# QiminWu/mceik

Hardware: AMD Instinct MI355X
Metric: MCMC proposals/sec (FSM eikonal + likelihood), 128³ grid, 1/2/4/8 MI355X (higher is better)
Workload: dtype f32

## Files before the change

### mceik_amd/csrc/capi.hip

```cpp
#include <hip/hip_runtime.h>
#include <float.h>
#include <math.h>
#include <stdint.h>
#include <stdio.h>
#include <stdlib.h>
#include <string.h>
#include <unistd.h>

#include <algorithm>
#include <vector>

#include "../../include/mceik.h"
#include "fsm_common.h"
#include "mcmc_common.h"
#include "fsm_single.h"
#include "rccl_rt.h"

hipError_t fsm_launch(const FsmLaunch &L, int is_double, int nwaves, hipStream_t st);
hipError_t fsm_zero_words(unsigned *p, int n, hipStream_t st);
int fsm_occupancy(const FsmLaunch &L, int is_double);
size_t fsm_launch_lds_bytes(const FsmLaunch &L, int is_double);
int fsm_launch_kind(const FsmLaunch &L, int is_double);
const char *fsm_launch_name(const FsmLaunch &L, int is_double);
hipError_t fsm_to_brick_f64(const double *src, void *dst, int dst_double, const FsmLaunch &L, int nfield, hipStream_t st);
hipError_t fsm_from_brick_f64(const void *src, int src_double, double *dst, const FsmLaunch &L, int nfield, hipStream_t st);
hipError_t fsm_from_brick_f32(const float *src, float *dst, const FsmLaunch &L, int nfield, hipStream_t st);
hipError_t fsm_to_brick_f32(const float *src, float *dst, const FsmLaunch &L, int nfield, hipStream_t st);
hipError_t mcmc_propose(const McmcDev &D, uint64_t step, hipStream_t st);
hipError_t mcmc_init_loglik(const McmcDev &D, hipStream_t st);
hipError_t mcmc_accept(const McmcDev &D, int keep_slot, hipStream_t st);
hipError_t mcmc_lpt_order(const unsigned long long *clk, int nsolve, int *order, hipStream_t st);
hipError_t l2_gridsearch_f32(int ldgrd, int ngrd, int nev, int iwantOT, float t0use, const int *ev_ptr,
                             const int *obs_row, const float *tc, const float *wt, const float *xnorm,
                             const float *test, float *t0, float *objfn, int negate, hipStream_t st);
size_t relocate_lds_bytes(int nrows, int nobs, int nev);
hipError_t relocate_lds(int ldgrd, int ngrd, int nrows, int nev, int nobs, int iwantOT, float t0use,
                        const int *ev_ptr, const int *obs_row, const float *tc, const float *wt, const float *xnorm,
                        const float *test, float *t0, float *objfn, int negate, hipStream_t st);
hipError_t gridsearch_f90(int is_double, int ldgrd, int ngrd, int nuse, int iwantOT, const int *row,
                          const void *tob, const void *w0, const void *wl, const void *test, void *logpdf,
                          hipStream_t st);
hipError_t l2_gridsearch(int ldgrd, int ngrd, int nuse, int iwantOT, double t0use, const int *use,
                         const double *tc, const double *wt, double xnorm, const double *test,
                         double *t0, double *objfn, hipStream_t st);

#define HIPCHK(x)                                                                      \
    do {                                                                               \
        hipError_t e_ = (x);                                                           \
        if (e_ != hipSuccess) {                                                        \
            fprintf(stderr, "mceik_hip: %s failed: %s (%s:%d)\n", #x,                  \
                    hipGetErrorString(e_), __FILE__, __LINE__);                        \
            return -1;                                                                 \
        }                                                                              \
    } while (0)

static double conv_threshold(double tol, int is_double)
{
    double tolr = is_double ? tol : (double)(float)tol;
    if (!(tolr > 0.0)) return HUGE_VAL;
    int p = is_double ? 53 : 24;
    int k = (int)ceil(log2(tolr)) + p;
    while (ldexp(1.0, k - p) < tolr) k++;
    while (ldexp(1.0, k - 1 - p) >= tolr) k--;
    double T = ldexp(1.0, k);
    double big = is_double ? DBL_MAX : (double)FLT_MAX;
    return T > big ? HUGE_VAL : T;
}

static void fill_launch(FsmLaunch &L, const mceik_fsm_batch *b)
{
    memset(&L, 0, sizeof(L));
    L.nx = b->nx; L.ny = b->ny; L.nz = b->nz;
    fsm_geometry(&L, b->precision == 64 ? 8 : 4);
    L.maxit = b->maxit; L.max_sweeps = b->max_sweeps;
    L.tol = b->tol; L.h = b->h; L.x0 = b->x0; L.y0 = b->y0; L.z0 = b->z0;
    int is_double = b->precision == 64;
    double T = conv_threshold(b->tol, is_double);
    L.conv_thresh = is_double ? (T == HUGE_VAL ? DBL_MAX : T) : (T == HUGE_VAL ? (double)FLT_MAX : T);
    L.nsolve = b->nmodel * b->nstat; L.nstat = b->nstat; L.nsrc = b->nsrc;
    L.src = b->src;
    L.slow_mode = b->slow_mode;
    L.nrx = b->nrx > 0 ? b->nrx : 1; L.nry = b->nry > 0 ? b->nry : 1; L.nrz = b->nrz > 0 ? b->nrz : 1;
    L.ncx = mceik_div_up(L.nx, L.nrx); L.ncy = mceik_div_up(L.ny, L.nry); L.ncz = mceik_div_up(L.nz, L.nrz);
    L.magic_rx = ((1u << 20) + L.nrx - 1) / L.nrx;
    L.magic_ry = ((1u << 20) + L.nry - 1) / L.nry;
    L.magic_rz = ((1u << 20) + L.nrz - 1) / L.nrz;
    L.ev_node = b->ev_node; L.nev = b->nev; L.ttab = b->ttab; L.ev_frac = b->ev_frac;
    L.model_phase = b->slow_mode == 1 ? b->model_phase : nullptr;
    L.skip = b->skip;
    L.solve_count = b->solve_count;
    L.nphase = b->nphase > 0 ? b->nphase : 1;
    {
        auto span = [](int a, int e, int nr) { return e / nr - a / nr + 1; };
        int mx = 0, my = 0, mz = 0;
        for (int t = 0; t < L.ntx; t++) {
            int v = span(t * 8, t * 8 + 7 < L.nx - 1 ? t * 8 + 7 : L.nx - 1, L.nrx); mx = v > mx ? v : mx;
        }
        for (int t = 0; t < L.nty; t++) {
            int v = span(t * 8, t * 8 + 7 < L.ny - 1 ? t * 8 + 7 : L.ny - 1, L.nry); my = v > my ? v : my;
        }
        for (int t = 0; t < L.nzk; t++) {
            int a = t * L.kb * 8, e = a + L.kb * 8 - 1 < L.nz - 1 ? a + L.kb * 8 - 1 : L.nz - 1;
            int v = span(a, e, L.nrz); mz = v > mz ? v : mz;
        }
        L.ccb = mx * my * mz;
        L.cell_cache = b->slow_mode == 1 && L.ccb <= MCEIK_CC_MAX && L.nx < 4096 && L.ny < 4096 && L.nz < 4096;
        if (!L.cell_cache) L.ccb = 0;
    }
    L.fast_sqrt = b->fast_sqrt;
    L.niter = b->niter; L.ierr = b->ierr;
    L.iter_total = b->iter_total;
    L.visit_stats = b->visit_stats;
    L.solve_order = b->solve_order;
    L.solve_clock = b->solve_clock;
    L.max_waves = b->max_waves;
    L.traffic = b->traffic;
    L.step_z = b->step_z;
}

static int g_device_cus = 0;

static int device_cus()
{
    if (g_device_cus == 0) {
        int dev = 0;
        hipDeviceProp_t p;
        if (hipGetDevice(&dev) == hipSuccess && hipGetDeviceProperties(&p, dev) == hipSuccess)
            g_device_cus = p.multiProcessorCount;
        else
            g_device_cus = 256;
    }
    return g_device_cus;
}

static size_t ws_budget_bytes()
{
    static size_t budget = 0;
    if (budget == 0) {
        const char *e = getenv("MCEIK_FSM_WS_GB");
        double gb = e ? atof(e) : 0.0;
        if (gb > 0.0) {
            budget = (size_t)(gb * 1073741824.0);
        } else {
            size_t fr = 0, tot = 0;
            const size_t margin = (size_t)8 << 30;
            if (hipMemGetInfo(&fr, &tot) == hipSuccess && tot) {
                budget = tot / 5 * 4;
                const size_t avail = fr > 2 * margin ? fr - margin : fr / 2;
                if (avail < budget) budget = avail;
            } else {
                budget = (size_t)96 << 30;
            }
        }
    }
    return budget;
}

static int batch_waves(const FsmLaunch &L, int is_double)
{
    int per_cu = fsm_occupancy(L, is_double);
    if (per_cu < 1) per_cu = 1;
    static const int env_cap = [] { const char *e = getenv("MCEIK_WAVES_PER_CU"); return e ? atoi(e) : 0; }();
    if (env_cap > 0 && env_cap < per_cu) per_cu = env_cap;
    long w = (long)per_cu * device_cus();
    if (L.max_waves > 0 && w > L.max_waves) w = L.max_waves;
    if (w > L.nsolve) w = L.nsolve;
    static const bool report = getenv("MCEIK_LAUNCH_REPORT") != nullptr;
    if (report)
        fprintf(stderr, "mceik fsm launch: %d-z steps, %d waves/CU (occupancy), %ld resident waves, %zu B LDS per wave\n",
                fsm_launch_kind(L, is_double), per_cu, w, fsm_launch_lds_bytes(L, is_double));
    return (int)(w < 1 ? 1 : w);
}

static int fsm_batch_waves_uncapped(const mceik_fsm_batch *b)
{
    FsmLaunch L;
    fill_launch(L, b);
    return batch_waves(L, b->precision == 64);
}

struct WsLayout {
    size_t counter, slow, u, u0, zf, total;
    int nwaves;
};

static WsLayout ws_layout(const mceik_fsm_batch *b)
{
    FsmLaunch L;
    fill_launch(L, b);
    int is_double = b->precision == 64;
    size_t es = is_double ? 8 : 4;
    WsLayout w;
    w.nwaves = batch_waves(L, is_double);
    const size_t zfw = fsm_launch_kind(L, is_double) == 16 ? zf_bytes(L, es) : 0;
    {
        const size_t per_wave = 2 * L.field_elems * es + zfw;
        const long cap = (long)(ws_budget_bytes() / (per_wave ? per_wave : 1));
        if (cap >= 1 && w.nwaves > cap) w.nwaves = (int)cap;
    }
    w.counter = 0;
    w.slow = 1024;
    size_t slow_bytes = b->slow_mode == 0 ? (size_t)b->nmodel * L.field_elems * es : 0;
    w.u = w.slow + ((slow_bytes + 255) & ~(size_t)255);
    size_t nu = b->u_out ? (size_t)L.nsolve : (size_t)w.nwaves;
    w.u0 = w.u + nu * L.field_elems * es;
    w.zf = w.u0 + (size_t)w.nwaves * L.field_elems * es;
    w.total = w.zf + (size_t)w.nwaves * zfw;
    return w;
}

extern "C" size_t mceik_fsm_workspace_bytes(const mceik_fsm_batch *b)
{
    return ws_layout(b).total;
}

extern "C" int mceik_fsm_step_z(const mceik_fsm_batch *b)
{
    if (!b) return 0;
    FsmLaunch L;
    fill_launch(L, b);
    return fsm_launch_kind(L, b->precision == 64);
}

extern "C" const char *mceik_fsm_kernel_name(const mceik_fsm_batch *b)
{
    if (!b) return "";
    FsmLaunch L;
    fill_launch(L, b);
    return fsm_launch_name(L, b->precision == 64);
}

extern "C" size_t mceik_fsm_lds_bytes(const mceik_fsm_batch *b)
{
    if (!b) return 0;
    FsmLaunch L;
    fill_launch(L, b);
    return fsm_launch_lds_bytes(L, b->precision == 64);
}

extern "C" double mceik_fsm_bytes_per_node_sweep(const mceik_fsm_batch *b)
{
    double es = b->precision == 64 ? 8.0 : 4.0;
    double s = b->slow_mode == 0 ? es : 4.0 / ((double)b->nrx * b->nry * b->nrz);
    return 2.0 * es + s / (b->nstat > 0 ? b->nstat : 1);
}

#define MCEIK_MC_CHUNK 64
struct McmcExt {
    const void *dev;
    unsigned *sync;
    unsigned spin_limit;
    int step0, nsteps, nburn, keepk, maxs, nkept0;
};

static int fsm_batch_solve_impl(const mceik_fsm_batch *b, void *workspace, size_t workspace_bytes, void *stream,
                                const McmcExt *ext);

extern "C" int mceik_fsm_batch_solve(const mceik_fsm_batch *b, void *workspace, size_t workspace_bytes,
                                     void *stream)
{
    return fsm_batch_solve_impl(b, workspace, workspace_bytes, stream, nullptr);
}

static int fsm_batch_solve_impl(const mceik_fsm_batch *b, void *workspace, size_t workspace_bytes, void *stream,
                                const McmcExt *ext)
{
    if (!b || b->nx < 2 || b->ny < 2 || b->nz < 2 || b->nx > 4096 || b->ny > 4096 || b->nz > 4096 ||
        b->nsrc < 1 ||
        b->nmodel < 1 || b->nstat < 1 || !(b->precision == 32 || b->precision == 64)) {
        fprintf(stderr, "mceik_fsm_batch_solve: invalid batch description\n");
        return 1;
    }
    if (b->slow_mode == 1 && b->precision != 32 && b->precision != 64) return 1;
    WsLayout w = ws_layout(b);
    {
        FsmLaunch G;
        fill_launch(G, b);
        if (G.field_elems * (b->precision == 64 ? 8 : 4) >= (size_t)1 << 31) {
            fprintf(stderr, "mceik_fsm_batch_solve: one travel-time field must stay below 2 GiB\n");
            return 1;
        }
        if (fsm_launch_lds_bytes(G, b->precision == 64) > MCEIK_MAX_LDS) {
            fprintf(stderr, "mceik_fsm_batch_solve: %d x %d x %d z-blocks exceed the LDS block tables\n", G.ntx, G.nty,
                    G.nzk);
            return 1;
        }
        const bool held = fsm_launch_kind(G, b->precision == 64) == 16 || fsm_compact_layout(G, 8);
        const int infl = fsm_launch_kind(G, b->precision == 64) == 16 ? fsm16_geo(G).infl : G.infl;
        if (held && hold_clock_bound(G.nblocks, infl) >= 65536) {
            fprintf(stderr, "mceik_fsm_batch_solve: %d z-blocks overflow the held stream's 16-bit clocks\n", G.nblocks);
            return 1;
        }
    }
    if (!workspace || workspace_bytes < w.total) {
        fprintf(stderr, "mceik_fsm_batch_solve: workspace too small (%zu < %zu)\n", workspace_bytes, w.total);
        return 1;
    }
    if (b->skip && b->u_out) {
        fprintf(stderr, "mceik_fsm_batch_solve: skip and u_out cannot be combined (a skipped solve has no field)\n");
        return 1;
    }
    hipStream_t st = (hipStream_t)stream;
    int is_double = b->precision == 64;
    FsmLaunch L;
    fill_launch(L, b);
    char *ws = (char *)workspace;
    L.counter = (unsigned *)(ws + w.counter);
    HIPCHK(fsm_zero_words(L.counter, 256, st));
    if (b->slow_mode == 0) {
        void *sb = ws + w.slow;
        if (is_double)
            HIPCHK(fsm_to_brick_f64((const double *)b->slow, sb, 1, L, b->nmodel, st));
        else
            HIPCHK(fsm_to_brick_f32((const float *)b->slow, (float *)sb, L, b->nmodel, st));
        L.slow = sb;
    } else {
        L.slow = b->slow;
    }
    L.u = ws + w.u;
    L.u0 = ws + w.u0;
    L.zf = ws + w.zf;
    L.slot_per_solve = b->u_out ? 1 : 0;
    if (ext) {
        if (is_double || fsm_launch_kind(L, 0) != 16 || b->solve_order || b->u_out) return 1;
        L.mc_dev = ext->dev;
        L.mc_sync = ext->sync;
        L.mc_spin_limit = ext->spin_limit;
        L.mc_step0 = ext->step0; L.mc_nsteps = ext->nsteps;
        L.mc_nburn = ext->nburn; L.mc_keepk = ext->keepk; L.mc_maxs = ext->maxs; L.mc_nkept0 = ext->nkept0;
        HIPCHK(fsm_zero_words(ext->sync, MC_SYNC_WORDS(L.nsolve / L.nstat) - 1, st));
    }
    HIPCHK(fsm_launch(L, is_double, w.nwaves, st));
    if (b->u_out) {
        if (is_double) HIPCHK(fsm_from_brick_f64(L.u, 1, (double *)b->u_out, L, L.nsolve, st));
        else HIPCHK(fsm_from_brick_f32((const float *)L.u, (float *)b->u_out, L, L.nsolve, st));
    }
    return 0;
}

static bool is_device_ptr(const void *p)
{
    hipPointerAttribute_t a;
    if (!p || hipPointerGetAttributes(&a, p) != hipSuccess) {
        (void)hipGetLastError();
        return false;
    }
    return a.type == hipMemoryTypeDevice;
}

extern "C" int eikonal3d_batch_solve(int nmodels, int nstations, int nx, int ny, int nz, double h, double x0,
                                     double y0, double z0, int maxit, double tol, const double *src,
                                     const float *slow, float *u, int *niter, int *ierr)
{
    if (nmodels < 1 || nstations < 1 || !src || !slow || !u) return 1;
    const size_t n = (size_t)nx * ny * nz, nsolve = (size_t)nmodels * nstations;
    mceik_fsm_batch b;
    memset(&b, 0, sizeof(b));
    b.nx = nx; b.ny = ny; b.nz = nz; b.h = h; b.x0 = x0; b.y0 = y0; b.z0 = z0;
    b.maxit = maxit; b.tol = tol; b.precision = 32;
    b.nmodel = nmodels; b.nstat = nstations; b.nsrc = 1; b.slow_mode = 0; b.max_sweeps = -1;
    std::vector<void *> tmp;
    auto stage = [&](const void *p, size_t bytes, bool in) -> void * {
        if (is_device_ptr(p)) return const_cast<void *>(p);
        void *d = nullptr;
        if (hipMalloc(&d, bytes) != hipSuccess) return nullptr;
        tmp.push_back(d);
        if (in && hipMemcpy(d, p, bytes, hipMemcpyHostToDevice) != hipSuccess) return nullptr;
        return d;
    };
    int rc = 0;
    void *d_src = stage(src, (size_t)nstations * 4 * sizeof(double), true);
    void *d_slow = stage(slow, (size_t)nmodels * n * sizeof(float), true);
    void *d_u = stage(u, nsolve * n * sizeof(float), false);
    void *d_it = niter ? stage(niter, nsolve * sizeof(int), false) : nullptr;
    void *d_ie = ierr ? stage(ierr, nsolve * sizeof(int), false) : nullptr;
    void *ws = nullptr;
    if (!d_src || !d_slow || !d_u || (niter && !d_it) || (ierr && !d_ie)) rc = -1;
    if (!rc) {
        b.src = (const double *)d_src; b.slow = d_slow; b.u_out = d_u;
        b.niter = (int *)d_it; b.ierr = (int *)d_ie;
        const size_t wsb = mceik_fsm_workspace_bytes(&b);
        if (hipMalloc(&ws, wsb) != hipSuccess) rc = -1;
        else rc = mceik_fsm_batch_solve(&b, ws, wsb, nullptr);
        if (!rc && hipDeviceSynchronize() != hipSuccess) rc = -1;
    }
    if (!rc && d_u != u) rc = hipMemcpy(u, d_u, nsolve * n * sizeof(float), hipMemcpyDeviceToHost) != hipSuccess;
    if (!rc && niter && d_it != niter) rc = hipMemcpy(niter, d_it, nsolve * sizeof(int), hipMemcpyDeviceToHost) != hipSuccess;
    if (!rc && ierr && d_ie != ierr) rc = hipMemcpy(ierr, d_ie, nsolve * sizeof(int), hipMemcpyDeviceToHost) != hipSuccess;
    if (ws) hipFree(ws);
    for (void *p : tmp) hipFree(p);
    return rc;
}

extern "C" int mceik_memcpy(void *dst, const void *src, size_t bytes, int kind)
{
    hipMemcpyKind k = kind == 0 ? hipMemcpyHostToDevice : kind == 1 ? hipMemcpyDeviceToHost : hipMemcpyDeviceToDevice;
    HIPCHK(hipMemcpy(dst, src, bytes, k));
    return 0;
}

struct SingleState {
    int init;
    int nx, ny, nz, maxit_cap, nsrc_cap;
    int is_double;
    SingleLaunch L;
    void *mem;
    double *dense, *src;
    int *ierr_bc;
    int nwaves;
    int bcfail;
    hipStream_t st;
    int iverb, maxit;
    double x0, y0, z0, h, tol;
    BlockDecomp D;
    double *snap;
    unsigned *d_count;
};
static SingleState g_single[3];

static void single_free(SingleState &S)
{
    if (S.snap) hipFree(S.snap);
    if (S.d_count) hipFree(S.d_count);
    if (S.mem) hipFree(S.mem);
    if (S.st) hipStreamDestroy(S.st);
    const SingleState keep = S;
    memset(&S, 0, sizeof(S));
    S.init = keep.init;
    S.iverb = keep.iverb; S.maxit = keep.maxit;
    S.x0 = keep.x0; S.y0 = keep.y0; S.z0 = keep.z0; S.h = keep.h; S.tol = keep.tol;
    S.D = keep.D;
}

static int blocks_buffers(SingleState &S)
{
    const size_t np = (size_t)S.L.nxp * S.L.nyp * S.L.nzp;
    if (!S.snap && hipMalloc(&S.snap, np * 8) != hipSuccess) { S.snap = nullptr; return 1; }
    if (!S.d_count && hipMalloc(&S.d_count, 16) != hipSuccess) { S.d_count = nullptr; return 1; }
    return 0;
}

static int single_alloc(SingleState &S, int is_double, int nx, int ny, int nz, int maxit, int nsrc)
{
    if (S.mem && S.is_double == is_double && S.nx == nx && S.ny == ny && S.nz == nz && maxit <= S.maxit_cap &&
        nsrc <= S.nsrc_cap)
        return 0;
    const int keep = S.init;
    single_free(S);
    S.init = keep;
    if (nx < 1 || ny < 1 || nz < 1 || (long)nx * ny * nz >= (1L << 31)) return 1;
    SingleLaunch &L = S.L;
    L.nx = nx; L.ny = ny; L.nz = nz;
    L.gx = nx; L.gy = ny; L.gz = nz;
    L.nbx = mceik_div_up(nx, 8); L.nby = mceik_div_up(ny, 8); L.nbz = mceik_div_up(nz, 8);
    if (L.nbx > 1024 || L.nby > 1024 || L.nbz > 1024) return 1;
    L.nxp = 8 * L.nbx; L.nyp = 8 * L.nby; L.nzp = 8 * L.nbz;
    L.nb = L.nbx * L.nby * L.nbz;
    if ((size_t)L.nxp * L.nyp * L.nzp * (is_double ? 8 : 4) >= ((size_t)1 << 31)) return 1;
    const int mcap = maxit > 0 ? maxit : 1, scap = nsrc > 0 ? nsrc : 1;
    const size_t es = is_double ? 8 : 4, np = (size_t)L.nxp * L.nyp * L.nzp, n = (size_t)nx * ny * nz;
    auto al = [](size_t v) { return (v + 255) & ~(size_t)255; };
    size_t off[12], o = 0;
    off[0] = o; o += al(np * es);
    off[1] = o; o += al(np * es);
    off[2] = o; o += al(np * es);
    off[3] = o; o += al(np);
    off[4] = o; o += al((size_t)L.nb * 4);
    off[5] = o; o += al((size_t)L.nb * 4);
    off[6] = o; o += al((size_t)(32 + mcap) * 4);
    off[7] = o; o += al((size_t)mcap * 8);
    off[8] = o; o += al((size_t)mcap * 4);
    off[9] = o; o += al(n * 8);
    off[10] = o; o += al((size_t)scap * 32);
    off[11] = o; o += al(16);
    if (hipMalloc(&S.mem, o) != hipSuccess) { S.mem = nullptr; return 1; }
    char *m = (char *)S.mem;
    L.u = m + off[0]; L.u0 = m + off[1]; L.slow = m + off[2]; L.bc = (unsigned char *)(m + off[3]);
    L.border = (const int *)(m + off[4]); L.done = (unsigned *)(m + off[5]); L.ctl = (unsigned *)(m + off[6]);
    L.arrive = (unsigned long long *)(m + off[7]); L.ierr_it = (int *)(m + off[8]);
    S.dense = (double *)(m + off[9]); S.src = (double *)(m + off[10]); S.ierr_bc = (int *)(m + off[11]);
    L.bcerr = S.ierr_bc;
    std::vector<int> ord;
    ord.reserve(L.nb);
    for (int lev = 0; lev <= L.nbx + L.nby + L.nbz - 3; lev++)
        for (int bz = 0; bz < L.nbz; bz++)
            for (int by = 0; by < L.nby; by++) {
                const int bx = lev - bz - by;
                if (bx >= 0 && bx < L.nbx) ord.push_back(bx | (by << 10) | (bz << 20));
            }
    if ((int)ord.size() != L.nb ||
        hipMemcpy((void *)L.border, ord.data(), ord.size() * 4, hipMemcpyHostToDevice) != hipSuccess ||
        hipStreamCreateWithFlags(&S.st, hipStreamNonBlocking) != hipSuccess) {
        single_free(S);
        return 1;
    }
    static const int wpc = [] { const char *e = getenv("MCEIK_SINGLE_WAVES_PER_CU"); return e ? atoi(e) : 2; }();
    int occ = fsm_single_occupancy(is_double);
    S.nwaves = device_cus() * std::max(1, std::min(wpc, occ));
    S.is_double = is_double; S.nx = nx; S.ny = ny; S.nz = nz; S.maxit_cap = mcap; S.nsrc_cap = scap;
    return 0;
}

static int single_solve(SingleState &S, int maxit, int nsrc, double tol, double h, double x0, double y0, double z0,
                        const double *ts, const double *xs, const double *ys, const double *zs, const double *slow,
                        double *u, int *niter_out)
{
    SingleLaunch &L = S.L;
    const size_t n = (size_t)L.nx * L.ny * L.nz;
    L.maxit = maxit; L.tol = tol; L.h = h; L.x0 = x0; L.y0 = y0; L.z0 = z0;
    std::vector<double> src((size_t)nsrc * 4);
    for (int k = 0; k < nsrc; k++) {
        src[k * 4 + 0] = ts[k]; src[k * 4 + 1] = xs[k]; src[k * 4 + 2] = ys[k]; src[k * 4 + 3] = zs[k];
    }
    const int mcap = maxit > 0 ? maxit : 1;
    std::vector<unsigned> ctl(32 + mcap);
    std::vector<int> ierr_it(mcap);
    int ierr_bc = 0;
    hipStream_t st = S.st;
    if (hipMemcpyAsync(S.dense, slow, n * 8, hipMemcpyHostToDevice, st) != hipSuccess ||
        hipMemcpyAsync(S.src, src.data(), src.size() * 8, hipMemcpyHostToDevice, st) != hipSuccess ||
        fsm_single_pad(S.dense, (void *)L.slow, S.is_double, L.nx, L.ny, L.nz, L.nxp, L.nyp, st) != hipSuccess ||
        hipMemsetAsync(L.done, 0, (size_t)L.nb * 4, st) != hipSuccess ||
        hipMemsetAsync(L.ctl, 0, (size_t)(32 + mcap) * 4, st) != hipSuccess ||
        hipMemsetAsync(L.arrive, 0, (size_t)mcap * 8, st) != hipSuccess ||
        hipMemsetAsync(L.ierr_it, 0, (size_t)mcap * 4, st) != hipSuccess ||
        fsm_single_solve(L, S.is_double, S.src, nsrc, S.ierr_bc, S.nwaves, st) != hipSuccess ||
        fsm_single_unpad(L.u, S.dense, S.is_double, L.nx, L.ny, L.nz, L.nxp, L.nyp, st) != hipSuccess ||
        hipMemcpyAsync(u, S.dense, n * 8, hipMemcpyDeviceToHost, st) != hipSuccess ||
        hipMemcpyAsync(ctl.data(), L.ctl, ctl.size() * 4, hipMemcpyDeviceToHost, st) != hipSuccess ||
        hipMemcpyAsync(ierr_it.data(), L.ierr_it, ierr_it.size() * 4, hipMemcpyDeviceToHost, st) != hipSuccess ||
        hipMemcpyAsync(&ierr_bc, S.ierr_bc, 4, hipMemcpyDeviceToHost, st) != hipSuccess ||
        hipStreamSynchronize(st) != hipSuccess)
        return -1;
    if (ctl[1] != 0) {
        std::vector<unsigned> done(L.nb);
        std::vector<unsigned long long> arr(mcap);
        hipMemcpy(done.data(), L.done, done.size() * 4, hipMemcpyDeviceToHost);
        hipMemcpy(arr.data(), L.arrive, arr.size() * 8, hipMemcpyDeviceToHost);
        unsigned dmin = ~0u, dmax = 0;
        for (unsigned d : done) { dmin = std::min(dmin, d); dmax = std::max(dmax, d); }
        fprintf(stderr, "mceik_hip: single-solve schedule timed out (code %u; waits timed out: deps %u, "
                        "iteration %u; tasks taken %u, nb %d, done %u..%u, arrivals it0 %llu/%llu it1 %llu, "
                        "decisions %u %u %u)\n", ctl[1], ctl[3], ctl[4], ctl[0], L.nb, dmin, dmax,
                arr[0] & 0xffffffffull, arr[0] >> 32, mcap > 1 ? arr[1] & 0xffffffffull : 0ull, ctl[32],
                mcap > 1 ? ctl[33] : 0u, mcap > 2 ? ctl[34] : 0u);
        return -1;
    }
    S.bcfail = ierr_bc != 0;
    if (ierr_bc) {
        if (niter_out) *niter_out = 0;
        return 1;
    }
    int niter = maxit > 0 ? maxit : 0;
    for (int it = 0; it < maxit; it++)
        if (ctl[32 + it] == 2) { niter = it + 1; break; }
    if (niter_out) *niter_out = niter;
    return niter > 0 ? ierr_it[niter - 1] : 0;
}

static void serial_driver(int is_double, const int *job, const int *iverb, const int *maxit,
                          const int *nsrc, const int *nx, const int *ny, const int *nz,
                          const double *tol, const double *h, const double *x0, const double *y0,
                          const double *z0, const double *ts, const double *xs, const double *ys,
                          const double *zs, const double *slow, double *u, int *ierr)
{
    SingleState &S = g_single[is_double];
    *ierr = 0;
    if (*job == 1) {
        if (S.init) { printf(" eikonal3d_serial_driver: Already initialized!\n"); *ierr = 1; return; }
        if (*iverb > 0) printf(" eikonal3d_serial_driver: Generating levels...\n");
        if (single_alloc(S, is_double, *nx, *ny, *nz, *maxit, *nsrc)) {
            printf(" eikonal3d_serial_driver: Error generating level structure\n");
            *ierr = 1;
            return;
        }
        S.init = 1;
        return;
    }
    if (*job != 2) {
        if (!S.init) printf(" eikonal3d_serial_driver: Never initialized!\n");
        single_free(S);
        S.init = 0;
        return;
    }
    if (!S.init) { printf(" eikonal3d_serial_driver: Solver not initalized!\n"); *ierr = 1; return; }
    if (*nsrc < 1) {
        printf(" eikonal3d_serial_driver: nsrc must be >= 1\n");
        *ierr = 1;
        return;
    }
    if (single_alloc(S, is_double, *nx, *ny, *nz, *maxit, *nsrc)) {
        printf(" eikonal3d_serial_driver: device allocation failed\n");
        *ierr = 1;
        return;
    }
    if (*iverb > 0) printf(" eikonal3d_serial_driver: Setting boundary conditions...\n");
    const int rc = single_solve(S, *maxit, *nsrc, *tol, *h, *x0, *y0, *z0, ts, xs, ys, zs, slow, u, nullptr);
    if (rc < 0) {
        printf(" eikonal3d_serial_driver: device failure\n");
        *ierr = 1;
        return;
    }
    *ierr = rc;
    if (S.bcfail) printf(" eikonal3d_serial_driver: Error setting boundary conditions\n");
    else if (rc != 0) printf(" eikonal3d_serial_driver: Error solving eikonal equation\n");
}

extern "C" void eikonal3d_serial_driver(const int *job, const int *iverb, const int *maxit, const int *nsrc,
                                        const int *nx, const int *ny, const int *nz, const double *tol,
                                        const double *h, const double *x0, const double *y0, const double *z0,
                                        const double *ts, const double *xs, const double *ys, const double *zs,
                                        const double *slow, double *u, int *ierr)
{
    serial_driver(1, job, iverb, maxit, nsrc, nx, ny, nz, tol, h, x0, y0, z0, ts, xs, ys, zs, slow, u, ierr);
}

extern "C" void eikonal3d_serial_driver_sp(const int *job, const int *iverb, const int *maxit, const int *nsrc,
                                           const int *nx, const int *ny, const int *nz, const double *tol,
                                           const double *h, const double *x0, const double *y0, const double *z0,
                                           const double *ts, const double *xs, const double *ys, const double *zs,
                                           const double *slow, double *u, int *ierr)
{
    serial_driver(0, job, iverb, maxit, nsrc, nx, ny, nz, tol, h, x0, y0, z0, ts, xs, ys, zs, slow, u, ierr);
// ... 1581 lines not shown
```

### mceik_amd/csrc/fsm16_kernel.hip

```cpp
#include <hip/hip_runtime.h>
#include <float.h>
#include <stdint.h>

#include "fsm_common.h"
#include "fsm_device.h"
#include "fsm_hold.h"
#include "fsm_update.h"
#include "mcmc_device.h"

namespace {

__device__ __forceinline__ uint32_t zoff16(int zb)
{
    const uint32_t u = (uint32_t)zb;
    return ((u >> 1) << 13) | ((u & 1u) << 6);
}

#ifdef MCEIK_PHASECLK
#undef TRAF
#undef TRAFU
#define TRAF(S, k, pred, bytes) do { } while (0)
#define TRAFU(S, k, bytes) do { } while (0)
#define PCLK(k)                                                                                         \
    do {                                                                                                \
        const unsigned long long t_ = __builtin_readcyclecounter();                                     \
        if (threadIdx.x == 0) S.scratch[8 + (k)] += (int)(t_ - pclk_t);                                 \
        pclk_t = t_;                                                                                    \
    } while (0)
#else
#define PCLK(k) do { } while (0)
#endif

struct Smem16 {
    int *box;
    float *cc;
    unsigned short *order;
    unsigned short *lastproc;
    unsigned short *lastchg;
    int *ring_e, *ring_b;
    unsigned *ring_base;
    unsigned *fmask;
    int *scratch;
    float *xr;
    unsigned *meta;
    unsigned char *fz;
    unsigned *vbits, *cbits;
};
template <bool FIXED>
__device__ __forceinline__ Smem16 smem16_bind(const FsmLaunch &L, unsigned char *base)
{
    size_t off[MCEIK_SMEM16_ARRAYS];
    if (FIXED) {
        off[8] = F16_CINFO; off[7] = F16_XR; off[1] = F16_CC; off[5] = F16_RING; off[6] = F16_SCRATCH;
        off[3] = F16_LASTPROC; off[4] = F16_LASTCHG; off[2] = F16_ORDER;
        off[9] = F16_ORDER + mceik_align16((size_t)L.ntiles * 2);
        off[10] = off[9] + mceik_align16((size_t)L.ntiles);
        off[0] = off[10] + f16_bitmap_bytes(L);
    } else {
        fsm16_smem_layout(L, off);
    }
    const int nr = fsm16_geo(L).nr;
    Smem16 S;
    S.box = reinterpret_cast<int *>(base + off[0]);
    S.cc = reinterpret_cast<float *>(base + off[1]);
    S.order = reinterpret_cast<unsigned short *>(base + off[2]);
    S.lastproc = reinterpret_cast<unsigned short *>(base + off[3]);
    S.lastchg = reinterpret_cast<unsigned short *>(base + off[4]);
    S.ring_e = reinterpret_cast<int *>(base + off[5]);
    S.ring_b = S.ring_e + (FIXED ? F16_NR : nr);
    S.ring_base = reinterpret_cast<unsigned *>(S.ring_b + (FIXED ? F16_NR : nr));
    S.fmask = S.ring_base + (FIXED ? F16_NR : nr);
    S.fz = base + off[9];
    S.vbits = reinterpret_cast<unsigned *>(base + off[10]);
    S.cbits = S.vbits + (L.nblocks + 31) / 32;
    S.scratch = reinterpret_cast<int *>(base + off[6]);
    S.xr = reinterpret_cast<float *>(base + off[7]);
    S.meta = reinterpret_cast<unsigned *>(base + off[8]);
    return S;
}

#define XROW16(arr, q, row) (((arr) * 4 + (q)) * MCEIK_X16Q + (row) * 4)
typedef float f4v16 __attribute__((ext_vector_type(4)));
__device__ __forceinline__ void lds_w4(float *p, float a, float b, float c, float d)
{
    *reinterpret_cast<f4v16 *>(p) = f4v16{a, b, c, d};
}
__device__ __forceinline__ void lds_r4(const float *p, float &a, float &b, float &c, float &d)
{
    const f4v16 v = *reinterpret_cast<const f4v16 *>(p);
    a = v.x; b = v.y; c = v.z; d = v.w;
}
__device__ __forceinline__ void store_row16(float *x, int arr, int lane, const float (&v)[16])
{
#pragma unroll
    for (int q = 0; q < 4; q++) lds_w4(x + XROW16(arr, q, lane), v[4 * q], v[4 * q + 1], v[4 * q + 2], v[4 * q + 3]);
}
__device__ __forceinline__ void load_row16(const float *x, int arr, int row, float (&v)[16])
{
#pragma unroll
    for (int q = 0; q < 4; q++) lds_r4(x + XROW16(arr, q, row), v[4 * q], v[4 * q + 1], v[4 * q + 2], v[4 * q + 3]);
}
__device__ __forceinline__ void load_half16(const float *x, int arr, int row, int h, float (&v)[8])
{
    lds_r4(x + XROW16(arr, 2 * h, row), v[0], v[1], v[2], v[3]);
    lds_r4(x + XROW16(arr, 2 * h + 1, row), v[4], v[5], v[6], v[7]);
}
__device__ __forceinline__ void halo_stage16(float *x, int lane, const float (&v)[8])
{
    const int j = lane >> 1, h = lane & 1;
    const int arr = (j >> 3) & 1, row = 64 + ((j >> 4) << 3) + (j & 7);
    lds_w4(x + XROW16(arr, 2 * h, row), v[0], v[1], v[2], v[3]);
    lds_w4(x + XROW16(arr, 2 * h + 1, row), v[4], v[5], v[6], v[7]);
}

#define NPASS16 4
#define W1_ZD (1u << 24)

__device__ __forceinline__ void seg_issue(Rsrc r, uint32_t seg, float (&a)[16])
{
    const bool odd = threadIdx.x & 1;
    const uint32_t segp = dpp_swap_pair(seg);
    float t[4];
    bload4(r, odd ? segp + 16u : seg, t);
    a[0] = t[0]; a[1] = t[1]; a[2] = t[2]; a[3] = t[3];
    bload4(r, odd ? segp + 48u : seg + 32u, t);
    a[4] = t[0]; a[5] = t[1]; a[6] = t[2]; a[7] = t[3];
    bload4(r, odd ? seg + 16u : segp, t);
    a[8] = t[0]; a[9] = t[1]; a[10] = t[2]; a[11] = t[3];
    bload4(r, odd ? seg + 48u : segp + 32u, t);
    a[12] = t[0]; a[13] = t[1]; a[14] = t[2]; a[15] = t[3];
}
#define XQE MCEIK_X16Q
__device__ __forceinline__ int pair_row(int arr, int lane)
{
    return (lane & 1) ? XROW16(arr, 1, lane - 1) : XROW16(arr, 0, lane);
}
__device__ __forceinline__ void raw_write(float *x, int pb, const float (&a)[16])
{
    lds_w4(x + pb, a[0], a[1], a[2], a[3]);
    lds_w4(x + pb + 2 * XQE, a[4], a[5], a[6], a[7]);
    lds_w4(x + pb + 4, a[8], a[9], a[10], a[11]);
    lds_w4(x + pb + 2 * XQE + 4, a[12], a[13], a[14], a[15]);
}
__device__ __forceinline__ void raw_read(const float *x, int pb, float (&a)[16])
{
    lds_r4(x + pb, a[0], a[1], a[2], a[3]);
    lds_r4(x + pb + 2 * XQE, a[4], a[5], a[6], a[7]);
    lds_r4(x + pb + 4, a[8], a[9], a[10], a[11]);
    lds_r4(x + pb + 2 * XQE + 4, a[12], a[13], a[14], a[15]);
}
template <int P>
struct Par16 {
    static constexpr int value = P;
};

struct LineLd {
    float a[8];
    int rowl, rowo;
};
__device__ __forceinline__ void line_issue(Rsrc r, uint32_t seg, bool isl, LineLd &q, float (&h)[8])
{
    const int lane = threadIdx.x, par = lane & 1;
    const bool islp = dpp_swap_pair((unsigned)isl) != 0u;
    const uint32_t segp = dpp_swap_pair(seg);
    const uint32_t sl = isl ? seg : (islp ? segp : OOB);
    const uint32_t o = (uint32_t)par * 16u;
    float t[4];
    bload4(r, sl + o, t);
    q.a[0] = t[0]; q.a[1] = t[1]; q.a[2] = t[2]; q.a[3] = t[3];
    bload4(r, sl + o + 32u, t);
    q.a[4] = t[0]; q.a[5] = t[1]; q.a[6] = t[2]; q.a[7] = t[3];
    const uint32_t sh = sl ^ 64u;
    bload4(r, sh + o, t);
    h[0] = t[0]; h[1] = t[1]; h[2] = t[2]; h[3] = t[3];
    bload4(r, sh + o + 32u, t);
    h[4] = t[0]; h[5] = t[1]; h[6] = t[2]; h[7] = t[3];
    q.rowl = isl ? lane : (lane ^ 1);
    q.rowo = lane ^ (q.rowl == lane ? 1 : 0);
}
__device__ __forceinline__ void line_write(float *x, const LineLd &q, const float (&hp)[8])
{
    const int par = threadIdx.x & 1;
    lds_w4(x + XROW16(1, par, q.rowl), q.a[0], q.a[1], q.a[2], q.a[3]);
    lds_w4(x + XROW16(1, par + 2, q.rowl), q.a[4], q.a[5], q.a[6], q.a[7]);
    lds_w4(x + XROW16(1, par, q.rowo), hp[0], hp[1], hp[2], hp[3]);
    lds_w4(x + XROW16(1, par + 2, q.rowo), hp[4], hp[5], hp[6], hp[7]);
}

__device__ __forceinline__ void raw_store(Rsrc r, uint32_t seg, bool chg, const float (&t)[16])
{
    const bool odd = threadIdx.x & 1;
    const uint32_t own = chg ? seg : OOB;
    const uint32_t oth = dpp_swap_pair(own);
    const uint32_t o = odd ? 16u : 0u;
    const uint32_t b01 = (odd ? oth : own) + o, b23 = (odd ? own : oth) + o;
    bstore4(r, b01, t[0], t[1], t[2], t[3]);
    bstore4(r, b01 + 32u, t[4], t[5], t[6], t[7]);
    bstore4(r, b23, t[8], t[9], t[10], t[11]);
    bstore4(r, b23 + 32u, t[12], t[13], t[14], t[15]);
}
__device__ __forceinline__ void store16_plain(Rsrc r, uint32_t off, const float (&v)[16])
{
#pragma unroll
    for (int q = 0; q < 4; q++) bstore4(r, off + 16u * q, v[4 * q], v[4 * q + 1], v[4 * q + 2], v[4 * q + 3]);
}

__device__ __forceinline__ void bload4h(Rsrc r, uint32_t off, float (&v)[4])
{
    f4v a = __builtin_bit_cast(f4v, __builtin_amdgcn_raw_buffer_load_b128(r, off, 0, 0));
    v[0] = a.x; v[1] = a.y; v[2] = a.z; v[3] = a.w;
}
struct BInfo16 {
    uint32_t seg;
    uint32_t zh;
    uint32_t lseg;
    uint32_t w1, w2, w3;
    __device__ __forceinline__ int fl() const { return (int)(w1 & 0xfffu); }
    __device__ __forceinline__ int zb() const { return (int)((w1 >> 12) & 0xffu); }
    __device__ __forceinline__ int ri() const { return (int)((w1 >> 20) & 0xfu); }
    __device__ __forceinline__ int ccb() const { return (int)(w2 << 16) >> 16; }
    __device__ __forceinline__ int clk() const { return (int)(w2 >> 16); }
    __device__ __forceinline__ int bid() const { return (int)(w3 & 0xffffu); }
    __device__ __forceinline__ int bcm() const { return (int)(w3 >> 16); }
};
template <bool RZ>
__device__ __forceinline__ BInfo16 brick_info16(const FsmLaunch &L, const Fsm16Geo &g, int kb, const Smem16 &S,
                                                const Pos &p, int nstream, int lx, int ly, const BcBoxes &bc,
                                                unsigned meta, uint32_t col)
{
    BInfo16 b;
    const int tz = ci_tz(meta);
    const int zb = tz * kb + (RZ ? kb - 1 - p.zbs : p.zbs);
    const bool valid = pos_valid(p, nstream) && (meta & C_BLK) && zb < g.nzb;
    b.seg = valid ? col + zoff16(zb) : OOB;
    b.lseg = pos_valid(p, nstream) && (meta & C_BLK) && (zb & ~1) < g.nzb ? col + zoff16(zb) : OOB;
    const int zu = RZ ? zb * 16 + 16 : zb * 16 - 1;
    b.zh = (valid && (meta & C_ZH) && p.zbs == 0) ? col + zoff16(zu >> 4) + (uint32_t)(zu & 15) * 4u : OOB;
    int fl = valid ? (int)((meta & 0x7f) | F_VALID) : 0;
    if (zb == (RZ ? g.nzb - 1 : 0)) fl |= F_FIRST;
    if (zb == (RZ ? 0 : g.nzb - 1)) fl |= F_LAST;
    const bool zd = valid && p.zbs == kb - 1 && !(fl & F_LAST);
    if (b.zh != OOB) b.zh = zf_boundary<float, RZ>(L, S.ring_b[p.ri], false, lx, ly);
    if (zd) b.zh = zf_boundary<float, RZ>(L, S.ring_b[p.ri], true, lx, ly);
    if ((meta & C_ZH) && p.zbs == 0) fl |= F_ZH;
    bool slow = (fl & C_PART) || ((fl & C_00) && zb == 0) || (valid && zb * 16 + 16 > L.nz);
    unsigned bcm = 0;
    if (__any(fl & C_BC)) {
        const int e = S.ring_e[p.ri];
        const int x = (e & 0xfff) * 8 + lx, y = ((e >> 12) & 0xfff) * 8 + ly;
        unsigned m = 0;
        if (fl & C_BC) {
            for (int k = 0; k < bc.n; k++) {
                const int *q = bc.box + 6 * k;
                if (x >= q[0] && x <= q[1] && y >= q[2] && y <= q[3]) {
                    int lo = q[4] - zb * 16, hi = q[5] - zb * 16;
                    lo = lo < 0 ? 0 : lo; hi = hi > 15 ? 15 : hi;
                    if (lo <= hi) m |= ((2u << hi) - (1u << lo));
                }
            }
        }
        bcm = m;
        slow |= m != 0;
    }
    if (slow) fl |= F_SLOW;
    const int ccb = ci_ccb(meta) + zb * 4;
    b.w1 = (uint32_t)fl | ((uint32_t)(valid ? zb : 0) << 12) | ((uint32_t)p.ri << 20) | (zd ? W1_ZD : 0u);
    b.w2 = ((uint32_t)ccb & 0xffffu) | ((uint32_t)p.sp << 16);
    b.w3 = ((uint32_t)S.ring_b[p.ri] & 0xffffu) | (bcm << 16);
    return b;
}
template <bool RZ>
__device__ __forceinline__ uint32_t halo_offset16(const Fsm16Geo &g, int kb, const Pos &pe, int nstream, int half,
                                                  unsigned meta, uint32_t col, unsigned hbit, uint32_t hdelta)
{
    const int zb = ci_tz(meta) * kb + (RZ ? kb - 1 - pe.zbs : pe.zbs);
    const bool valid = pos_valid(pe, nstream) && (meta & C_BLK) && zb < g.nzb;
    const uint32_t base = col + ((meta & hbit) ? 0u : hdelta);
    return valid ? base + zoff16(zb) + (uint32_t)half * 32u : OOB;
}

#define LW_G(p) (9 + 5 * (p))
#define LW_CCB 19
template <bool RZ>
__device__ __forceinline__ unsigned lean_word(const FsmLaunch &L, const Fsm16Geo &g, const ColTile &ct, int tz, int ri,
                                              int u0flag, int zh)
{
    int cz0, nczb;
    block_zcells(L, L.kb, tz, cz0, nczb);
    const int m = ct.fl | C_BLK | (u0flag ? C_U0 : 0) | (zh ? C_ZH : 0);
    const int zb0 = 2 * tz + (RZ ? 1 : 0);
    unsigned w = (unsigned)m & 0x1ffu;
#pragma unroll
    for (int p = 0; p < 2; p++) {
        const int zb = RZ ? zb0 - p : zb0 + p;
        unsigned gp = zb < g.nzb ? 16u : 0u;
        if (zb == (RZ ? g.nzb - 1 : 0)) gp |= 1u;
        if (zb == (RZ ? 0 : g.nzb - 1)) gp |= 2u;
        if ((m & C_PART) || ((m & C_00) && zb == 0) || zb * 16 + 16 > L.nz) gp |= 4u;
        if (p == 0 && (m & C_ZH)) gp |= 8u;
        w |= gp << LW_G(p);
    }
    const int ccb0 = ri * L.ccb + ct.cl * nczb - cz0 + zb0 * 4;
    return w | ((unsigned)ccb0 << LW_CCB);
}
template <bool RZ>
__device__ __forceinline__ BInfo16 brick_info_lean(const FsmLaunch &L, const Smem16 &S, const Pos &p, int nstream,
                                                   int lx, int ly, const BcBoxes &bc, unsigned w, uint32_t base)
{
    BInfo16 b;
    const int ph = p.zbs;
    const unsigned gp = (w >> (ph ? LW_G(1) : LW_G(0))) & 31u;
    const bool pv = pos_valid(p, nstream);
    const bool valid = pv && (gp & 16u);
    const uint32_t off = base + ((uint32_t)(ph ^ (RZ ? 1 : 0)) << 6);
    b.seg = valid ? off : OOB;
    b.lseg = pv && (w & ((16u << LW_G(0)) | (16u << LW_G(1)))) ? off : OOB;
    b.zh = valid && (gp & 8u) ? off + (RZ ? 8192u - 64u : 124u - 8192u) : OOB;
    const bool zd = valid && ph == 1 && !(gp & 2u);
    if (b.zh != OOB) b.zh = zf_boundary<float, RZ>(L, S.ring_b[p.ri], false, lx, ly);
    if (zd) b.zh = zf_boundary<float, RZ>(L, S.ring_b[p.ri], true, lx, ly);
    int fl = valid ? (int)((w & 0x7fu) | F_VALID | ((gp & 15u) << 8)) : 0;
    unsigned bcm = 0;
    if (__any(fl & C_BC)) {
        const int e = S.ring_e[p.ri];
        const int zb = 2 * ((e >> 24) & 0xff) + (RZ ? 1 - ph : ph);
        const int x = (e & 0xfff) * 8 + lx, y = ((e >> 12) & 0xfff) * 8 + ly;
        if (fl & C_BC) {
            for (int k = 0; k < bc.n; k++) {
                const int *q = bc.box + 6 * k;
                if (x >= q[0] && x <= q[1] && y >= q[2] && y <= q[3]) {
                    int lo = q[4] - zb * 16, hi = q[5] - zb * 16;
                    lo = lo < 0 ? 0 : lo; hi = hi > 15 ? 15 : hi;
                    if (lo <= hi) bcm |= ((2u << hi) - (1u << lo));
                }
            }
        }
        if (bcm) fl |= F_SLOW;
    }
    const int ccb = (int)(w >> LW_CCB) + (RZ ? -4 * ph : 4 * ph);
    b.w1 = (uint32_t)fl | ((uint32_t)ph << 12) | ((uint32_t)p.ri << 20) | (zd ? W1_ZD : 0u);
    b.w2 = ((uint32_t)ccb & 0xffffu) | ((uint32_t)p.sp << 16);
    b.w3 = ((uint32_t)S.ring_b[p.ri] & 0xffffu) | (bcm << 16);
    return b;
}
template <bool RZ>
__device__ __forceinline__ uint32_t halo_offset_lean(const Pos &pe, int nstream, int half, unsigned me, uint32_t base,
                                                     unsigned hbit, uint32_t hdelta)
{
    const int ph = pe.zbs;
    const bool valid = pos_valid(pe, nstream) && ((me >> (ph ? LW_G(1) : LW_G(0))) & 16u);
    const uint32_t o = base + ((me & hbit) ? 0u : hdelta) + ((uint32_t)(ph ^ (RZ ? 1 : 0)) << 6) + (uint32_t)half * 32u;
    return valid ? o : OOB;
}
template <bool RZ>
__device__ __forceinline__ uint32_t halo_line_lean(const Pos &pe, int nstream, unsigned me, uint32_t base,
                                                   unsigned hbit, uint32_t hdelta)
{
    const bool valid = pos_valid(pe, nstream) && (me & ((16u << LW_G(0)) | (16u << LW_G(1))));
    return valid ? base + ((me & hbit) ? 0u : hdelta) : OOB;
}
__device__ __forceinline__ unsigned dpp_swap_quad_half(unsigned v)
{
    return (unsigned)__builtin_amdgcn_mov_dpp((int)v, 0x4E, 0xf, 0xf, false);
}
template <bool RZ, bool LEAN>
__device__ __forceinline__ BInfo16 brick_info_any(const FsmLaunch &L, const Fsm16Geo &g, int kb, const Smem16 &S,
                                                  const Pos &p, int nstream, int lx, int ly, const BcBoxes &bc,
                                                  unsigned meta, uint32_t col)
{
    if (LEAN) return brick_info_lean<RZ>(L, S, p, nstream, lx, ly, bc, meta, col);
    return brick_info16<RZ>(L, g, kb, S, p, nstream, lx, ly, bc, meta, col);
}
template <bool RZ, bool LEAN>
__device__ __forceinline__ uint32_t halo_offset_any(const Fsm16Geo &g, int kb, const Pos &pe, int nstream, int half,
                                                    unsigned meta, uint32_t col, unsigned hbit, uint32_t hdelta)
{
    if (LEAN) return halo_offset_lean<RZ>(pe, nstream, half, meta, col, hbit, hdelta);
    return halo_offset16<RZ>(g, kb, pe, nstream, half, meta, col, hbit, hdelta);
}

__device__ __forceinline__ void build_order16(const FsmLaunch &L, unsigned short *order)
{
    for (int id = threadIdx.x; id < L.ntiles; id += 64) {
        const int txs = id % L.ntx, tys = id / L.ntx, dg = txs + tys;
        int rank = 0;
        for (int e = 0; e < dg; e++)
            rank += min(e, L.nty - 1) - max(0, e - L.ntx + 1) + 1;
        rank += tys - max(0, dg - L.ntx + 1);
        order[rank] = (unsigned short)(txs | (tys << 8));
    }
}


__device__ __forceinline__ HoldLds<unsigned short> hold_lds16(const Smem16 &S)
{
    HoldLds<unsigned short> H;
    H.order = S.order; H.fz = S.fz; H.lastproc = S.lastproc; H.need = S.lastchg; H.fmask = S.fmask;
    H.ring_e = S.ring_e; H.vbits = S.vbits; H.cbits = S.cbits;
    return H;
}


template <bool RZ, bool LEAN>
__device__ __forceinline__ void admit16(const FsmLaunch &L, const Fsm16Geo &g, const Smem16 &S, const BcBoxes &bc,
                                        int entry, int zh, int u0flag, int ri, int C, int lx, int ly, int lxs,
                                        int lys, int rx, int ry, ColTile &ct)
{
    unsigned meta = 0;
    int bid = 0, nbv = 0;
    uint32_t base = 0;
    if (entry >= 0) {
        const int tz = (entry >> 24) & 0xff, tx = entry & 0xfff, ty = (entry >> 12) & 0xfff;
        bid = tz * L.ntiles + tx + ty * L.ntx;
        nbv = min(L.kb, L.nzb - tz * L.kb);
        if ((entry & 0xffffff) != ct.tile) column_tile<float>(L, bc, entry, lx, ly, lxs, lys, rx, ry, ct);
        meta = LEAN ? lean_word<RZ>(L, g, ct, tz, ri, u0flag, zh) : column_word(L, L.kb, ct, tz, ri, u0flag, zh);
        base = (uint32_t)(ty * L.ntx + tx) * tile_bytes<float>(L) + (LEAN ? (uint32_t)tz << 13 : 0u);
    }
    const int nact = L.visit_stats && entry >= 0 ? __builtin_popcountll(__ballot(ct.fl & C_ACT)) : 0;
    asm volatile("" ::: "memory");
    S.meta[ri * 64 + threadIdx.x] = meta;
    if (threadIdx.x == 0) {
        if (entry >= 0) {
            S.lastproc[bid] = (unsigned short)C;
            S.vbits[bid >> 5] |= 1u << (bid & 31);
            if (L.visit_stats) {
                S.scratch[0] += nbv;
                S.scratch[1] += nbv * nact;
            }
        }
        S.ring_e[ri] = entry;
        S.ring_b[ri] = bid;
        S.ring_base[ri] = base;
    }
    asm volatile("" ::: "memory");
}


template <bool RZ, bool GENERIC, bool LEAN, bool NC = true>
__device__ __forceinline__ void brick16(const FsmLaunch &L, const Smem16 &S, const BInfo16 &b0, float (&v)[16],
                                        float zprev0, float znext, int lx, int ly, int rx, int ry, bool &changed,
                                        bool &nc, int &ierr_last, bool &c0, bool &c15)
{
    const int lane = threadIdx.x;
    const float T = (float)L.conv_thresh;
    const int fl = b0.fl();
    bool xp = true, xn = true, yp = true, yn = true, act = true;
    int zbg = 0;
    if (GENERIC) {
        const int e = S.ring_e[b0.ri()];
        zbg = LEAN ? 2 * ((e >> 24) & 0xff) + (RZ ? 1 - b0.zb() : b0.zb()) : b0.zb();
        const int x = (e & 0xfff) * 8 + lx, y = ((e >> 12) & 0xfff) * 8 + ly;
        const bool xlo = x > 0, xhi = x < L.nx - 1, ylo = y > 0, yhi = y < L.ny - 1;
        xp = rx ? xhi : xlo; xn = rx ? xlo : xhi; yp = ry ? yhi : ylo; yn = ry ? ylo : yhi;
        act = (fl & C_ACT) != 0;
    }
    const bool first = (fl & F_FIRST) != 0, last = (fl & F_LAST) != 0;
    const int lxs = lane & 7, lys = lane >> 3;
    const int rxm = lxs > 0 ? lane - 1 : 64 + lys, rym = lys > 0 ? lane - 8 : 72 + lxs;
    const int rxp = lxs < 7 ? lane + 1 : 64 + lys, ryp = lys < 7 ? lane + 8 : 72 + lxs;
    float fc = 0.f, ffc = 0.f, ff2c = 0.f, ff3c = 0.f;
#pragma unroll
    for (int hh = 0; hh < NPASS16; hh++) {
        constexpr int PZ = 16 / NPASS16;
        const int h = RZ ? NPASS16 - 1 - hh : hh;
        float xm[PZ], xq[PZ], ym[PZ], yq[PZ];
        lds_r4(S.xr + XROW16(0, h, rxm), xm[0], xm[1], xm[2], xm[3]);
        lds_r4(S.xr + XROW16(0, h, rym), ym[0], ym[1], ym[2], ym[3]);
        lds_r4(S.xr + XROW16(1, h, rxp), xq[0], xq[1], xq[2], xq[3]);
        lds_r4(S.xr + XROW16(1, h, ryp), yq[0], yq[1], yq[2], yq[3]);
#pragma unroll
        for (int jj = 0; jj < PZ; jj++) {
            const int j = hh * PZ + jj;
            const int pj = RZ ? 15 - j : j;
            const int ph = pj % PZ;
            const int pprev = RZ ? pj + 1 : pj - 1, pnext = RZ ? pj - 1 : pj + 1;
            const float self = v[pj];
            if (!GENERIC) {
                if ((j & 3) == 0) {
                    fc = S.cc[b0.ccb() + (pj >> 2)];
                    ffc = fc * fc;
                    ff2c = ffc + ffc;
                    ff3c = 3.0f * ffc;
                }
            }
            float xup = xm[ph], xdn = xq[ph], yup = ym[ph], ydn = yq[ph];
            float zup, zdn;
            if (GENERIC) {
                xup = xp ? xup : self; xdn = xn ? xdn : self; yup = yp ? yup : self; ydn = yn ? ydn : self;
                const int zabs = zbg * 16 + pj;
                const bool zp_ex = RZ ? (zabs < L.nz - 1) : (zabs > 0);
                const bool zn_ex = RZ ? (zabs > 0) : (zabs < L.nz - 1);
                zup = zp_ex ? (j > 0 ? v[pprev] : zprev0) : self;
                zdn = zn_ex ? (j < 15 ? v[pnext] : znext) : self;
            } else {
                zup = j > 0 ? v[pprev] : (first ? self : zprev0);
                zdn = j < 15 ? v[pnext] : (last ? self : znext);
            }
            const float ux = fmin_(xup, xdn), uy = fmin_(yup, ydn), uz = fmin_(zup, zdn);
            float nv;
            if (GENERIC) {
                const int zabs = zbg * 16 + pj;
                const int zc_ = zabs < L.nz ? zabs : L.nz - 1;
                const float f = S.cc[b0.ccb() - zbg * 4 + (zc_ >> 2)];
                int e;
                const float ub = godunov_bl<true>(ux, uy, uz, f, e);
                const bool upd = act && zabs < L.nz && !((b0.bcm() >> pj) & 1);
                nv = upd ? fmin_(self, ub) : self;
                if ((fl & C_00) && zabs == 0) ierr_last = upd ? e : 0;
            } else {
                nv = fmin_(self, godunov_v<true>(ux, uy, uz, fc, ffc, ff2c, ff3c));
            }
            const bool dec = nv < self;
            if (NC) nc |= dec && self >= T;
            changed |= dec;
            if (pj == 0) c0 = dec;
            if (pj == 15) c15 = dec;
            v[pj] = nv;
        }
    }
}

template <bool RZ, int KB16, int CCR>
__device__ __forceinline__ int sweep16(const FsmLaunch &L, const Fsm16Geo &g, Rsrc ur, Rsrc u0r, Rsrc sr, Rsrc zfr,
                                       const BcBoxes &bc, const Smem16 &S, int rx, int ry, int clock0, bool &notconv,
                                       int &ierr_last, unsigned &nchg, unsigned &nsteps)
{
    const Rsrc zr_ = zfr;
#ifdef MCEIK_PHASECLK
    unsigned long long pclk_t = __builtin_readcyclecounter();
#endif
    const int lane = threadIdx.x, lxs = lane & 7, lys = lane >> 3, d = lxs + lys;
    const int lx = rx ? 7 - lxs : lxs, ly = ry ? 7 - lys : lys;
    const float UN = FLT_MAX;
    const int kb = KB16 > 0 ? KB16 : g.kb;
    const int nr = KB16 > 0 ? F16_NR : g.nr;
    const uint32_t lanecol = (uint32_t)colpos(lx, ly) * 128u;

    const int hj = lane >> 1, hh = lane & 1, he = halo_edge_lane(hj), hd = (he & 7) + (he >> 3);
    const unsigned hbit = hj < 16 ? C_XOWN : C_YOWN;
    const uint32_t hdelta = halo_delta(L, tile_bytes<float>(L), hj, he, rx, ry);
    const int hlx = rx ? 7 - (he & 7) : (he & 7), hly = ry ? 7 - (he >> 3) : (he >> 3);
    const uint32_t hcol = (uint32_t)colpos(hlx, hly) * 128u;

    const HoldLds<unsigned short> H = hold_lds16(S);
    const unsigned xyface = HOLD_OWN | (lx == 0 ? 2u : 0u) | (lx == 7 ? 4u : 0u) | (ly == 0 ? 8u : 0u) |
                            (ly == 7 ? 16u : 0u);
    hold_norm(L, H);
    if (lane == 0) { S.scratch[4] = 0; S.scratch[5] = -1; }
    clock0 = 64;
    auto decide_any = [&](int pos, int ri, int &zh, int &u0) __attribute__((always_inline)) -> int {
        const HoldSt hs = hold_state(S.scratch + 4);
        const int q = pos - g.infl;
        if (q >= 0) hold_settle(L, H, q % nr, clock0 + q);
        return hold_decide<RZ>(L, H, S.scratch + 4, hs, clock0 + pos, rx, ry, ri == 0 ? nr - 1 : ri - 1, g.infl,
                               g.vis, zh, u0);
    };
    constexpr bool FL = KB16 == 2;
    constexpr bool LEAN = KB16 == 2;
    float v[16], qa[16], hs[2][8];
    LineLd lq;
    float hps[2][8];
    float (&hq)[8] = hs[0];
    constexpr bool HFL = FL && LEAN;
    const int hr = lane & 3, hpi = (lane >> 4) & 1, hcme = (lane >> 1) & 1;
    const int hj0 = (lane >> 1) & ~1;
    const int hst = XROW16((hj0 >> 3) & 1, hr, 64 + ((hj0 >> 4) << 3) + (hj0 & 7));
    float hA[2][4], hB[2][4], hBs[4];
    float (&hn)[8] = hs[1];
    float (&hp)[8] = hps[0];
    float zc, zn, zq;
    float ccv[CCR];
    int ccsize = 0;
    ColTile ct;
    ct.tile = -1;
    constexpr int AH = MCEIK_AHEAD16;
    int ndecided = 0, nstream = 0x7fffffff, dri = 0;
    for (int pos = 0; pos <= (AH - 1) / kb; pos++) {
        int zh, u0;
        const int e = decide_any(pos, dri, zh, u0);
        if (e == -2) {
            if (pos == 0) return 0;
            nstream = pos;
            break;
        }
        admit16<RZ, LEAN>(L, g, S, bc, e, zh, u0, dri, clock0 + pos, lx, ly, lxs, lys, rx, ry, ct);
        if (e >= 0) {
            cc_issue<CCR>(L, L.kb, sr, e, ccv, ccsize);
            TRAFU(S, 5, ccsize * 4);
            cc_write<float, CCR>(L, S.cc, dri, ccv, ccsize, (float)L.h);
        }
        ndecided = pos + 1;
        if (++dri == nr) dri = 0;
    }
    asm volatile("" ::: "memory");
    Pos p3, pe;
    pos_init(p3, -d, kb, nr);
    BInfo16 b0 = brick_info_any<RZ, LEAN>(L, g, kb, S, p3, nstream, lx, ly, bc, S.meta[p3.ri * 64 + lane],
                                  S.ring_base[p3.ri] + lanecol);
    const int pbr = pair_row(0, lane), pbn = pair_row(1, lane);
    {
        float t[16];
        seg_issue(ur, b0.seg, t);
        raw_write(S.xr, pbn, t);
        load_row16(S.xr, 1, lane, v);
    }
    pos_init(pe, -hd, kb, nr);
    {
        const uint32_t ho = halo_offset_any<RZ, LEAN>(g, kb, pe, nstream, hh, S.meta[pe.ri * 64 + he],
                                              S.ring_base[pe.ri] + hcol, hbit, hdelta);
        bload4h(ur, ho, *reinterpret_cast<float (*)[4]>(&hq[0]));
        bload4h(ur, ho + 16u, *reinterpret_cast<float (*)[4]>(&hq[4]));
        TRAF(S, 1, ho != OOB, 32);
    }
    zc = bload1(zr_, b0.zh, 0.0f);
    TRAF(S, 0, b0.seg != OOB, 64);
    TRAF(S, 2, b0.zh != OOB, 4);
    pos_adv(p3, kb, nr);
    BInfo16 b1 = brick_info_any<RZ, LEAN>(L, g, kb, S, p3, nstream, lx, ly, bc, S.meta[p3.ri * 64 + lane],
                                  S.ring_base[p3.ri] + lanecol);
    {
        float t[16];
        seg_issue(ur, b1.seg, t);
        raw_write(S.xr, pbn, t);
    }
    if (FL) {
        Pos pn = p3;
        pos_adv(pn, kb, nr);
        const bool nl = pn.vb >= 0 && pn.zbs == 1;
        const uint32_t sn = nl ? brick_info_any<RZ, LEAN>(L, g, kb, S, pn, nstream, lx, ly, bc, S.meta[pn.ri * 64 + lane],
                                                  S.ring_base[pn.ri] + lanecol).seg
                               : OOB;
        const bool nlp = dpp_swap_pair((unsigned)nl) != 0u;
        const uint32_t snp = dpp_swap_pair(sn);
        const uint32_t s0 = (nl ? sn : (nlp ? snp : OOB)) + (uint32_t)(lane & 1) * 16u;
        float t[4];
        bload4(ur, s0, t);
        hp[0] = t[0]; hp[1] = t[1]; hp[2] = t[2]; hp[3] = t[3];
        bload4(ur, s0 + 32u, t);
        hp[4] = t[0]; hp[5] = t[1]; hp[6] = t[2]; hp[7] = t[3];
#pragma unroll
        for (int i = 0; i < 8; i++) asm volatile("" : "+v"(hp[i]));
    }
    pos_adv(pe, kb, nr);
    if (HFL) {
        const uint32_t lo = halo_line_lean<RZ>(pe, nstream, S.meta[pe.ri * 64 + he], S.ring_base[pe.ri] + hcol, hbit,
                                               hdelta);
        const uint32_t lp = dpp_swap_quad_half(lo);
        const uint32_t l1 = hcme == (hpi ^ 1) ? lo : lp, l0 = hcme == hpi ? lo : lp;
        const uint32_t qo = 16u * (uint32_t)hr, oa = (RZ ? 64u : 0u) + qo, ob = (RZ ? 0u : 64u) + qo;
        bload4h(ur, l1 + oa, hA[1]);
        bload4h(ur, l0 + ob, hB[0]);
        bload4h(ur, l1 + ob, hB[1]);
        TRAF(S, 1, l1 != OOB, 32);
    } else {
        const uint32_t ho = halo_offset_any<RZ, LEAN>(g, kb, pe, nstream, hh, S.meta[pe.ri * 64 + he],
                                              S.ring_base[pe.ri] + hcol, hbit, hdelta);
        bload4h(ur, ho, *reinterpret_cast<float (*)[4]>(&hn[0]));
        bload4h(ur, ho + 16u, *reinterpret_cast<float (*)[4]>(&hn[4]));
        TRAF(S, 1, ho != OOB, 32);
    }
    zn = bload1(zr_, b1.zh, 0.0f);
    TRAF(S, 0, b1.seg != OOB, 64);
    TRAF(S, 2, b1.zh != OOB, 4);
    {
        float un[16];
#pragma unroll
        for (int i = 0; i < 16; i++) un[i] = UN;
        store_row16(S.xr, 0, lane, un);
    }
    halo_stage16(S.xr, lane, hq);
    float zprev = UN;
    if (HFL) {
#pragma unroll
        for (int i = 0; i < 4; i++) asm volatile("" : "+v"(hA[1][i]), "+v"(hB[0][i]), "+v"(hB[1][i]));
    } else {
#pragma unroll
        for (int i = 0; i < 8; i++) hs[0][i] = hs[1][i];
#pragma unroll
        for (int i = 0; i < 8; i++) asm volatile("" : "+v"(hs[0][i]));
    }
#pragma unroll
    for (int i = 0; i < 16; i++) asm volatile("" : "+v"(v[i]));
    asm volatile("" : "+v"(zc), "+v"(zn));
    asm volatile("" ::: "memory");

    int ph = AH % kb;
    int cc_pend = -1;
    int B = 0;
    bool ccfill = false;
    int ccri = 0;
    auto decide_step = [&]() __attribute__((always_inline)) {
        ccfill = false;
        ccri = 0;
        if (ph == 0 && nstream == 0x7fffffff) {
            const int pos = ndecided;
            int zh, u0;
            const int e = decide_any(pos, dri, zh, u0);
            PCLK(4);
            if (e == -2) {
                nstream = pos;
            } else {
                admit16<RZ, LEAN>(L, g, S, bc, e, zh, u0, dri, clock0 + pos, lx, ly, lxs, lys, rx, ry, ct);
                if (e >= 0) {
                    cc_issue<CCR>(L, L.kb, sr, e, ccv, ccsize);
                    TRAFU(S, 5, ccsize * 4);
                    ccfill = true;
                    ccri = dri;
                }
                ndecided = pos + 1;
                if (++dri == nr) dri = 0;
            }
        }
    };
    auto more = [&]() __attribute__((always_inline)) -> bool {
        return !(nstream != 0x7fffffff && B >= nstream * kb + 14);
    };
    auto step = [&](auto par) __attribute__((always_inline)) -> bool {
        constexpr int P = FL ? decltype(par)::value : 0;
        float (&hcur)[8] = hs[P];
        float (&hnew)[8] = hs[1 - P];
        float (&hpcur)[8] = hps[P];
        float (&hpnew)[8] = hps[1 - P];
        pos_adv(p3, kb, nr);
        pos_adv(pe, kb, nr);
        const unsigned m3 = S.meta[p3.ri * 64 + lane], me = S.meta[pe.ri * 64 + he];
        const uint32_t c3 = S.ring_base[p3.ri] + lanecol, ce = S.ring_base[pe.ri] + hcol;
        __builtin_amdgcn_sched_barrier(0);
        const BInfo16 b3 = brick_info_any<RZ, LEAN>(L, g, kb, S, p3, nstream, lx, ly, bc, m3, c3);
        if (FL)
            line_issue(ur, b3.lseg, p3.vb >= 0 && p3.zbs == 0, lq, hpnew);
        else
            seg_issue(ur, b3.seg, qa);
        zq = __any(b3.zh != OOB) ? bload1(zr_, b3.zh, 0.0f) : 0.0f;
        if (HFL) {
            const uint32_t lo = halo_line_lean<RZ>(pe, nstream, me, ce, hbit, hdelta);
            const uint32_t lp = dpp_swap_quad_half(lo);
            const uint32_t sl = hcme == (hpi ^ P) ? lo : lp;
            const uint32_t qo = 16u * (uint32_t)hr;
#pragma unroll
            for (int i = 0; i < 4; i++) hBs[i] = hB[P][i];
            bload4h(ur, sl + (RZ ? 64u : 0u) + qo, hA[P]);
            bload4h(ur, sl + (RZ ? 0u : 64u) + qo, hB[P]);
            TRAF(S, 1, sl != OOB, 32);
            TRAF(S, 0, b3.seg != OOB, 64);
            TRAF(S, 2, b3.zh != OOB, 4);
        } else {
            const uint32_t ho = halo_offset_any<RZ, LEAN>(g, kb, pe, nstream, hh, me, ce, hbit, hdelta);
            bload4h(ur, ho, *reinterpret_cast<float (*)[4]>(&hnew[0]));
            bload4h(ur, ho + 16u, *reinterpret_cast<float (*)[4]>(&hnew[4]));
            TRAF(S, 1, ho != OOB, 32);
            TRAF(S, 0, b3.seg != OOB, 64);
            TRAF(S, 2, b3.zh != OOB, 4);
        }
        PCLK(0);
        __builtin_amdgcn_s_setprio(0);
        const bool wnc = !__any(notconv);
        if (wnc && __any(b0.fl() & C_U0)) {
            unsigned m = __builtin_bit_cast(unsigned, v[0]);
#pragma unroll
            for (int i = 1; i < 16; i++) m = min(m, __builtin_bit_cast(unsigned, v[i]));
            const bool st0 = __builtin_bit_cast(float, m) < (float)L.conv_thresh && (b0.fl() & C_U0);
            if (__any(st0)) store16_plain(u0r, st0 ? b0.seg : OOB, v);
            TRAF(S, 4, st0, 64);
        }
        float znext = S.xr[XROW16(1, RZ ? 3 : 0, lane) + (RZ ? 3 : 0)];
        const unsigned fmk = S.fmask[b0.ri()];
        if ((b0.w1 & W1_ZD) && !(fmk & HOLD_CONT)) znext = zc;
        const float zp0 = (b0.fl() & F_ZH) ? zc : zprev;
        PCLK(1);
        bool changed = false, nc = false, c0 = false, c15 = false;
        if (__any(b0.fl() & F_SLOW))
            brick16<RZ, true, LEAN>(L, S, b0, v, zp0, znext, lx, ly, rx, ry, changed, nc, ierr_last, c0, c15);
        else if (wnc)
            brick16<RZ, false, LEAN>(L, S, b0, v, zp0, znext, lx, ly, rx, ry, changed, nc, ierr_last, c0, c15);
        else
            brick16<RZ, false, LEAN, false>(L, S, b0, v, zp0, znext, lx, ly, rx, ry, changed, nc, ierr_last, c0, c15);
        const bool val = (b0.fl() & F_VALID) != 0;
        changed = changed && val;
        notconv |= nc && val;
        nchg += changed ? 2u : 0u;
        PCLK(2);
        __builtin_amdgcn_s_setprio(2);

        if (cc_pend >= 0) cc_write<float, CCR>(L, S.cc, cc_pend, ccv, ccsize, (float)L.h);
        cc_pend = ccfill ? ccri : -1;
        float nn[16];
        if (FL) {
#pragma unroll
            for (int i = 0; i < 8; i++) asm volatile("" : "+v"(lq.a[i]), "+v"(hpnew[i]));
        } else {
#pragma unroll
            for (int i = 0; i < 16; i++) nn[i] = qa[i];
        }
        if (HFL) {
            const int lc = hpi ^ P;
            lds_w4(S.xr + hst + 4 * (1 - lc), hA[1 - P][0], hA[1 - P][1], hA[1 - P][2], hA[1 - P][3]);
            lds_w4(S.xr + hst + 4 * lc, hBs[0], hBs[1], hBs[2], hBs[3]);
        } else {
            halo_stage16(S.xr, lane, hcur);
        }
        zc = zn; zn = zq;
        if (!FL) {
#pragma unroll
            for (int i = 0; i < 16; i++) asm volatile("" : "+v"(nn[i]));
        }
        if (!FL) {
#pragma unroll
            for (int i = 0; i < 8; i++) hcur[i] = hnew[i];
        }
        if (HFL) {
#pragma unroll
            for (int i = 0; i < 4; i++) asm volatile("" : "+v"(hA[P][i]), "+v"(hB[P][i]));
        } else {
            asm volatile("" : "+v"(hnew[0]), "+v"(hnew[1]), "+v"(hnew[2]), "+v"(hnew[3]), "+v"(hnew[4]),
                         "+v"(hnew[5]), "+v"(hnew[6]), "+v"(hnew[7]));
        }
        asm volatile("" : "+v"(zn));
        asm volatile("" ::: "memory");
        store_row16(S.xr, 0, lane, v);
        zprev = v[RZ ? 0 : 15];
        if (__any(changed)) {
            float t[16];
            raw_read(S.xr, pbr, t);
            raw_store(ur, b0.seg, changed, t);
        }
        TRAF(S, 3, changed, 64);
        {
            const int zr = LEAN ? (b0.zb() ^ (RZ ? 1 : 0)) : b0.zb() % kb;
            const bool zlo = changed && zr == 0 && c0, zhi = changed && zr == kb - 1 && c15;
            if (changed) atomicOr(&S.fmask[b0.ri()], xyface | (zlo ? HOLD_ZLO : 0u) | (zhi ? HOLD_ZHI : 0u));
            if (__any(zlo || zhi)) {
                bstore1(zfr, zlo ? zf_off<float>(b0.bid(), 0, lx, ly) : OOB, v[0]);
                bstore1(zfr, zhi ? zf_off<float>(b0.bid(), 1, lx, ly) : OOB, v[15]);
            }
        }
        load_row16(S.xr, 1, lane, v);
        if (FL) {
            line_write(S.xr, lq, hpcur);
        } else {
            raw_write(S.xr, pbn, nn);
        }
        asm volatile("" ::: "memory");
        b0 = b1;
        b1 = b3;
        if (++ph == kb) ph = 0;
        B++;
        PCLK(3);
        decide_step();
        PCLK(5);
        return more();
    };
    decide_step();
    PCLK(6);
    if (more()) {
        if (FL) {
            do {
                if (!step(Par16<0>())) break;
            } while (step(Par16<1>()));
        } else {
            do {
            } while (step(Par16<0>()));
        }
    }
    __builtin_amdgcn_s_setprio(0);
    nsteps += (unsigned)B;
    for (int q = max(0, nstream - g.infl + 1); q < nstream; q++) hold_settle(L, H, q % nr, clock0 + q);
    PCLK(6);
    return nstream;
}

__device__ __forceinline__ void verify16(const FsmLaunch &L, Rsrc ur, Rsrc u0r, const Smem16 &S, bool &notconv)
{
    const int lane = threadIdx.x, lx = lane & 7, ly = lane >> 3;
    const float T = (float)L.conv_thresh, tolr = (float)L.tol;
    for (int base = 0; base < L.nblocks; base += 64) {
        const int k = base + lane;
        const bool flag = k < L.nblocks && ((S.cbits[k >> 5] >> (k & 31)) & 1u) != 0;
        unsigned long long m = __ballot(flag);
        while (m) {
            const int bid = base + __builtin_ctzll(m);
            m &= m - 1;
            const int tz = bid / L.ntiles, id = bid - tz * L.ntiles;
            const int tx = id % L.ntx, ty = id / L.ntx;
            const int x = tx * 8 + lx, y = ty * 8 + ly;
            const int zend = min(tz * L.kb + L.kb, L.nzb);
            for (int zb = tz * L.kb; zb < zend; zb++) {
                const uint32_t seg = (uint32_t)id * tile_bytes<float>(L) + zoff_bytes<float>(zb) +
                                     (uint32_t)colpos(lx, ly) * 128u;
                float u[8], v0[8];
                bload8(ur, seg, u);
                bload8(u0r, seg, v0);
                TRAF(S, 6, x < L.nx && y < L.ny, 64);
#pragma unroll
                for (int i = 0; i < 8; i++) {
                    float dl = v0[i] - u[i];
                    dl = dl < 0.0f ? -dl : dl;
                    if (x < L.nx && y < L.ny && zb * 8 + i < L.nz && u[i] < T && !(dl < tolr)) notconv = true;
                }
            }
        }
    }
}

struct McQueue {
    unsigned xcc;
    int cur;
};
__device__ __forceinline__ unsigned mc_group_tickets(const FsmLaunch &L, int g, int &clo)
{
    const int nch = L.nsolve / L.nstat;
    clo = (int)((long long)nch * g / 8);
    const int chi = (int)((long long)nch * (g + 1) / 8);
    return (unsigned)(chi - clo) * (unsigned)L.nstat;
}
__device__ __forceinline__ void mc_l1_invalidate()
{
    asm volatile("buffer_inv sc1\n\ts_waitcnt vmcnt(0)" ::: "memory");
}
__device__ __forceinline__ void mc_stores_done()
{
    asm volatile("s_waitcnt vmcnt(0)" ::: "memory");
}
__device__ __forceinline__ bool mc_next(const FsmLaunch &L, McQueue &q, int &solve, int &k)
{
    const int lane = threadIdx.x;
    unsigned *owner = L.mc_sync, *tick = L.mc_sync + 8;
    int *ready = reinterpret_cast<int *>(L.mc_sync + 8 + 8 * 32);
    for (;;) {
        if (q.cur >= 0) {
            int clo;
            const unsigned gs = mc_group_tickets(L, q.cur, clo), tot = gs * (unsigned)L.mc_nsteps;
            unsigned t = 0;
            if (lane == 0) t = atomicAdd(tick + 32 * q.cur, 1u);
            t = __builtin_amdgcn_readfirstlane(__shfl(t, 0, 64));
            if (t < tot) {
                k = (int)(t / gs);
                solve = clo * L.nstat + (int)(t - (unsigned)k * gs);
                const int c = solve / L.nstat;
                unsigned broken = 0;
                if (lane == 0) {
                    for (unsigned it = 0; atomicAdd(ready + c, 0) < k; it++) {
                        if (it >= L.mc_spin_limit) {
                            atomicExch(L.mc_sync + MC_SYNC_WORDS(L.nsolve / L.nstat) - 1, 1u);
                            broken = 1;
                            break;
                        }
                        __builtin_amdgcn_s_sleep(32);
                    }
                }
                broken = __builtin_amdgcn_readfirstlane(__shfl(broken, 0, 64));
                if (broken) return false;
                __builtin_amdgcn_wave_barrier();
                mc_l1_invalidate();
                return true;
            }
            q.cur = -1;
        }
        int found = -1;
        for (int j = 0; j < 8 && found < 0; j++) {
            const int g = (int)((q.xcc - 1u + (unsigned)j) & 7u);
            unsigned own = 0, left = 0;
            if (lane == 0) {
                own = atomicCAS(owner + g, 0u, q.xcc);
                if (own == 0u) own = q.xcc;
                int clo;
                const unsigned tot = mc_group_tickets(L, g, clo) * (unsigned)L.mc_nsteps;
                left = own == q.xcc && atomicAdd(tick + 32 * g, 0u) < tot ? 1u : 0u;
            }
            left = __builtin_amdgcn_readfirstlane(__shfl(left, 0, 64));
            if (left) found = g;
        }
        if (found < 0) return false;
        q.cur = found;
    }
}
__device__ __forceinline__ int mc_keep_slot(const FsmLaunch &L, long long gs)
{
    if (!L.mc_maxs || gs < L.mc_nburn || (gs - L.mc_nburn) % L.mc_keepk) return -1;
    auto nk = [&](long long x) -> long long {
        return x <= L.mc_nburn ? 0 : (x - L.mc_nburn + L.mc_keepk - 1) / L.mc_keepk;
    };
    return (int)((L.mc_nkept0 + nk(gs) - nk(L.mc_step0)) % L.mc_maxs);
}
__device__ __forceinline__ void mc_finish(const FsmLaunch &L, int solve, int k)
{
    const int lane = threadIdx.x;
    const int nch = L.nsolve / L.nstat, c = solve / L.nstat;
    int *ready = reinterpret_cast<int *>(L.mc_sync + 8 + 8 * 32);
    unsigned *done = L.mc_sync + 8 + 8 * 32 + nch;
    mc_stores_done();
    unsigned old = 0;
    if (lane == 0) old = atomicAdd(done + c, 1u);
    old = __builtin_amdgcn_readfirstlane(__shfl(old, 0, 64));
    if (old + 1u != (unsigned)(k + 1) * (unsigned)L.nstat) return;
    mc_l1_invalidate();
    const McmcDev &D = *reinterpret_cast<const McmcDev *>(L.mc_dev);
    const long long gstep = (long long)L.mc_step0 + k;
    const int keep_slot = mc_keep_slot(L, gstep);
    const int inp = mcmcd::ldv(&D.prop_inprior[c]), ph = mcmcd::ldv(&D.prop_phase[c]);
    double ln = 0.0;
    if (inp) {
        for (int e0 = 0; e0 < D.nev; e0 += 64) {
            const int e = e0 + lane, n = min(64, D.nev - e0);
            const double obj = e < D.nev ? mcmcd::event_obj(D, c, ph, e) : 0.0;
            for (int i = 0; i < n; i++) ln = ln - __shfl(obj, i, 64);
        }
    }
    int acc = 0;
    if (lane == 0) acc = mcmcd::chain_accept(D, c, ln, keep_slot);
    acc = __builtin_amdgcn_readfirstlane(__shfl(acc, 0, 64));
    if (acc && D.nphase > 1) mcmcd::chain_copy_tables(D, c, ph, lane, 64);
    if (keep_slot >= 0) {
        const int cell = mcmcd::ldv(&D.prop_cell[c]), pv = mcmcd::ldv(&D.prop_v[c]);
        int *dst = D.keep_v + ((size_t)keep_slot * D.keep_stride + c) * D.ncm;
        const int *src = D.v + (size_t)c * D.ncm;
        for (int j = lane; j < D.ncm; j += 64) dst[j] = (acc && j == cell) ? pv : mcmcd::ldv(src + j);
    }
    if (k + 1 < L.mc_nsteps && lane == 0) mcmcd::chain_propose(D, c, (uint64_t)(gstep + 1));
    mc_stores_done();
    if (lane == 0) atomicExch(ready + c, k + 1);
}

template <int KB16, int CCR, bool MC>
__device__ __forceinline__ void fsm16_body(const FsmLaunch &L)
{
    extern __shared__ __attribute__((aligned(16))) unsigned char smem[];
    const Smem16 S = smem16_bind<KB16 == 2>(L, smem);
    const Fsm16Geo g = fsm16_geo(L);
    const int lane = threadIdx.x;
    const uint32_t fbytes = (uint32_t)(L.field_elems * 4);
    build_order16(L, S.order);
    int pass = 0;
    McQueue mq;
    mq.cur = -1;
    mq.xcc = 1u;
    if (MC) {
        unsigned x;
        asm volatile("s_getreg_b32 %0, hwreg(HW_REG_XCC_ID)" : "=s"(x));
        mq.xcc = (x & 0xfu) + 1u;
    }
    for (;;) {
        int snext, mk = 0;
        if (MC) {
            if (!mc_next(L, mq, snext, mk)) break;
        } else {
            snext = next_solve(L, pass);
            if (snext < 0) break;
        }
        const unsigned solve = (unsigned)snext;
        if (L.solve_clock && lane == 0) L.solve_clock[2 * (size_t)solve] = __builtin_amdgcn_s_memrealtime();
        const int model = (int)solve / L.nstat, station = (int)solve - model * L.nstat;
        const size_t slot = L.slot_per_solve ? solve : blockIdx.x;
        float *u = reinterpret_cast<float *>(L.u) + slot * L.field_elems;
        float *u0 = reinterpret_cast<float *>(L.u0) + (size_t)blockIdx.x * L.field_elems;
        const size_t ncell = (size_t)L.ncx * L.ncy * L.ncz;
        const int phase = L.model_phase ? (MC ? mcmcd::ldv(L.model_phase + model) : L.model_phase[model])
                                        : fsm_plain_phase(L, model);
        if (L.skip && L.skip[phase * L.nstat + station]) {
            skip_solve<float>(L, solve);
            if (MC) mc_finish(L, (int)solve, mk);
            __builtin_amdgcn_s_waitcnt(0);
            __builtin_amdgcn_fence(__ATOMIC_SEQ_CST, "workgroup");
            continue;
        }
        const size_t sentry = !L.model_phase ? (size_t)model : (size_t)model * L.nphase + phase;
        const void *slow_model = reinterpret_cast<const float *>(L.slow) + sentry * ncell;
        const Rsrc ur = make_rsrc(u, fbytes), u0r = make_rsrc(u0, fbytes),
                   sr = make_rsrc(slow_model, (uint32_t)(ncell * 4));
        const size_t zfb = zf_bytes(L, 4);
        const Rsrc zfr = make_rsrc(reinterpret_cast<char *>(L.zf) + (size_t)blockIdx.x * zfb, (uint32_t)zfb);
        if (lane == 0) { S.scratch[0] = 0; S.scratch[1] = 0; S.scratch[2] = 0; S.scratch[3] = 0; }
#ifdef MCEIK_TRAFFIC
        if (lane == 0)
            for (int k = 0; k < MCEIK_TRAFFIC_N; k++) S.scratch[8 + k] = 0;
#endif
        unsigned nchg = 0, nsteps = 0;
        BcBoxes bc;
        bc.box = S.box;
        const bool ok = init_field<float, 1>(L, u, ur, slow_model, L.src + (size_t)station * L.nsrc * 4, bc);
        hold_solve_start(L, hold_lds16(S), bc, g.nr);
        zf_init<float>(L, zfr, u, bc);
        asm volatile("" ::: "memory");
        int iters = 0, ierr_last = 0;
        if (ok) {
            int sweeps_left = L.max_sweeps < 0 ? 0x7fffffff : L.max_sweeps;
            for (int it = 0; it < L.maxit && sweeps_left > 0; it++) {
                bool notconv = false;
                hold_iter_start(L, hold_lds16(S));
                int clock = 64;
                for (int sw = 0; sw < 8 && sweeps_left > 0; sw++, sweeps_left--) {
                    const int rx = sw & 1, ry = (sw >> 1) & 1;
                    if (sw & 4)
                        clock += g.infl + sweep16<true, KB16, CCR>(L, g, ur, u0r, sr, zfr, bc, S, rx, ry, clock, notconv,
                                                              ierr_last, nchg, nsteps);
                    else
                        clock += g.infl + sweep16<false, KB16, CCR>(L, g, ur, u0r, sr, zfr, bc, S, rx, ry, clock, notconv,
                                                               ierr_last, nchg, nsteps);
                    __builtin_amdgcn_s_waitcnt(0);
                    __builtin_amdgcn_fence(__ATOMIC_SEQ_CST, "workgroup");
                    TRAF_FLUSH(L, S);
                }
                iters = it + 1;
                if (sweeps_left > 0 || L.max_sweeps < 0) {
                    if (!__any(notconv)) verify16(L, ur, u0r, S, notconv);
                    if (!__any(notconv)) break;
                }
            }
        }
        int ierr = ierr_last;
        for (int o = 32; o > 0; o >>= 1) ierr = max(ierr, __shfl_xor(ierr, o, 64));
        if (!ok) ierr = 1;
        if (L.visit_stats) {
            for (int o = 32; o > 0; o >>= 1) nchg += __shfl_xor(nchg, o, 64);
            asm volatile("" ::: "memory");
            if (lane == 0) {
                atomicAdd(L.visit_stats, (unsigned long long)(unsigned)S.scratch[0]);
                atomicAdd(L.visit_stats + 1, (unsigned long long)(unsigned)S.scratch[1]);
                atomicAdd(L.visit_stats + 2, (unsigned long long)nchg);
                atomicAdd(L.visit_stats + 3, (unsigned long long)nsteps);
            }
        }
        if (lane == 0) {
            if (L.solve_clock) L.solve_clock[2 * (size_t)solve + 1] = __builtin_amdgcn_s_memrealtime();
            if (L.iter_total) atomicAdd(L.iter_total, (unsigned long long)iters);
            if (L.solve_count) atomicAdd(L.solve_count, 1ull);
            if (L.niter) L.niter[solve] = iters;
            if (L.ierr) L.ierr[solve] = ierr;
        }
        TRAFU(S, 7, (unsigned)(L.field_elems * 4) + (L.ttab ? (unsigned)L.nev * (4u + 64u) : 0u));
        TRAF_FLUSH(L, S);
        if (L.ttab) {
            for (int e = lane; e < L.nev; e += 64) L.ttab[(size_t)solve * L.nev + e] = event_time<float>(L, u, e);
        }
        if (MC) mc_finish(L, (int)solve, mk);
        __builtin_amdgcn_s_waitcnt(0);
        __builtin_amdgcn_fence(__ATOMIC_SEQ_CST, "workgroup");
    }
}

#define FSM16_WPE __attribute__((amdgpu_waves_per_eu(2, 2)))
template <int KB16, int CCR, bool MC>
__global__ __launch_bounds__(64) FSM16_WPE void fsm16_solve_kernel(FsmLaunch L)
{
    fsm16_body<KB16, CCR, MC>(L);
}

}

hipError_t fsm16_launch(const FsmLaunch &L, int nwaves, hipStream_t st)
{
    if (!fsm16_eligible(L, 4)) return hipErrorInvalidValue;
    const size_t lds = fsm16_lds_bytes(L);
    const bool mc = L.mc_dev != nullptr;
    if (fsm16_fixed_layout(L)) {
        if (mc) hipLaunchKernelGGL((fsm16_solve_kernel<2, 1, true>), dim3(nwaves), dim3(64), lds, st, L);
        else hipLaunchKernelGGL((fsm16_solve_kernel<2, 1, false>), dim3(nwaves), dim3(64), lds, st, L);
    } else if (L.ccb <= 64) {
        if (mc) hipLaunchKernelGGL((fsm16_solve_kernel<0, 1, true>), dim3(nwaves), dim3(64), lds, st, L);
        else hipLaunchKernelGGL((fsm16_solve_kernel<0, 1, false>), dim3(nwaves), dim3(64), lds, st, L);
    } else {
        if (mc) hipLaunchKernelGGL((fsm16_solve_kernel<0, 4, true>), dim3(nwaves), dim3(64), lds, st, L);
        else hipLaunchKernelGGL((fsm16_solve_kernel<0, 4, false>), dim3(nwaves), dim3(64), lds, st, L);
    }
    return hipGetLastError();
}

int fsm16_occupancy(const FsmLaunch &L)
{
    int nb = 0;
    const size_t lds = fsm16_lds_bytes(L);
    hipError_t e;
    if (fsm16_fixed_layout(L))
        e = hipOccupancyMaxActiveBlocksPerMultiprocessor(&nb, fsm16_solve_kernel<2, 1, false>, 64, lds);
    else if (L.ccb <= 64)
        e = hipOccupancyMaxActiveBlocksPerMultiprocessor(&nb, fsm16_solve_kernel<0, 1, false>, 64, lds);
    else
        e = hipOccupancyMaxActiveBlocksPerMultiprocessor(&nb, fsm16_solve_kernel<0, 4, false>, 64, lds);
    return e == hipSuccess ? nb : 1;
}
```

### mceik_amd/csrc/fsm_common.h

```cpp
#pragma once
#include <stddef.h>
#include <stdint.h>
#include <hip/hip_runtime.h>

#define MCEIK_TILE 8
#define MCEIK_BRICK 512
#define MCEIK_KB 4
#define MCEIK_MAX_BLOCKS 1024
#define MCEIK_AHEAD 2

struct FsmLaunch {
    int nx, ny, nz;
    int ntx, nty, nzb, ntiles;
    int kb, nzk, nblocks, nr;
    int infl, vis;
    int ccb;
    int maxit, max_sweeps;
    double tol, h, x0, y0, z0;
    double conv_thresh;
    int nsolve, nstat, nsrc;
    const double *src;
    int slow_mode;
    const void *slow;
    int ncx, ncy, ncz, nrx, nry, nrz;
    unsigned magic_rx, magic_ry, magic_rz;
    int nzq;
    size_t field_elems;
    void *u;
    void *u0;
    void *zf;
    int slot_per_solve;
    const int *ev_node;
    int nev;
    float *ttab;
    int *niter;
    int *ierr;
    int cell_cache;
    int fast_sqrt;
    unsigned *counter;
    unsigned long long *iter_total;
    unsigned long long *visit_stats;
    const int *solve_order;
    unsigned long long *solve_clock;
    int max_waves;
    unsigned long long *traffic;
    int step_z;
    const float *ev_frac;
    const int *model_phase;
    int nphase;
    const unsigned char *skip;
    unsigned long long *solve_count;
    const void *mc_dev;
    unsigned *mc_sync;
    unsigned mc_spin_limit;
    int mc_step0, mc_nsteps;
    int mc_nburn, mc_keepk, mc_maxs, mc_nkept0;
};
#define MC_SYNC_WORDS(nchains) (8 + 8 * 32 + 2 * (nchains) + 1)

static inline __host__ __device__ int fsm_plain_phase(const FsmLaunch &L, int m)
{
    return L.nphase > 1 ? m % L.nphase : 0;
}

static inline __host__ __device__ size_t fsm_slow_entry(const FsmLaunch &L, int m)
{
    return L.model_phase ? (size_t)m * L.nphase + L.model_phase[m] : (size_t)m;
}

static inline __host__ __device__ int mceik_div_up(int a, int b) { return (a + b - 1) / b; }
static inline __host__ __device__ size_t zf_bytes(const FsmLaunch &L, size_t es) { return (size_t)L.nblocks * 128 * es; }

#if defined(MCEIK_TRAFFIC)
#define MCEIK_SCRATCH_BYTES 64
#else
#define MCEIK_SCRATCH_BYTES 32
#endif
#define MCEIK_TRAFFIC_N 8

#define MCEIK_CC_MAX 256
#define MCEIK_F64_HOLD (2 * 64 * 16)
#define MCEIK_SMEM_ARRAYS 14
#define MCEIK_XROWS 80
static inline __host__ __device__ size_t mceik_align16(size_t v) { return (v + 15) & ~(size_t)15; }
#define FSMF_NR (2 + (16 + MCEIK_KB - 1) / MCEIK_KB)
#define FSMF_CINFO 0
#define FSMF_XR (FSMF_CINFO + FSMF_NR * 64 * 8)
#define FSMF_XN (FSMF_XR + 2 * MCEIK_XROWS * 16)
#define FSMF_CC (FSMF_XN + 2 * MCEIK_XROWS * 16)
#define FSMF_RING (FSMF_CC + FSMF_NR * 64 * 4)
#define FSMF_SCRATCH (FSMF_RING + 64)
#define FSMF_LASTPROC (FSMF_SCRATCH + MCEIK_SCRATCH_BYTES)
#define FSMF_LASTCHG (FSMF_LASTPROC + MCEIK_MAX_BLOCKS * 4)
#define FSMF_ORDER (FSMF_LASTCHG + MCEIK_MAX_BLOCKS * 4)
static inline __host__ __device__ bool fsm_fixed_layout(const FsmLaunch &L, size_t es)
{
    return es == 4 && L.slow_mode != 0 && L.cell_cache && L.fast_sqrt && L.nrz == 4 && L.ccb <= 64 &&
           L.kb == MCEIK_KB && L.nr == FSMF_NR && L.nblocks <= MCEIK_MAX_BLOCKS;
}
static inline __host__ __device__ bool fsm_compact_layout(const FsmLaunch &L, size_t es)
{
    return es == 8 && L.slow_mode != 0 && L.cell_cache && L.nrz == 4 && L.ccb <= 64 && L.kb == MCEIK_KB &&
           L.nblocks <= MCEIK_MAX_BLOCKS;
}
static inline __host__ __device__ size_t fsm_smem_layout(const FsmLaunch &L, size_t es, size_t *off)
{
    if (fsm_fixed_layout(L, es)) {
        off[11] = FSMF_CINFO; off[9] = FSMF_XR; off[10] = FSMF_XN; off[1] = FSMF_CC;
        off[6] = FSMF_RING; off[7] = FSMF_SCRATCH; off[3] = FSMF_LASTPROC; off[4] = FSMF_LASTCHG;
        off[5] = FSMF_ORDER; off[2] = FSMF_ORDER; off[8] = FSMF_ORDER;
        off[0] = FSMF_ORDER + mceik_align16((size_t)L.ntiles * 4);
        off[12] = off[13] = off[0];
        return off[0] + mceik_align16((size_t)(L.nsrc > 0 ? L.nsrc : 1) * 6 * 4);
    }
    const bool cached = L.slow_mode != 0 && L.cell_cache;
    const size_t nt = (size_t)L.ntiles, nb = (size_t)L.nblocks, nr = (size_t)L.nr;
    size_t o = 0;
    off[0] = o; o += mceik_align16((size_t)(L.nsrc > 0 ? L.nsrc : 1) * 6 * 4);
    off[1] = o; o += cached ? mceik_align16(nr * L.ccb * 4) : 0;
    const bool cmp = fsm_compact_layout(L, es);
    off[2] = o; o += mceik_align16(nt * 4);
    off[3] = o; o += mceik_align16(nb * (cmp ? 2 : 4));
    off[4] = o; o += mceik_align16(nb * (cmp ? 2 : 4));
    off[5] = o;
    off[6] = o; o += mceik_align16(nr * (cmp ? 16 : 8));
    off[12] = o; o += cmp ? mceik_align16(nt) : 0;
    off[13] = o; o += cmp ? mceik_align16((nb + 31) / 32 * 4 * 2) : 0;
    off[7] = o; o += MCEIK_SCRATCH_BYTES;
    off[8] = o; o += cached ? 0 : 512 * es;
    off[9] = o; o += 2 * MCEIK_XROWS * 4 * es;
    off[10] = o; o += 2 * MCEIK_XROWS * 4 * es + (es == 8 ? MCEIK_F64_HOLD : 0);
    off[11] = o; o += nr * 64 * (cmp ? 4 : 8);
    return o;
}
static inline size_t fsm_lds_bytes(const FsmLaunch &L, size_t es)
{
    size_t off[MCEIK_SMEM_ARRAYS];
    return fsm_smem_layout(L, es, off);
}
#define MCEIK_MAX_LDS (64 * 1024)

#define MCEIK_AHEAD16 2
struct Fsm16Geo {
    int nzb, kb, nr, infl, vis;
};
static inline __host__ __device__ Fsm16Geo fsm16_geo(const FsmLaunch &L)
{
    Fsm16Geo g;
    g.nzb = mceik_div_up(L.nz, 16);
    g.kb = L.kb / 2;
    g.infl = 1 + mceik_div_up(14 + MCEIK_AHEAD16, g.kb);
    g.vis = mceik_div_up(12, g.kb);
    g.nr = 1 + mceik_div_up(15 + MCEIK_AHEAD16, g.kb);
    return g;
}
static inline __host__ __device__ bool fsm16_eligible(const FsmLaunch &L, size_t es)
{
    return es == 4 && L.slow_mode != 0 && L.cell_cache && L.fast_sqrt && L.nrz == 4 && L.ccb <= MCEIK_CC_MAX &&
           L.kb >= 4 && (L.kb & 1) == 0 && L.nblocks <= MCEIK_MAX_BLOCKS && L.ntx <= 256 && L.nty <= 256;
}
#define MCEIK_SMEM16_ARRAYS 11
#define MCEIK_X16PAD 4
#define MCEIK_X16Q (MCEIK_XROWS * 4 + MCEIK_X16PAD)
#define F16_NR (1 + (15 + MCEIK_AHEAD16 + 1) / 2)
#define F16_CINFO 0
#define F16_XR (F16_CINFO + F16_NR * 64 * 4)
#define F16_CC (F16_XR + 2 * 4 * MCEIK_X16Q * 4)
#define F16_RING (F16_CC + F16_NR * 32 * 4)
#define F16_SCRATCH (F16_RING + 176)
#define F16_LASTPROC (F16_SCRATCH + MCEIK_SCRATCH_BYTES)
#define F16_LASTCHG (F16_LASTPROC + MCEIK_MAX_BLOCKS * 2)
#define F16_ORDER (F16_LASTCHG + MCEIK_MAX_BLOCKS * 2)
static inline __host__ __device__ bool fsm16_fixed_layout(const FsmLaunch &L)
{
    return fsm16_eligible(L, 4) && L.kb == 4 && L.ccb <= 32 && fsm16_geo(L).nr == F16_NR;
}
static inline __host__ __device__ size_t f16_bitmap_bytes(const FsmLaunch &L)
{
    return mceik_align16((size_t)((L.nblocks + 31) / 32) * 4 * 2);
}
static inline __host__ __device__ size_t fsm16_smem_layout(const FsmLaunch &L, size_t *off)
{
    const size_t nbox = mceik_align16((size_t)(L.nsrc > 0 ? L.nsrc : 1) * 6 * 4);
    if (fsm16_fixed_layout(L)) {
        off[8] = F16_CINFO; off[7] = F16_XR; off[1] = F16_CC; off[5] = F16_RING; off[6] = F16_SCRATCH;
        off[3] = F16_LASTPROC; off[4] = F16_LASTCHG; off[2] = F16_ORDER;
        off[9] = F16_ORDER + mceik_align16((size_t)L.ntiles * 2);
        off[10] = off[9] + mceik_align16((size_t)L.ntiles);
        off[0] = off[10] + f16_bitmap_bytes(L);
        return off[0] + nbox;
    }
    const Fsm16Geo g = fsm16_geo(L);
    const size_t nr = (size_t)g.nr, nb = (size_t)L.nblocks;
    size_t o = 0;
    off[0] = o; o += nbox;
    off[1] = o; o += mceik_align16(nr * L.ccb * 4);
    off[2] = o; o += mceik_align16((size_t)L.ntiles * 2);
    off[3] = o; o += mceik_align16(nb * 2);
    off[4] = o; o += mceik_align16(nb * 2);
    off[9] = o; o += mceik_align16((size_t)L.ntiles);
    off[10] = o; o += f16_bitmap_bytes(L);
    off[5] = o; o += mceik_align16(nr * 16);
    off[6] = o; o += MCEIK_SCRATCH_BYTES;
    off[7] = o; o += 2 * 4 * MCEIK_X16Q * 4;
    off[8] = o; o += nr * 64 * 4;
    return o;
}
static inline size_t fsm16_lds_bytes(const FsmLaunch &L)
{
    size_t off[MCEIK_SMEM16_ARRAYS];
    return fsm16_smem_layout(L, off);
}

static inline __host__ __device__ constexpr int hold_clock_bound(int nblocks, int infl)
{
    return nblocks * (1 + infl) + 64;
}
static_assert(hold_clock_bound(MCEIK_MAX_BLOCKS, 1 + (14 + MCEIK_AHEAD16 + 1) / 2) < 65536,
              "16-bit held-stream clocks: MCEIK_MAX_BLOCKS / MCEIK_AHEAD16 too large");
static_assert(hold_clock_bound(MCEIK_MAX_BLOCKS, 1 + (14 + MCEIK_AHEAD + MCEIK_KB - 1) / MCEIK_KB) < 65536,
              "16-bit held-stream clocks: MCEIK_MAX_BLOCKS / MCEIK_AHEAD too large");

static inline void fsm_geometry(FsmLaunch *L, int es)
{
    L->ntx = mceik_div_up(L->nx, MCEIK_TILE);
    L->nty = mceik_div_up(L->ny, MCEIK_TILE);
    L->nzb = mceik_div_up(L->nz, MCEIK_TILE);
    L->ntiles = L->ntx * L->nty;
    int kb = L->nzb < MCEIK_KB ? L->nzb : MCEIK_KB;
    while (kb < L->nzb && ((long)L->ntiles * mceik_div_up(L->nzb, kb) > MCEIK_MAX_BLOCKS || mceik_div_up(L->nzb, kb) > 128))
        kb *= 2;
    if (kb > L->nzb) kb = L->nzb;
    L->kb = kb;
    L->nzk = mceik_div_up(L->nzb, kb);
    L->nblocks = L->ntiles * L->nzk;
    L->infl = 1 + mceik_div_up(14 + MCEIK_AHEAD, kb);
    L->vis = mceik_div_up(12, kb);
    L->nr = 2 + mceik_div_up(16, kb);
    const int bpl = 16 / es;
    L->nzq = mceik_div_up(L->nzb, bpl);
    L->field_elems = (size_t)L->ntiles * L->nzq * 64 * (128 / es);
}
```

### mceik_amd/csrc/fsm_device.h

```cpp
#pragma once
#include <hip/hip_runtime.h>
#include <float.h>
#include <stdint.h>

#include "fsm_common.h"
#include "fsm_update.h"

namespace {

#define OOB 0x80000000u
typedef __amdgpu_buffer_rsrc_t Rsrc;

__device__ __forceinline__ Rsrc make_rsrc(const void *p, uint32_t bytes)
{
    return __builtin_amdgcn_make_buffer_rsrc(const_cast<void *>(p), 0, bytes, 0x00020000);
}

typedef float f4v __attribute__((ext_vector_type(4)));
typedef double d2v __attribute__((ext_vector_type(2)));
typedef unsigned u4v __attribute__((ext_vector_type(4)));
typedef unsigned u2v __attribute__((ext_vector_type(2)));

__device__ __forceinline__ void bload8(Rsrc r, uint32_t off, float (&v)[8])
{
    f4v a = __builtin_bit_cast(f4v, __builtin_amdgcn_raw_buffer_load_b128(r, off, 0, 0));
    f4v b = __builtin_bit_cast(f4v, __builtin_amdgcn_raw_buffer_load_b128(r, off + 16, 0, 0));
    v[0] = a.x; v[1] = a.y; v[2] = a.z; v[3] = a.w; v[4] = b.x; v[5] = b.y; v[6] = b.z; v[7] = b.w;
}
__device__ __forceinline__ void bstore8(Rsrc r, uint32_t off, const float (&v)[8])
{
    f4v a = {v[0], v[1], v[2], v[3]}, b = {v[4], v[5], v[6], v[7]};
    __builtin_amdgcn_raw_buffer_store_b128(__builtin_bit_cast(u4v, a), r, off, 0, 0);
    __builtin_amdgcn_raw_buffer_store_b128(__builtin_bit_cast(u4v, b), r, off + 16, 0, 0);
}
__device__ __forceinline__ void bload8(Rsrc r, uint32_t off, double (&v)[8])
{
#pragma unroll
    for (int k = 0; k < 4; k++) {
        d2v a = __builtin_bit_cast(d2v, __builtin_amdgcn_raw_buffer_load_b128(r, off + 16 * k, 0, 0));
        v[2 * k] = a.x; v[2 * k + 1] = a.y;
    }
}
__device__ __forceinline__ void bstore8(Rsrc r, uint32_t off, const double (&v)[8])
{
#pragma unroll
    for (int k = 0; k < 4; k++) {
        d2v a = {v[2 * k], v[2 * k + 1]};
        __builtin_amdgcn_raw_buffer_store_b128(__builtin_bit_cast(u4v, a), r, off + 16 * k, 0, 0);
    }
}
__device__ __forceinline__ void bstore4(Rsrc r, uint32_t off, float a0, float a1, float a2, float a3)
{
    f4v a = {a0, a1, a2, a3};
    __builtin_amdgcn_raw_buffer_store_b128(__builtin_bit_cast(u4v, a), r, off, 0, 0);
}
__device__ __forceinline__ float bload1f(Rsrc r, uint32_t off)
{
    return __builtin_bit_cast(float, __builtin_amdgcn_raw_buffer_load_b32(r, off, 0, 0));
}

__host__ __device__ __forceinline__ int colpos(int lx, int ly)
{
    if (ly == 0) return lx;
    if (ly == 7) return 8 + lx;
    if (lx == 0) return 15 + ly;
    if (lx == 7) return 21 + ly;
    return 28 + (ly - 1) * 6 + (lx - 1);
}
__host__ __device__ __forceinline__ void colpos_inv(int p, int &lx, int &ly)
{
    if (p < 8) { lx = p; ly = 0; }
    else if (p < 16) { lx = p - 8; ly = 7; }
    else if (p < 22) { lx = 0; ly = p - 15; }
    else if (p < 28) { lx = 7; ly = p - 21; }
    else { lx = 1 + (p - 28) % 6; ly = 1 + (p - 28) / 6; }
}

template <typename R> struct Lay {
    static constexpr int ZQ = 128 / (int)sizeof(R);
    static constexpr int BPL = ZQ / 8;
};
template <typename R>
__device__ __forceinline__ uint32_t zoff_bytes(int zb)
{
    constexpr int LB = Lay<R>::BPL == 4 ? 2 : 1, LS = sizeof(R) == 4 ? 5 : 6;
    const uint32_t u = (uint32_t)zb;
    return ((u >> LB) << 13) | ((u & (uint32_t)(Lay<R>::BPL - 1)) << LS);
}
template <typename R>
__device__ __forceinline__ uint32_t tile_bytes(const FsmLaunch &L) { return (uint32_t)L.nzq * 8192u; }

template <typename R>
__device__ __forceinline__ size_t brick_index(const FsmLaunch &L, int x, int y, int z)
{
    constexpr int ZQ = Lay<R>::ZQ;
    const int tile = (y >> 3) * L.ntx + (x >> 3);
    return (((size_t)tile * L.nzq + z / ZQ) * 64 + colpos(x & 7, y & 7)) * ZQ + z % ZQ;
}

template <typename R>
__device__ __forceinline__ float event_time(const FsmLaunch &L, const R *u, int e)
{
    const int node = L.ev_node[e];
    const int nxy = L.nx * L.ny;
    const int z = node / nxy, rem = node - z * nxy, y = rem / L.nx, x = rem - y * L.nx;
    if (!L.ev_frac) return (float)u[brick_index<R>(L, x, y, z)];
    const float wx = L.ev_frac[3 * e], wy = L.ev_frac[3 * e + 1], wz = L.ev_frac[3 * e + 2];
    const int x1 = min(x + 1, L.nx - 1), y1 = min(y + 1, L.ny - 1), z1 = min(z + 1, L.nz - 1);
    float c[8];
#pragma unroll
    for (int k = 0; k < 8; k++)
        c[k] = (float)u[brick_index<R>(L, (k & 1) ? x1 : x, (k & 2) ? y1 : y, (k & 4) ? z1 : z)];
    float a[4];
#pragma unroll
    for (int k = 0; k < 4; k++) a[k] = __fadd_rn(c[2 * k], __fmul_rn(wx, __fsub_rn(c[2 * k + 1], c[2 * k])));
    const float b0 = __fadd_rn(a[0], __fmul_rn(wy, __fsub_rn(a[1], a[0])));
    const float b1 = __fadd_rn(a[2], __fmul_rn(wy, __fsub_rn(a[3], a[2])));
    return __fadd_rn(b0, __fmul_rn(wz, __fsub_rn(b1, b0)));
}

template <typename R>
__device__ __forceinline__ void skip_solve(const FsmLaunch &L, unsigned solve)
{
    const int lane = threadIdx.x;
    if (lane == 0) {
        if (L.solve_clock) {
            const unsigned long long t = __builtin_amdgcn_s_memrealtime();
            L.solve_clock[2 * (size_t)solve] = t;
            L.solve_clock[2 * (size_t)solve + 1] = t;
        }
        if (L.niter) L.niter[solve] = 0;
        if (L.ierr) L.ierr[solve] = 0;
    }
    if (L.ttab)
        for (int e = lane; e < L.nev; e += 64) L.ttab[(size_t)solve * L.nev + e] = FLT_MAX;
}

struct BcBoxes {
    int n;
    int *box;
};

#ifdef MCEIK_TRAFFIC
#define TRAF(S, k, pred, bytes)                                                                         \
    do {                                                                                                \
        const unsigned n_ = (unsigned)__builtin_popcountll(__ballot(pred));                             \
        if (threadIdx.x == 0) (S).scratch[8 + (k)] += (int)(n_ * (unsigned)(bytes));                     \
    } while (0)
#define TRAFU(S, k, bytes)                                                                              \
    do {                                                                                                \
        if (threadIdx.x == 0) (S).scratch[8 + (k)] += (int)(bytes);                                     \
    } while (0)
#endif
#ifdef MCEIK_TRAFFIC
#define TRAF_FLUSH(L, S)                                                                                \
    do {                                                                                                \
        asm volatile("" ::: "memory");                                                                  \
        if (threadIdx.x == 0 && (L).traffic)                                                            \
            for (int k_ = 0; k_ < MCEIK_TRAFFIC_N; k_++) {                                              \
                atomicAdd((L).traffic + k_, (unsigned long long)(unsigned)(S).scratch[8 + k_]);         \
                (S).scratch[8 + k_] = 0;                                                                \
            }                                                                                           \
        asm volatile("" ::: "memory");                                                                  \
    } while (0)
#else
#define TRAF(S, k, pred, bytes) do { } while (0)
#define TRAFU(S, k, bytes) do { } while (0)
#define TRAF_FLUSH(L, S) do { } while (0)
#endif

__device__ __forceinline__ void tile_cells(int t, int n, unsigned magic, int &c0, int &nc)
{
    const int a = t * 8, b = min(t * 8 + 7, n - 1);
    c0 = (int)(((unsigned)a * magic) >> 20);
    nc = (int)(((unsigned)b * magic) >> 20) - c0 + 1;
}
__device__ __forceinline__ void block_zcells(const FsmLaunch &L, int kb, int tz, int &cz0, int &ncz)
{
    const int a = tz * kb * 8, b = min(a + kb * 8, L.nz) - 1;
    cz0 = (int)(((unsigned)a * L.magic_rz) >> 20);
    ncz = (int)(((unsigned)b * L.magic_rz) >> 20) - cz0 + 1;
}

__device__ __forceinline__ void bload4(Rsrc r, uint32_t off, float (&v)[4])
{
    f4v a = __builtin_bit_cast(f4v, __builtin_amdgcn_raw_buffer_load_b128(r, off, 0, 0));
    v[0] = a.x; v[1] = a.y; v[2] = a.z; v[3] = a.w;
}
__device__ __forceinline__ void bload4(Rsrc r, uint32_t off, double (&v)[4])
{
    d2v a = __builtin_bit_cast(d2v, __builtin_amdgcn_raw_buffer_load_b128(r, off, 0, 0));
    d2v b = __builtin_bit_cast(d2v, __builtin_amdgcn_raw_buffer_load_b128(r, off + 16, 0, 0));
    v[0] = a.x; v[1] = a.y; v[2] = b.x; v[3] = b.y;
}
__device__ __forceinline__ void bstore1(Rsrc r, uint32_t off, float v)
{
    __builtin_amdgcn_raw_buffer_store_b32(__builtin_bit_cast(unsigned, v), r, off, 0, 0);
}
__device__ __forceinline__ void bstore1(Rsrc r, uint32_t off, double v)
{
    __builtin_amdgcn_raw_buffer_store_b64(__builtin_bit_cast(u2v, v), r, off, 0, 0);
}
__device__ __forceinline__ float bload1(Rsrc r, uint32_t off, float)
{
    return __builtin_bit_cast(float, __builtin_amdgcn_raw_buffer_load_b32(r, off, 0, 0));
}
__device__ __forceinline__ double bload1(Rsrc r, uint32_t off, double)
{
    return __builtin_bit_cast(double, __builtin_amdgcn_raw_buffer_load_b64(r, off, 0, 0));
}

template <typename R, int SLOWMODE>
__device__ __forceinline__ double slow_at(const FsmLaunch &L, const void *slow_model, int x, int y, int z)
{
    if (SLOWMODE == 0)
        return (double)reinterpret_cast<const R *>(slow_model)[brick_index<R>(L, x, y, z)];
    const float *si = reinterpret_cast<const float *>(slow_model);
    asm volatile("" : "+v"(si));
    return (double)si[((size_t)(z / L.nrz) * L.ncy + y / L.nry) * L.ncx + x / L.nrx];
}

__device__ __forceinline__ int wave_max(int v)
{
#pragma unroll
    for (int o = 32; o > 0; o >>= 1) v = max(v, __shfl_xor(v, o, 64));
    return v;
}

template <bool FAST>
__device__ __forceinline__ float godunov_v(float a, float b, float c, float f, float ff, float ff2, float ff3)
{
    const unsigned ia = __builtin_bit_cast(unsigned, a), ib = __builtin_bit_cast(unsigned, b),
                   ic = __builtin_bit_cast(unsigned, c);
    unsigned u1, u2, u3;
    asm("v_min3_u32 %0, %1, %2, %3" : "=v"(u1) : "v"(ia), "v"(ib), "v"(ic));
    asm("v_med3_u32 %0, %1, %2, %3" : "=v"(u2) : "v"(ia), "v"(ib), "v"(ic));
    asm("v_max3_u32 %0, %1, %2, %3" : "=v"(u3) : "v"(ia), "v"(ib), "v"(ic));
    const float a1 = __builtin_bit_cast(float, u1), a2 = __builtin_bit_cast(float, u2),
                a3 = __builtin_bit_cast(float, u3);
    const float d2 = a2 - a1, d3 = a3 - a1;
    const float e = d3 - d2;
    const float d22 = d2 * d2, d33 = d3 * d3;
    const float t = d33 + e * e;
    const bool two = t >= ff;
    const float r2 = ff2 - d22;
    const float sm = d2 + d3;
    const float disc = ff3 - (d22 + t);
    const float rad = two ? r2 : disc;
    const float s = FAST ? sqrt_normal(rad) : __builtin_sqrtf(rad);
    const float y23 = ((two ? d2 : sm) + s) * (two ? 0.5f : (1.0f / 3.0f));
    const float y = !(f > d2) ? f : y23;
    const unsigned ix = __builtin_bit_cast(unsigned, a1 + y);
    return __builtin_bit_cast(float, __builtin_elementwise_min(ix, 0x7f7fffffu));
}
template <bool FAST>
__device__ __forceinline__ double godunov_v(double a, double b, double c, double f, double, double, double)
{
    return godunov_fast64<FAST>(a, b, c, f);
}

template <typename R, int SLOWMODE>
__device__ __forceinline__ bool init_field(const FsmLaunch &L, R *u, Rsrc ur, const void *slow_model, const double *src,
                           BcBoxes &bc)
{
    const int lane = threadIdx.x;
    const R UN = Num<R>::unan();
    const uint32_t nvec = (uint32_t)(L.field_elems / 8);
    R fill[8];
#pragma unroll
    for (int i = 0; i < 8; i++) fill[i] = UN;
    for (uint32_t i = lane; i < nvec; i += 64) bstore8(ur, i * 8u * (uint32_t)sizeof(R), fill);
    __builtin_amdgcn_s_waitcnt(0);
    __builtin_amdgcn_fence(__ATOMIC_SEQ_CST, "workgroup");
    bc.n = L.nsrc;
    bool ok = true;
    for (int s = 0; s < L.nsrc; s++) {
        const double *sp = src + (size_t)s * 4;
        const double ts = sp[0];
        int loc[3][3];
        const int nn[3] = {L.nx, L.ny, L.nz};
        const double org[3] = {L.x0, L.y0, L.z0};
        for (int a = 0; a < 3; a++) {
            double xs = sp[1 + a], x0 = org[a], dx = L.h;
            int n = nn[a], is;
            if (xs <= x0) is = 1;
            else if (xs >= x0 + (double)(n - 1) * dx) is = n;
            else is = (int)((xs - x0) / dx + 0.5) + 1;
            int np = 0;
            loc[a][0] = loc[a][1] = loc[a][2] = -1;
            double xe = x0 + (double)(is - 1) * dx;
            if (xe > xs) { loc[a][0] = is - 1; loc[a][1] = is; np = 2; }
            else if (xe < xs) { loc[a][0] = is; loc[a][1] = is + 1; np = 2; }
            else {
                loc[a][np++] = is - 1;
                loc[a][np++] = is;
                if (is < n - 1) loc[a][np++] = is + 1;
            }
            for (int i = 0; i < np; i++) if (loc[a][i] < 1 || loc[a][i] > n) ok = false;
            int lo = 1 << 30, hi = -1;
            for (int i = 0; i < np; i++) { lo = min(lo, loc[a][i] - 1); hi = max(hi, loc[a][i] - 1); }
            if (lane == 0) { bc.box[6 * s + 2 * a] = lo; bc.box[6 * s + 2 * a + 1] = hi; }
        }
        if (!ok) { bc.n = s; break; }
        if (lane < 27) {
            int i = lane % 3, j = (lane / 3) % 3, k = lane / 9;
            int ix = loc[0][i], iy = loc[1][j], iz = loc[2][k];
            if (ix != -1 && iy != -1 && iz != -1) {
                double x = L.x0 + (double)(ix - 1) * L.h, y = L.y0 + (double)(iy - 1) * L.h,
                       z = L.z0 + (double)(iz - 1) * L.h;
                double ddx = sp[1] - x, ddy = sp[2] - y, ddz = sp[3] - z;
                double dd = __builtin_sqrt((ddx * ddx + ddy * ddy) + ddz * ddz);
                double sl = slow_at<R, SLOWMODE>(L, slow_model, ix - 1, iy - 1, iz - 1);
                R t = (R)(ts + dd * sl);
                size_t idx = brick_index<R>(L, ix - 1, iy - 1, iz - 1);
                R cur = u[idx];
                u[idx] = (__builtin_fabs(dd) < 1.e-10) ? t : (cur < t ? cur : t);
            }
        }
        __builtin_amdgcn_s_waitcnt(0);
        __builtin_amdgcn_fence(__ATOMIC_SEQ_CST, "workgroup");
    }
    __builtin_amdgcn_fence(__ATOMIC_SEQ_CST, "workgroup");
    return ok;
}

__device__ __forceinline__ int next_solve(const FsmLaunch &L, int &pass)
{
    const int g0 = blockIdx.x & 7;
    while (pass < 8) {
        const int g = (g0 + pass) & 7;
        const int lo = (int)((long long)L.nsolve * g / 8), hi = (int)((long long)L.nsolve * (g + 1) / 8);
        unsigned i = 0;
        if (threadIdx.x == 0) i = atomicAdd(L.counter + 32 * g, 1u);
        i = __builtin_amdgcn_readfirstlane(__shfl(i, 0, 64));
        if ((int)i < hi - lo) return L.solve_order ? L.solve_order[lo + (int)i] : lo + (int)i;
        pass++;
    }
    return -1;
}

__device__ __forceinline__ void build_order(const FsmLaunch &L, int *order)
{
    for (int id = threadIdx.x; id < L.ntiles; id += 64) {
        const int txs = id % L.ntx, tys = id / L.ntx, dg = txs + tys;
        int rank = 0;
        for (int e = 0; e < dg; e++)
            rank += min(e, L.nty - 1) - max(0, e - L.ntx + 1) + 1;
        rank += tys - max(0, dg - L.ntx + 1);
        order[rank] = txs | (tys << 16);
    }
}

struct Pos {
    int vb, sp, zbs, ri;
};
__device__ __forceinline__ void pos_init(Pos &p, int vb, int kb, int nr)
{
    p.vb = vb;
    const int v = vb < 0 ? 0 : vb;
    p.sp = v / kb; p.zbs = v - p.sp * kb;
    p.ri = p.sp % nr;
}
__device__ __forceinline__ void pos_adv(Pos &p, int kb, int nr)
{
    const int z1 = p.zbs + (p.vb >= 0 ? 1 : 0);
    const bool wrap = z1 == kb;
    const int r1 = p.ri + (wrap ? 1 : 0);
    p.zbs = wrap ? 0 : z1;
    p.sp += wrap ? 1 : 0;
    p.ri = r1 == nr ? 0 : r1;
    p.vb++;
}
__device__ __forceinline__ bool pos_valid(const Pos &p, int nstream)
{
    return p.vb >= 0 && p.sp < nstream;
}

enum {
    C_ACT = 1,
    C_U0 = 2,
    C_PART = 4,
    C_00 = 8,
    C_BC = 16,
    C_BLK = 32,
    C_ZH = 64,
    C_XOWN = 128,
    C_YOWN = 256,
    F_VALID = 128, F_FIRST = 256, F_LAST = 512, F_SLOW = 1024, F_ZH = 2048
};
__device__ __forceinline__ int ci_tz(unsigned w) { return (int)((w >> 9) & 0x7f); }
__device__ __forceinline__ int ci_ccb(unsigned w) { return (int)w >> 16; }

struct ColTile {
    int tile;
    uint32_t col;
    int fl, cl;
};
template <typename R>
__device__ __forceinline__ void column_tile(const FsmLaunch &L, const BcBoxes &bc, int entry, int lx, int ly,
                                            int lxs, int lys, int rx, int ry, ColTile &t)
{
    const int tx = entry & 0xfff, ty = (entry >> 12) & 0xfff;
    const int x = tx * 8 + lx, y = ty * 8 + ly;
    const uint32_t st = tile_bytes<R>(L);
    const uint32_t col = (uint32_t)(ty * L.ntx + tx) * st + (uint32_t)colpos(lx, ly) * 128u;
    int m = (x < L.nx && y < L.ny) ? C_ACT : 0;
    if (lxs == 0 || lxs == 7) {
        const int xn = x + (((lxs == 0) != (rx != 0)) ? -1 : 1);
        if (!(xn >= 0 && xn < L.nx)) m |= C_XOWN;
    }
    if (lys == 0 || lys == 7) {
        const int yn = y + (((lys == 0) != (ry != 0)) ? -1 : 1);
        if (!(yn >= 0 && yn < L.ny)) m |= C_YOWN;
    }
    if (tx * 8 + 8 > L.nx || ty * 8 + 8 > L.ny) m |= C_PART;
    if (x == 0 && y == 0) m |= C_00;
    for (int k = 0; k < bc.n; k++) {
        const int *q = bc.box + 6 * k;
        if (x >= q[0] && x <= q[1] && y >= q[2] && y <= q[3]) m |= C_BC;
    }
    int cx0, ncxt, cy0, ncyt;
    tile_cells(tx, L.nx, L.magic_rx, cx0, ncxt);
    tile_cells(ty, L.ny, L.magic_ry, cy0, ncyt);
    const int xc = x < L.nx ? x : L.nx - 1, yc = y < L.ny ? y : L.ny - 1;
    const int cxl = (int)(((unsigned)xc * L.magic_rx) >> 20) - cx0;
    const int cyl = (int)(((unsigned)yc * L.magic_ry) >> 20) - cy0;
    t.tile = entry & 0xffffff;
    t.col = col;
    t.fl = m;
    t.cl = cyl * ncxt + cxl;
}
__device__ __forceinline__ unsigned column_word(const FsmLaunch &L, int kb, const ColTile &t, int tz, int ri,
                                                int u0flag, int zh)
{
    int cz0, nczb;
    block_zcells(L, kb, tz, cz0, nczb);
    const int ccb = ri * L.ccb + t.cl * nczb - cz0;
    const int m = t.fl | C_BLK | (u0flag ? C_U0 : 0) | (zh ? C_ZH : 0);
    return (unsigned)(m | (tz << 9) | (ccb << 16));
}

__device__ __forceinline__ int halo_edge_lane(int j)
{
    return j < 8 ? j * 8 : j < 16 ? (j - 8) * 8 + 7 : j < 24 ? j - 16 : 56 + (j - 24);
}
__device__ __forceinline__ uint32_t halo_delta(const FsmLaunch &L, uint32_t tile_bytes, int j, int he, int rx, int ry)
{
    const int lxs = he & 7, lys = he >> 3;
    const int lx = rx ? 7 - lxs : lxs, ly = ry ? 7 - lys : lys;
    if (j < 16) {
        const int dx = ((j < 8) != (rx != 0)) ? -1 : 1;
        return (uint32_t)(dx * (int)tile_bytes) + (uint32_t)((colpos((lx + dx) & 7, ly) - colpos(lx, ly)) * 128);
    }
    const int dy = ((j < 24) != (ry != 0)) ? -1 : 1;
    return (uint32_t)(dy * L.ntx * (int)tile_bytes) + (uint32_t)((colpos(lx, (ly + dy) & 7) - colpos(lx, ly)) * 128);
}
__device__ __forceinline__ unsigned dpp_swap_pair(unsigned v)
{
    return (unsigned)__builtin_amdgcn_mov_dpp((int)v, 0xB1, 0xf, 0xf, false);
}
template <int CCR>
__device__ __forceinline__ void cc_issue(const FsmLaunch &L, int kb, Rsrc sr, int entry, float (&v)[CCR], int &size)
{
    const int lane = threadIdx.x;
    const int tx = entry & 0xfff, ty = (entry >> 12) & 0xfff, tz = (entry >> 24) & 0xff;
    int cx0, ncxt, cy0, ncyt, cz0, nczb;
    tile_cells(tx, L.nx, L.magic_rx, cx0, ncxt);
    tile_cells(ty, L.ny, L.magic_ry, cy0, ncyt);
    block_zcells(L, kb, tz, cz0, nczb);
    size = entry >= 0 ? ncxt * ncyt * nczb : 0;
    const float rz = __builtin_amdgcn_rcpf((float)nczb), rx = __builtin_amdgcn_rcpf((float)ncxt);
#pragma unroll
    for (int r = 0; r < CCR; r++) {
        const int idx = lane + 64 * r;
        const int t = (int)(((float)idx + 0.5f) * rz), cz = idx - t * nczb;
        const int cyl = (int)(((float)t + 0.5f) * rx), cxl = t - cyl * ncxt;
        const uint32_t off = (uint32_t)((((cz0 + cz) * L.ncy + cy0 + cyl) * L.ncx) + cx0 + cxl) * 4u;
        v[r] = bload1f(sr, idx < size ? off : OOB);
    }
}
template <typename R, int CCR>
__device__ __forceinline__ void cc_write(const FsmLaunch &L, float *cc, int ri, const float (&v)[CCR], int size,
                                         float h)
{
    const int lane = threadIdx.x;
#pragma unroll
    for (int r = 0; r < CCR; r++) {
        const int idx = lane + 64 * r;
        if (idx < size) cc[ri * L.ccb + idx] = sizeof(R) == 4 ? v[r] * h : v[r];
    }
}

struct Stream {
    int cursor, tile, k, k0, wait;
};

}
```

### mceik_amd/csrc/fsm_hold.h

```cpp
#pragma once
#include <hip/hip_runtime.h>

#include "fsm_common.h"
#include "fsm_device.h"

#define HOLD_OWN 1u
#define HOLD_ZLO 32u
#define HOLD_ZHI 64u
#define HOLD_CONT 256u

namespace {

template <typename OrderT>
struct HoldLds {
    const OrderT *order;
    unsigned char *fz;
    unsigned short *lastproc;
    unsigned short *need;
    unsigned *fmask;
    const int *ring_e;
    unsigned *vbits, *cbits;
};
enum { HOLD_DONE = 0, HOLD_BLOCKED, HOLD_HELD, HOLD_WAIT, HOLD_SKIP, HOLD_READY };

// ... 22 lines not shown
    u0 = !((vw >> (b & 31)) & 1u);
    runon = 0;
    if (k >= nzk) return HOLD_DONE;
    if ((xu >= 0 && fxu <= k) || (yu >= 0 && fyu <= k)) return HOLD_BLOCKED;
    const bool reason = nb >= lb;
    int dep = -0x40000000;
    if (xu >= 0) dep = max(dep, lxu);
    if (yu >= 0) dep = max(dep, lyu);
    const int zl = k > 0 ? lzl : -0x40000000;
    runon = zl == C - 1;
    if (!runon) dep = max(dep, zl);
    if (reason) return dep + vis <= C ? HOLD_READY : HOLD_WAIT;
    return (runon || dep > C - infl) ? HOLD_HELD : HOLD_SKIP;
}
struct HoldSt {
    int done, last, lc;
};
__device__ __forceinline__ HoldSt hold_state(const int *sst)
{
    asm volatile("" ::: "memory");
    return HoldSt{sst[0], sst[1], sst[2]};
}
template <bool RZ, typename OrderT>
__device__ __forceinline__ int hold_decide(const FsmLaunch &L, const HoldLds<OrderT> &H, int *sst, const HoldSt &sr,
                                           int C, int rx, int ry, int rprev, int infl, int vis, int &zh, int &u0)
{
    const int lane = threadIdx.x, nt = L.ntiles, nzk = L.nzk;
    const int dxu = rx ? 1 : -1, dyu = ry ? L.ntx : -L.ntx;
    zh = 0;
    u0 = 0;
    int pick = -1, pid = 0, pk = 0, pro = 0, pfl = 0, pu0 = 0;
    int done = __builtin_amdgcn_readfirstlane(sr.done);
    const int last = __builtin_amdgcn_readfirstlane(sr.last), lc = __builtin_amdgcn_readfirstlane(sr.lc);
    if (last >= 0) {
        const int id = lc & 0xffff, k = (lc >> 16) & 0xff, fl = (lc >> 24) & 3;
        int ro, v0;
        const int s = hold_status<RZ>(L, H, id, (fl & 1) ? id + dxu : -1, (fl & 2) ? id + dyu : -1, k, C, infl, vis,
                                      ro, v0);
        if (__builtin_amdgcn_readfirstlane(s) == HOLD_READY) {
            pick = last;
            pid = id;
            pk = k;
            pro = __builtin_amdgcn_readfirstlane(ro);
            pu0 = __builtin_amdgcn_readfirstlane(v0);
            pfl = fl;
        }
    }
    if (pick < 0) {
        int wbase = -1, ti = 0, id = 0, xu = -1, yu = -1, k = 255;
        auto window = [&](int base) __attribute__((always_inline)) {
            wbase = base;
            ti = base + lane;
            const bool in = ti < nt;
            int txs, tys;
            hold_txy(H, in ? ti : 0, txs, tys);
            const int tx = rx ? L.ntx - 1 - txs : txs, ty = ry ? L.nty - 1 - tys : tys;
            id = ty * L.ntx + tx;
            xu = txs > 0 ? id + dxu : -1;
            yu = tys > 0 ? id + dyu : -1;
            const int f = H.fz[id];
            k = in ? f : 255;
        };
        for (;;) {
            window(done);
            const unsigned long long m = ~__ballot(ti < nt && k >= nzk);
            const int n = m ? __builtin_ctzll(m) : 64;
            done += n;
            if (n < 64) break;
        }
        if (done >= nt) {
            asm volatile("" ::: "memory");
            if (lane == 0) { sst[0] = done; sst[1] = -1; }
            asm volatile("" ::: "memory");
            return -2;
        }
        for (int base = done; base < nt && pick < 0; base += 64) {
            if (base != wbase) window(base);
            for (;;) {
#ifdef MCEIK_PHASECLK
                if (lane == 0) sst[4 + 7] += 1;
#endif
                int ro, v0;
                const int s0 = hold_status<RZ>(L, H, id, xu, yu, k, C, infl, vis, ro, v0);
                const int s = ti < nt ? s0 : HOLD_DONE;
                const bool sk = s == HOLD_SKIP;
                if (sk) H.fz[id] = (unsigned char)(k + 1);
                const unsigned long long rm = __ballot(s == HOLD_READY);
                if (rm) {
                    const int f = __builtin_ctzll(rm);
                    pick = base + f;
                    pid = __builtin_amdgcn_readfirstlane(__shfl(id, f, 64));
                    pk = __builtin_amdgcn_readfirstlane(__shfl(k, f, 64));
                    pro = __builtin_amdgcn_readfirstlane(__shfl(ro, f, 64));
                    pu0 = __builtin_amdgcn_readfirstlane(__shfl(v0, f, 64));
                    pfl = __builtin_amdgcn_readfirstlane(__shfl((xu >= 0 ? 1 : 0) | (yu >= 0 ? 2 : 0), f, 64));
                    break;
                }
                if (!__ballot(sk)) break;
                k += sk ? 1 : 0;
                asm volatile("" ::: "memory");
            }
        }
    }
    asm volatile("" ::: "memory");
    if (pick < 0) {
        if (lane == 0) { sst[0] = done; sst[1] = -1; }
        asm volatile("" ::: "memory");
        return -1;
    }
    if (lane == 0) {
        H.fz[pid] = (unsigned char)(pk + 1);
        if (pro) atomicOr(&H.fmask[rprev], HOLD_CONT);
        sst[0] = done;
        sst[1] = pick;
        sst[2] = pid | ((pk + 1) << 16) | (pfl << 24);
    }
    asm volatile("" ::: "memory");
    zh = pk > 0 && !pro;
    u0 = pu0;
    const int ty = pid / L.ntx, tx = pid - ty * L.ntx;
    return tx | (ty << 12) | ((RZ ? L.nzk - 1 - pk : pk) << 24);
}
template <typename OrderT>
__device__ __forceinline__ int hold_tile_id(const FsmLaunch &L, const HoldLds<OrderT> &H, int ti, int rx, int ry)
{
    int txs, tys;
    hold_txy(H, ti, txs, tys);
    return (ry ? L.nty - 1 - tys : tys) * L.ntx + (rx ? L.ntx - 1 - txs : txs);
}
template <bool RZ, typename OrderT>
__device__ __forceinline__ int hold_status_scan(const FsmLaunch &L, const HoldLds<OrderT> &H, int ti, int C, int rx, int ry,
                                           int infl, int vis, int &id, int &k, int &runon)
{
    int txs, tys;
    hold_txy(H, ti, txs, tys);
    const int tx = rx ? L.ntx - 1 - txs : txs, ty = ry ? L.nty - 1 - tys : tys;
    const int nt = L.ntiles, nzk = L.nzk;
    id = ty * L.ntx + tx;
    k = H.fz[id];
    runon = 0;
    if (k >= nzk) return HOLD_DONE;
    const int xu = txs > 0 ? id + (rx ? 1 : -1) : -1;
    const int yu = tys > 0 ? id + (ry ? L.ntx : -L.ntx) : -1;
    if ((xu >= 0 && (int)H.fz[xu] <= k) || (yu >= 0 && (int)H.fz[yu] <= k)) return HOLD_BLOCKED;
    const int tz = RZ ? nzk - 1 - k : k;
    const int b = tz * nt + id;
    const bool reason = H.need[b] >= H.lastproc[b];
    int dep = -0x40000000;
    if (xu >= 0) dep = max(dep, (int)H.lastproc[tz * nt + xu]);
    if (yu >= 0) dep = max(dep, (int)H.lastproc[tz * nt + yu]);
    const int zl = k > 0 ? (int)H.lastproc[b + (RZ ? nt : -nt)] : -0x40000000;
    runon = zl == C - 1;
    if (!runon) dep = max(dep, zl);
    if (reason) return dep + vis <= C ? HOLD_READY : HOLD_WAIT;
    return (runon || dep > C - infl) ? HOLD_HELD : HOLD_SKIP;
}
template <bool RZ, typename OrderT>
__device__ __forceinline__ int hold_decide_scan(const FsmLaunch &L, const HoldLds<OrderT> &H, int *sst, int C, int rx,
                                           int ry, int rprev, int infl, int vis, int &zh)
{
    const int lane = threadIdx.x, nt = L.ntiles;
    zh = 0;
    int pick = -1, pid = 0, pk = 0, pro = 0;
    asm volatile("" ::: "memory");
    struct { int done, last; } st = {__builtin_amdgcn_readfirstlane(sst[0]), __builtin_amdgcn_readfirstlane(sst[1])};
    if (st.last >= 0) {
        int id, k, ro;
        const int s = hold_status_scan<RZ>(L, H, st.last, C, rx, ry, infl, vis, id, k, ro);
        if (__builtin_amdgcn_readfirstlane(s) == HOLD_READY) {
            pick = st.last;
            pid = __builtin_amdgcn_readfirstlane(id);
            pk = __builtin_amdgcn_readfirstlane(k);
            pro = __builtin_amdgcn_readfirstlane(ro);
        }
    }
    if (pick < 0) {
        for (;;) {
            const int ti = st.done + lane;
            const bool cpl = ti < nt && (int)H.fz[hold_tile_id(L, H, ti, rx, ry)] >= L.nzk;
            const unsigned long long m = ~__ballot(cpl);
            const int n = m ? __builtin_ctzll(m) : 64;
            st.done += n;
            if (n < 64) break;
        }
        if (st.done >= nt) {
            asm volatile("" ::: "memory");
            if (lane == 0) { sst[0] = st.done; sst[1] = -1; }
            asm volatile("" ::: "memory");
            return -2;
        }
        for (int base = st.done; base < nt && pick < 0; base += 64) {
            const int ti = base + lane;
            for (;;) {
                int s = HOLD_DONE, id = 0, k = 0, ro = 0;
                if (ti < nt) s = hold_status_scan<RZ>(L, H, ti, C, rx, ry, infl, vis, id, k, ro);
                const bool sk = s == HOLD_SKIP;
                if (sk) H.fz[id] = (unsigned char)(k + 1);
                const unsigned long long rm = __ballot(s == HOLD_READY);
                if (rm) {
                    const int f = __builtin_ctzll(rm);
                    pick = base + f;
                    pid = __builtin_amdgcn_readfirstlane(__shfl(id, f, 64));
                    pk = __builtin_amdgcn_readfirstlane(__shfl(k, f, 64));
                    pro = __builtin_amdgcn_readfirstlane(__shfl(ro, f, 64));
                    break;
                }
                if (!__ballot(sk)) break;
                asm volatile("" ::: "memory");
            }
        }
    }
    asm volatile("" ::: "memory");
    if (pick < 0) {
        if (lane == 0) { sst[0] = st.done; sst[1] = -1; }
        asm volatile("" ::: "memory");
        return -1;
    }
    if (lane == 0) {
        H.fz[pid] = (unsigned char)(pk + 1);
        if (pro) atomicOr(&H.fmask[rprev], HOLD_CONT);
        sst[0] = st.done;
        sst[1] = pick;
    }
    asm volatile("" ::: "memory");
    zh = pk > 0 && !pro;
    const int ty = pid / L.ntx, tx = pid - ty * L.ntx;
    return tx | (ty << 12) | ((RZ ? L.nzk - 1 - pk : pk) << 24);
}
template <typename OrderT>
__device__ __forceinline__ void hold_settle(const FsmLaunch &L, const HoldLds<OrderT> &H, int ri, int clk)
{
    const int lane = threadIdx.x;
    asm volatile("" ::: "memory");
    const int e = H.ring_e[ri];
    const unsigned m = H.fmask[ri];
    if (e >= 0 && lane < 7 && ((m >> lane) & 1u)) {
        const int tx = e & 0xfff, ty = (e >> 12) & 0xfff, tz = (e >> 24) & 0xff;
        const int nt = L.ntiles, b = tz * nt + ty * L.ntx + tx;
        const int t = lane == 0 ? b
                    : lane == 1 ? (tx > 0 ? b - 1 : -1)
                    : lane == 2 ? (tx < L.ntx - 1 ? b + 1 : -1)
                    : lane == 3 ? (ty > 0 ? b - L.ntx : -1)
                    : lane == 4 ? (ty < L.nty - 1 ? b + L.ntx : -1)
                    : lane == 5 ? (tz > 0 ? b - nt : -1)
                    : (tz < L.nzk - 1 ? b + nt : -1);
        if (t >= 0) H.need[t] = (unsigned short)clk;
        if (lane == 0) H.cbits[b >> 5] |= 1u << (b & 31);
    }
    asm volatile("" ::: "memory");
    if (lane == 0) H.fmask[ri] = 0;
    asm volatile("" ::: "memory");
}
template <typename OrderT>
__device__ __forceinline__ void hold_norm(const FsmLaunch &L, const HoldLds<OrderT> &H)
{
    asm volatile("" ::: "memory");
    for (int b = threadIdx.x; b < L.nblocks; b += 64) {
        const bool pend = H.need[b] >= H.lastproc[b];
        H.lastproc[b] = 1;
        H.need[b] = pend ? 1 : 0;
    }
    for (int t = threadIdx.x; t < L.ntiles; t += 64) H.fz[t] = 0;
    asm volatile("" ::: "memory");
}
template <typename OrderT>
__device__ __forceinline__ void hold_iter_start(const FsmLaunch &L, const HoldLds<OrderT> &H)
{
    for (int w = threadIdx.x; w < (L.nblocks + 31) / 32; w += 64) {
        H.vbits[w] = 0;
        H.cbits[w] = 0;
    }
    asm volatile("" ::: "memory");
}
template <typename OrderT>
__device__ __forceinline__ void hold_solve_start(const FsmLaunch &L, const HoldLds<OrderT> &H, const BcBoxes &bc, int nr)
{
    const int lane = threadIdx.x;
    for (int t = lane; t < L.nblocks; t += 64) {
        H.lastproc[t] = 2;
        H.need[t] = 1;
    }
    if (lane < nr) H.fmask[lane] = 0;
    asm volatile("" ::: "memory");
    if (lane == 0) {
        for (int k = 0; k < bc.n; k++) {
            const int *q = bc.box + 6 * k;
            for (int tz = q[4] / (8 * L.kb); tz <= q[5] / (8 * L.kb); tz++)
                for (int ty = q[2] >> 3; ty <= q[3] >> 3; ty++)
                    for (int tx = q[0] >> 3; tx <= q[1] >> 3; tx++) {
                        const int b = (tz * L.nty + ty) * L.ntx + tx;
                        H.need[b] = 3;
                        if (tx > 0) H.need[b - 1] = 3;
                        if (tx < L.ntx - 1) H.need[b + 1] = 3;
                        if (ty > 0) H.need[b - L.ntx] = 3;
                        if (ty < L.nty - 1) H.need[b + L.ntx] = 3;
                        if (tz > 0) H.need[b - L.ntiles] = 3;
                        if (tz < L.nzk - 1) H.need[b + L.ntiles] = 3;
                    }
        }
    }
    asm volatile("" ::: "memory");
}

template <typename R>
__device__ __forceinline__ uint32_t zf_off(int b, int side, int lx, int ly)
{
    return ((uint32_t)(b * 2 + side) * 64u + (uint32_t)(lx + 8 * ly)) * (uint32_t)sizeof(R);
}
template <typename R, bool RZ>
__device__ __forceinline__ uint32_t zf_boundary(const FsmLaunch &L, int b, bool zd, int lx, int ly)
{
    const bool up = zd != RZ;
    return zf_off<R>(b + (up ? L.ntiles : -L.ntiles), up ? 0 : 1, lx, ly);
}
template <typename R>
__device__ __forceinline__ void zf_init(const FsmLaunch &L, Rsrc zfr, const R *u, const BcBoxes &bc)
{
    const int lane = threadIdx.x;
    const R UN = Num<R>::unan();
    R fill[8];
#pragma unroll
    for (int i = 0; i < 8; i++) fill[i] = UN;
    const uint32_t nvec = (uint32_t)(zf_bytes(L, sizeof(R)) / (8 * sizeof(R)));
    for (uint32_t i = lane; i < nvec; i += 64) bstore8(zfr, i * 8u * (uint32_t)sizeof(R), fill);
    __builtin_amdgcn_s_waitcnt(0);
    const int zbk = 8 * L.kb;
    for (int s = 0; s < bc.n; s++) {
        const int *q = bc.box + 6 * s;
        const int x = q[0] + lane % 3, y = q[2] + (lane / 3) % 3, z = q[4] + lane / 9;
        if (lane < 27 && x <= q[1] && y <= q[3] && z <= q[5]) {
            const int zr = z % zbk;
            if (zr == 0 || zr == zbk - 1) {
                const int b = ((z / zbk) * L.nty + (y >> 3)) * L.ntx + (x >> 3);
                bstore1(zfr, zf_off<R>(b, zr == 0 ? 0 : 1, x & 7, y & 7), u[brick_index<R>(L, x, y, z)]);
            }
        }
    }
    __builtin_amdgcn_s_waitcnt(0);
    __builtin_amdgcn_fence(__ATOMIC_SEQ_CST, "workgroup");
}

}
```

### mceik_amd/csrc/fsm_kernel.hip

```cpp
#include <hip/hip_runtime.h>
#include <float.h>
#include <stdint.h>
#include <stdlib.h>

#include <type_traits>

#include "fsm_common.h"
#include "fsm_device.h"
#include "fsm_hold.h"
#include "fsm_update.h"


namespace {


template <typename R, bool CMP = false>
struct Smem {
    using clk_t = typename std::conditional<CMP, unsigned short, int>::type;
    int *box;
    float *cc;
    int *order;
    clk_t *lastproc, *lastchg;
    int *ring;
    int *scratch;
// ... 706 lines not shown
            } else if (ccfill) {
                cc_write<R, CCR>(L, S.cc, ccri, ccv, ccsize, (float)L.h);
            }
        } else {
#pragma unroll
            for (int i = 0; i < 8; i++) S.sf[i * 64 + lane] = fq[i] * hr;
        }
        store4(S.xr + hso, hq);
        R nn[8];
        if (PAIR) {
            pair_finish(qa, qb, reinterpret_cast<float (&)[8]>(nn));
        } else {
#pragma unroll
            for (int i = 0; i < 8; i++) {
                if (!FL64) nn[i] = q[i];
            }
        }
        auto u0_store = [&]() __attribute__((always_inline)) {
            if (__any(b0.fl & C_U0) && !__any(notconv)) {
                R m = fmin_(fmin_(fmin_(c[0], c[1]), fmin_(c[2], c[3])), fmin_(fmin_(c[4], c[5]), fmin_(c[6], c[7])));
                const bool st0 = m < (R)L.conv_thresh && (b0.fl & C_U0);
                if (__any(st0)) bstore8(u0r, st0 ? b0.seg : OOB, c);
                TRAF(S, 4, st0, 8 * sizeof(R));
            }
        };
        constexpr bool LAZYN = sizeof(R) == 8;
        if (LAZYN) u0_store();
        store_row(S.xr, 0, lane, r);
        if (LAZYN) load_row(S.xr, xrow<R>(1, lane), c);
        if (FL64)
            line_write64(reinterpret_cast<double *>(S.xr), rowl, rowo, la, lh);
        else
            store_row(S.xr, 1, lane, nn);
#pragma unroll
        for (int i = 0; i < 4; i++) hq[i] = hn[i];
        zc = zn; zn = zq;
#pragma unroll
        for (int i = 0; i < 8; i++) {
            if (!FL64) asm volatile("" : "+v"(nn[i]));
        }
        if (FL64) {
#pragma unroll
            for (int i = 0; i < 4; i++) asm volatile("" : "+v"(la[i]), "+v"(lh[i]));
        }
        asm volatile("" : "+v"(hq[0]), "+v"(hq[1]), "+v"(hq[2]), "+v"(hq[3]));
        asm volatile("" : "+v"(zn));
        asm volatile("" ::: "memory");

        if (__any(changed)) {
            if (PAIR)
                pair_store(ur, b0.seg, changed, reinterpret_cast<const float (&)[8]>(r));
            else
                bstore8(ur, changed ? b0.seg : OOB, r);
            TRAF(S, 3, changed, 8 * sizeof(R));
        }
        if (!LAZYN) u0_store();
        if constexpr (HOLD) {
            const int zr = (b0.zb8 >> 3) % kb;
            const bool zlo = changed && zr == 0 && c0, zhi = changed && zr == kb - 1 && c7;
            if (changed) atomicOr(&S.fmask[b0.ri], xyface | (zlo ? HOLD_ZLO : 0u) | (zhi ? HOLD_ZHI : 0u));
        } else if (changed) {
            S.lastchg[b0.bid] = (typename Smem<R, CMP>::clk_t)(clock0 + b0.clk);
        }
        asm volatile("" ::: "memory");
        if (!LAZYN) {
#pragma unroll
            for (int i = 0; i < 8; i++) {
                c[i] = n[i];
                n[i] = nn[i];
            }
        }
        b0 = b1;
        b1 = b3;
        if (++ph == kb) ph = 0;
        B++;
        decide_step();
        return more();
    };
    decide_step();
    if (more()) {
        do {
        } while (step(c, n, hq, hn));
    }
    __builtin_amdgcn_s_setprio(0);
    nsteps += (unsigned)B;
    if constexpr (HOLD) {
        const HoldLds<int> H = hold_lds(S);
        for (int q = max(0, nstream - L.infl + 1); q < nstream; q++) hold_settle(L, H, q % nr, clock0 + q);
    }
    return nstream;
}

template <typename R, bool CMP>
__device__ __forceinline__ void verify_small(const FsmLaunch &L, Rsrc ur, Rsrc u0r, const Smem<R, CMP> &S, int clock_it, bool &notconv)
{
    const int lane = threadIdx.x, lx = lane & 7, ly = lane >> 3;
    const R T = (R)L.conv_thresh, tolr = (R)L.tol;
    for (int base = 0; base < L.nblocks; base += 64) {
        const int k = base + lane;
        const bool flag = k < L.nblocks && (CMP ? ((S.cbits[k >> 5] >> (k & 31)) & 1u) != 0
                                                 : S.lastchg[k] >= clock_it);
        unsigned long long m = __ballot(flag);
        while (m) {
            const int bid = base + __builtin_ctzll(m);
            m &= m - 1;
            const int tz = bid / L.ntiles, id = bid - tz * L.ntiles;
            const int tx = id % L.ntx, ty = id / L.ntx;
            const int x = tx * 8 + lx, y = ty * 8 + ly;
            const int zend = min(tz * L.kb + L.kb, L.nzb);
            for (int zb = tz * L.kb; zb < zend; zb++) {
                const uint32_t seg = (uint32_t)id * tile_bytes<R>(L) + zoff_bytes<R>(zb) + (uint32_t)colpos(lx, ly) * 128u;
                R u[8], v0[8];
                bload8(ur, seg, u);
                bload8(u0r, seg, v0);
                TRAF(S, 6, x < L.nx && y < L.ny, 16 * sizeof(R));
#pragma unroll
                for (int i = 0; i < 8; i++) {
                    R dl = v0[i] - u[i];
                    dl = dl < (R)0 ? -dl : dl;
                    if (x < L.nx && y < L.ny && zb * 8 + i < L.nz && u[i] < T && !(dl < tolr)) notconv = true;
                }
            }
            if (__any(notconv)) return;
        }
    }
}

#define FSM_WPE __attribute__((amdgpu_waves_per_eu(sizeof(R) == 8 ? 2 : 1)))
template <typename R, int SLOWMODE, bool FAST, int ZSH, int CCR, int KB>
__global__ __launch_bounds__(64) FSM_WPE void fsm_solve_kernel(FsmLaunch L)
{
    extern __shared__ __attribute__((aligned(16))) unsigned char smem[];
    constexpr bool CMP = sizeof(R) == 8 && KB > 0;
    const Smem<R, CMP> S = smem_bind<R, KB == MCEIK_KB && sizeof(R) == 4 && SLOWMODE == 2, CMP>(L, smem);
    const int lane = threadIdx.x;
    const uint32_t fbytes = (uint32_t)(L.field_elems * sizeof(R));
    build_order(L, S.order);
    int pass = 0;
    for (;;) {
        const int snext = next_solve(L, pass);
        if (snext < 0) break;
        const unsigned solve = (unsigned)snext;
        if (L.solve_clock && lane == 0) L.solve_clock[2 * (size_t)solve] = __builtin_amdgcn_s_memrealtime();
        const int model = (int)solve / L.nstat, station = (int)solve - model * L.nstat;
        if (L.skip && L.skip[(L.model_phase && SLOWMODE != 0 ? L.model_phase[model] : fsm_plain_phase(L, model)) *
                                 L.nstat + station]) {
            skip_solve<R>(L, solve);
            __builtin_amdgcn_s_waitcnt(0);
            __builtin_amdgcn_fence(__ATOMIC_SEQ_CST, "workgroup");
            continue;
        }
        const size_t slot = L.slot_per_solve ? solve : blockIdx.x;
        R *u = reinterpret_cast<R *>(L.u) + slot * L.field_elems;
        R *u0 = reinterpret_cast<R *>(L.u0) + (size_t)blockIdx.x * L.field_elems;
        const void *slow_model;
        uint32_t slow_bytes;
        if (SLOWMODE == 0) {
            slow_model = reinterpret_cast<const R *>(L.slow) + (size_t)model * L.field_elems;
            slow_bytes = fbytes;
        } else {
            const size_t ncell = (size_t)L.ncx * L.ncy * L.ncz;
            slow_model = reinterpret_cast<const float *>(L.slow) + fsm_slow_entry(L, model) * ncell;
            slow_bytes = (uint32_t)(ncell * 4);
        }
        const Rsrc ur = make_rsrc(u, fbytes), u0r = make_rsrc(u0, fbytes), sr = make_rsrc(slow_model, slow_bytes);
        constexpr bool HOLD = CMP;
        if (!HOLD) {
            for (int t = lane; t < L.nblocks; t += 64) {
                S.lastproc[t] = -2; S.lastchg[t] = -3;
            }
        }
        if (lane == 0) { S.scratch[0] = 0; S.scratch[1] = 0; S.scratch[2] = 0; S.scratch[3] = 0; }
#ifdef MCEIK_TRAFFIC
        if (lane == 0)
            for (int k = 0; k < MCEIK_TRAFFIC_N; k++) S.scratch[8 + k] = 0;
#endif
        unsigned nchg = 0, nsteps = 0;
        BcBoxes bc;
        bc.box = S.box;
        const bool ok = init_field<R, SLOWMODE>(L, u, ur, slow_model, L.src + (size_t)station * L.nsrc * 4, bc);
        if constexpr (HOLD) {
            hold_solve_start(L, hold_lds(S), bc, L.nr);
        } else if (lane == 0) {
            for (int k = 0; k < bc.n; k++) {
                const int *q = bc.box + 6 * k;
                for (int tz = q[4] / (8 * L.kb); tz <= q[5] / (8 * L.kb); tz++)
                    for (int ty = q[2] >> 3; ty <= q[3] >> 3; ty++)
                        for (int tx = q[0] >> 3; tx <= q[1] >> 3; tx++)
                            S.lastchg[(tz * L.nty + ty) * L.ntx + tx] = -1;
            }
        }
        asm volatile("" ::: "memory");
        int iters = 0, ierr_last = 0, clock = 64;
        if (ok) {
            int sweeps_left = L.max_sweeps < 0 ? 0x7fffffff : L.max_sweeps;
            for (int it = 0; it < L.maxit && sweeps_left > 0; it++) {
                bool notconv = false;
                if constexpr (HOLD) {
                    hold_iter_start(L, hold_lds(S));
                    clock = 64;
                }
                const int clock_it = clock;
                for (int sw = 0; sw < 8 && sweeps_left > 0; sw++, sweeps_left--) {
                    const int rx = sw & 1, ry = (sw >> 1) & 1;
#ifdef MCEIK_STEPSTATS
                    const int clock_sw = clock;
#endif
                    if (sw & 4)
                        clock += L.infl + sweep<R, SLOWMODE, FAST, true, ZSH, CCR, KB>(
                                              L, ur, u0r, sr, bc, S, rx, ry, clock_it, clock, notconv, ierr_last, nchg,
                                              nsteps);
                    else
                        clock += L.infl + sweep<R, SLOWMODE, FAST, false, ZSH, CCR, KB>(
                                              L, ur, u0r, sr, bc, S, rx, ry, clock_it, clock, notconv, ierr_last, nchg,
                                              nsteps);
#ifdef MCEIK_STEPSTATS
                    {
                        const int c1 = clock - L.infl;
                        unsigned nu = 0;
                        for (int t = lane; t < L.nblocks; t += 64) {
                            const int lp = S.lastproc[t];
                            nu += (lp >= c1 - 0x100000 && lp > 63 && lp >= clock_sw && S.lastchg[t] < lp) ? 1u : 0u;
                        }
                        for (int o = 32; o > 0; o >>= 1) nu += __shfl_xor(nu, o, 64);
                        if (lane == 0) S.scratch[3] += nu;
                    }
#endif
                    __builtin_amdgcn_s_waitcnt(0);
                    __builtin_amdgcn_fence(__ATOMIC_SEQ_CST, "workgroup");
                    TRAF_FLUSH(L, S);
                }
                iters = it + 1;
                if (sweeps_left > 0 || L.max_sweeps < 0) {
                    if (!__any(notconv)) verify_small<R>(L, ur, u0r, S, clock_it, notconv);
                    if (!__any(notconv)) break;
                }
            }
        }
        int ierr = ierr_last;
        for (int o = 32; o > 0; o >>= 1) ierr = max(ierr, __shfl_xor(ierr, o, 64));
        if (!ok) ierr = 1;
        if (L.visit_stats) {
            for (int o = 32; o > 0; o >>= 1) nchg += __shfl_xor(nchg, o, 64);
            asm volatile("" ::: "memory");
            if (lane == 0) {
                atomicAdd(L.visit_stats, (unsigned long long)(unsigned)S.scratch[0]);
#ifdef MCEIK_STEPSTATS
                atomicAdd(L.visit_stats + 1, (unsigned long long)(unsigned)S.scratch[2]);
                atomicAdd(L.visit_stats + 2, (unsigned long long)(unsigned)S.scratch[3]);
#else
                atomicAdd(L.visit_stats + 1, (unsigned long long)(unsigned)S.scratch[1]);
                atomicAdd(L.visit_stats + 2, (unsigned long long)nchg);
                atomicAdd(L.visit_stats + 3, (unsigned long long)nsteps);
#endif
            }
        }
        if (lane == 0) {
            if (L.solve_clock) L.solve_clock[2 * (size_t)solve + 1] = __builtin_amdgcn_s_memrealtime();
            if (L.iter_total) atomicAdd(L.iter_total, (unsigned long long)iters);
            if (L.solve_count) atomicAdd(L.solve_count, 1ull);
            if (L.niter) L.niter[solve] = iters;
            if (L.ierr) L.ierr[solve] = ierr;
        }
        TRAFU(S, 7, (unsigned)(L.field_elems * sizeof(R)) + (L.ttab ? (unsigned)L.nev * (4u + 64u) : 0u));
        TRAF_FLUSH(L, S);
        if (L.ttab) {
            for (int e = lane; e < L.nev; e += 64) L.ttab[(size_t)solve * L.nev + e] = event_time<R>(L, u, e);
        }
        __builtin_amdgcn_s_waitcnt(0);
        __builtin_amdgcn_fence(__ATOMIC_SEQ_CST, "workgroup");
    }
}

template <typename RS, typename RD>
__global__ void to_brick_kernel(const RS *src, RD *dst, FsmLaunch L, int nfield)
{
    size_t n = L.field_elems * (size_t)nfield;
    for (size_t i = blockIdx.x * (size_t)blockDim.x + threadIdx.x; i < n; i += (size_t)gridDim.x * blockDim.x) {
        size_t fld = i / L.field_elems, e = i - fld * L.field_elems;
        constexpr int ZQ = Lay<RD>::ZQ;
        const int zi = (int)(e % ZQ);
        size_t t = e / ZQ;
        const int col = (int)(t & 63); t >>= 6;
        const int zq = (int)(t % L.nzq); const int tile = (int)(t / L.nzq);
        int ty = tile / L.ntx, tx = tile - ty * L.ntx;
        int clx, cly;
        colpos_inv(col, clx, cly);
        int x = tx * 8 + clx, y = ty * 8 + cly, z = zq * ZQ + zi;
        RD v = 0;
        if (x < L.nx && y < L.ny && z < L.nz)
            v = (RD)src[fld * (size_t)L.nx * L.ny * L.nz + ((size_t)z * L.ny + y) * L.nx + x];
        dst[i] = v;
    }
}

template <typename RS, typename RD>
__global__ void from_brick_kernel(const RS *src, RD *dst, FsmLaunch L, int nfield)
{
    size_t nn = (size_t)L.nx * L.ny * L.nz, n = nn * nfield;
    for (size_t i = blockIdx.x * (size_t)blockDim.x + threadIdx.x; i < n; i += (size_t)gridDim.x * blockDim.x) {
        size_t fld = i / nn, e = i - fld * nn;
        int x = (int)(e % L.nx); size_t t = e / L.nx;
        int y = (int)(t % L.ny); int z = (int)(t / L.ny);
        dst[i] = (RD)src[fld * L.field_elems + brick_index<RS>(L, x, y, z)];
    }
}

}

template <typename R, int SLOWMODE, bool FAST, int ZSH, int CCR, int KB>
static hipError_t launch_fsm(const FsmLaunch &L, int nwaves, hipStream_t st)
{
    size_t lds = fsm_lds_bytes(L, sizeof(R));
    if (KB == MCEIK_KB && sizeof(R) == 4 && SLOWMODE == 2 && !fsm_fixed_layout(L, 4)) return hipErrorInvalidValue;
    hipLaunchKernelGGL((fsm_solve_kernel<R, SLOWMODE, FAST, ZSH, CCR, KB>), dim3(nwaves), dim3(64), lds, st, L);
    return hipGetLastError();
}

template <typename R, int SLOWMODE, bool FAST, int ZSH, int CCR, int KB>
static int occupancy_of(size_t lds)
{
    int nb = 0;
    return hipOccupancyMaxActiveBlocksPerMultiprocessor(&nb, fsm_solve_kernel<R, SLOWMODE, FAST, ZSH, CCR, KB>, 64,
                                                        lds) == hipSuccess ? nb : 1;
}

static int variant(const FsmLaunch &L, int is_double)
{
    const int mode = L.slow_mode == 0 ? 0 : (L.cell_cache ? 2 : 1);
    if (is_double) {
        const int v = 9 + mode * 2 + (mode == 2 && L.nrz == 4 && L.ccb <= 64 ? (fsm_compact_layout(L, 8) ? 2 : 1) : 0);
        return v == 15 && L.fast_sqrt ? 16 : v;
    }
    if (mode != 2) return mode * 2;
    return 4 + (L.fast_sqrt ? 1 : 0) + (L.nrz == 4 && L.fast_sqrt && L.ccb <= 64 ? (L.kb == MCEIK_KB ? 3 : 2) : 0);
}

#define FSM_VARIANTS(X)                         \
    X(0, float, 0, false, -1, 1, 0)             \
    X(2, float, 1, false, -1, 1, 0)             \
    X(4, float, 2, false, -1, 4, 0)             \
    X(5, float, 2, true, -1, 4, 0)              \
    X(7, float, 2, true, 2, 1, 0)               \
    X(8, float, 2, true, 2, 1, MCEIK_KB)        \
    X(9, double, 0, false, -1, 1, 0)            \
    X(11, double, 1, false, -1, 1, 0)           \
    X(13, double, 2, false, -1, 4, 0)           \
    X(14, double, 2, false, 2, 1, 0)            \
    X(15, double, 2, false, 2, 1, MCEIK_KB)     \
    X(16, double, 2, true, 2, 1, MCEIK_KB)

hipError_t fsm16_launch(const FsmLaunch &L, int nwaves, hipStream_t st);
int fsm16_occupancy(const FsmLaunch &L);
static bool use_fsm16(const FsmLaunch &L, int is_double)
{
    static const bool on = [] { const char *e = getenv("MCEIK_FSM16"); return !(e && e[0] == '0'); }();
    const int v = variant(L, is_double);
    return on && L.step_z != 8 && (v == 5 || v == 7 || v == 8) && fsm16_eligible(L, 4);
}
size_t fsm_launch_lds_bytes(const FsmLaunch &L, int is_double)
{
    return use_fsm16(L, is_double) ? fsm16_lds_bytes(L) : fsm_lds_bytes(L, is_double ? 8 : 4);
}
int fsm_launch_kind(const FsmLaunch &L, int is_double) { return use_fsm16(L, is_double) ? 16 : 8; }
const char *fsm_launch_name(const FsmLaunch &L, int is_double)
{
    if (use_fsm16(L, is_double))
        return fsm16_fixed_layout(L) ? "fsm16_solve_kernel<2, 1>" : L.ccb <= 64 ? "fsm16_solve_kernel<0, 1>"
                                                                                 : "fsm16_solve_kernel<0, 4>";
    switch (variant(L, is_double)) {
    case 0: return "fsm_solve_kernel<float, 0, false, -1, 1, 0>";
    case 2: return "fsm_solve_kernel<float, 1, false, -1, 1, 0>";
    case 4: return "fsm_solve_kernel<float, 2, false, -1, 4, 0>";
    case 5: return "fsm_solve_kernel<float, 2, true, -1, 4, 0>";
    case 7: return "fsm_solve_kernel<float, 2, true, 2, 1, 0>";
    case 8: return "fsm_solve_kernel<float, 2, true, 2, 1, 4>";
    case 9: return "fsm_solve_kernel<double, 0, false, -1, 1, 0>";
    case 11: return "fsm_solve_kernel<double, 1, false, -1, 1, 0>";
    case 13: return "fsm_solve_kernel<double, 2, false, -1, 4, 0>";
    case 14: return "fsm_solve_kernel<double, 2, false, 2, 1, 0>";
    case 15: return "fsm_solve_kernel<double, 2, false, 2, 1, 4>";
    case 16: return "fsm_solve_kernel<double, 2, true, 2, 1, 4>";
    }
    return "?";
}

__global__ void fsm_zero_words_kernel(unsigned *p, int n)
{
    for (int i = threadIdx.x; i < n; i += blockDim.x) p[i] = 0u;
}
hipError_t fsm_zero_words(unsigned *p, int n, hipStream_t st)
{
    hipLaunchKernelGGL(fsm_zero_words_kernel, dim3(1), dim3(256), 0, st, p, n);
    return hipGetLastError();
}

hipError_t fsm_launch(const FsmLaunch &L, int is_double, int nwaves, hipStream_t st)
{
    if (use_fsm16(L, is_double)) return fsm16_launch(L, nwaves, st);
    switch (variant(L, is_double)) {
#define X(v, R, M, F, Z, CR, K) case v: return launch_fsm<R, M, F, Z, CR, K>(L, nwaves, st);
        FSM_VARIANTS(X)
#undef X
    default: return hipErrorInvalidValue;
    }
}

int fsm_occupancy(const FsmLaunch &L, int is_double)
{
    if (use_fsm16(L, is_double)) return fsm16_occupancy(L);
    const size_t lds = fsm_lds_bytes(L, is_double ? 8 : 4);
    switch (variant(L, is_double)) {
#define X(v, R, M, F, Z, CR, K) case v: return occupancy_of<R, M, F, Z, CR, K>(lds);
        FSM_VARIANTS(X)
#undef X
    default: return 1;
    }
}

hipError_t fsm_to_brick_f64(const double *src, void *dst, int dst_double, const FsmLaunch &L, int nfield, hipStream_t st)
{
    if (dst_double) hipLaunchKernelGGL((to_brick_kernel<double, double>), dim3(1024), dim3(256), 0, st, src, (double *)dst, L, nfield);
    else hipLaunchKernelGGL((to_brick_kernel<double, float>), dim3(1024), dim3(256), 0, st, src, (float *)dst, L, nfield);
    return hipGetLastError();
}

hipError_t fsm_from_brick_f64(const void *src, int src_double, double *dst, const FsmLaunch &L, int nfield, hipStream_t st)
{
    if (src_double) hipLaunchKernelGGL((from_brick_kernel<double, double>), dim3(1024), dim3(256), 0, st, (const double *)src, dst, L, nfield);
    else hipLaunchKernelGGL((from_brick_kernel<float, double>), dim3(1024), dim3(256), 0, st, (const float *)src, dst, L, nfield);
    return hipGetLastError();
}

hipError_t fsm_from_brick_f32(const float *src, float *dst, const FsmLaunch &L, int nfield, hipStream_t st)
{
    hipLaunchKernelGGL((from_brick_kernel<float, float>), dim3(1024), dim3(256), 0, st, src, dst, L, nfield);
    return hipGetLastError();
}

hipError_t fsm_to_brick_f32(const float *src, float *dst, const FsmLaunch &L, int nfield, hipStream_t st)
{
    hipLaunchKernelGGL((to_brick_kernel<float, float>), dim3(1024), dim3(256), 0, st, src, dst, L, nfield);
    return hipGetLastError();
}
```

Before: 633.9.

## Lazily initialize travel-time field blocks instead of filling whole field per solve

```diff
diff --git a/mceik_amd/csrc/capi.hip b/mceik_amd/csrc/capi.hip
--- a/mceik_amd/csrc/capi.hip
+++ b/mceik_amd/csrc/capi.hip
@@ -116,6 +116,11 @@
     L.max_waves = b->max_waves;
     L.traffic = b->traffic;
     L.step_z = b->step_z;
+    L.upad = fsm_launch_kind(L, is_double) == 16 ? MCEIK_UNAN_PAD / 4 : 0;
+    {
+        const char *e = getenv("MCEIK_LAZY_INIT");
+        L.lazy_init = !(e && e[0] == '0');
+    }
 }
 
 static int g_device_cus = 0;
@@ -192,9 +197,10 @@
     size_t es = is_double ? 8 : 4;
     WsLayout w;
     w.nwaves = batch_waves(L, is_double);
-    const size_t zfw = fsm_launch_kind(L, is_double) == 16 ? zf_bytes(L, es) : 0;
+    const size_t zfw = fsm_launch_kind(L, is_double) == 16 ? zf_slot_bytes(L, es) : 0;
+    const size_t fslot = (L.field_elems + (size_t)L.upad) * es;
     {
-        const size_t per_wave = 2 * L.field_elems * es + zfw;
+        const size_t per_wave = 2 * fslot + zfw;
         const long cap = (long)(ws_budget_bytes() / (per_wave ? per_wave : 1));
         if (cap >= 1 && w.nwaves > cap) w.nwaves = (int)cap;
     }
@@ -203,8 +209,8 @@
     size_t slow_bytes = b->slow_mode == 0 ? (size_t)b->nmodel * L.field_elems * es : 0;
     w.u = w.slow + ((slow_bytes + 255) & ~(size_t)255);
     size_t nu = b->u_out ? (size_t)L.nsolve : (size_t)w.nwaves;
-    w.u0 = w.u + nu * L.field_elems * es;
-    w.zf = w.u0 + (size_t)w.nwaves * L.field_elems * es;
+    w.u0 = w.u + nu * fslot;
+    w.zf = w.u0 + (size_t)w.nwaves * fslot;
     w.total = w.zf + (size_t)w.nwaves * zfw;
     return w;
 }
@@ -317,8 +323,8 @@
     } else {
         L.slow = b->slow;
     }
-    L.u = ws + w.u;
-    L.u0 = ws + w.u0;
+    L.u = ws + w.u + (size_t)L.upad * (is_double ? 8 : 4);
+    L.u0 = ws + w.u0 + (size_t)L.upad * (is_double ? 8 : 4);
     L.zf = ws + w.zf;
     L.slot_per_solve = b->u_out ? 1 : 0;
     if (ext) {
diff --git a/mceik_amd/csrc/fsm16_kernel.hip b/mceik_amd/csrc/fsm16_kernel.hip
--- a/mceik_amd/csrc/fsm16_kernel.hip
+++ b/mceik_amd/csrc/fsm16_kernel.hip
@@ -45,6 +45,7 @@
     unsigned *meta;
     unsigned char *fz;
     unsigned *vbits, *cbits;
+    unsigned *wbits;
 };
 template <bool FIXED>
 __device__ __forceinline__ Smem16 smem16_bind(const FsmLaunch &L, unsigned char *base)
@@ -73,6 +74,7 @@
     S.fz = base + off[9];
     S.vbits = reinterpret_cast<unsigned *>(base + off[10]);
     S.cbits = S.vbits + (L.nblocks + 31) / 32;
+    S.wbits = S.cbits + (L.nblocks + 31) / 32;
     S.scratch = reinterpret_cast<int *>(base + off[6]);
     S.xr = reinterpret_cast<float *>(base + off[7]);
     S.meta = reinterpret_cast<unsigned *>(base + off[8]);
@@ -115,6 +117,13 @@
 
 #define NPASS16 4
 #define W1_ZD (1u << 24)
+
+#define LZ_OWN 1u
+#define LZ_ZB 32u
+#define LZ_ZA 64u
+#define LZ_MASK 127u
+#define W1_FW (1u << 25)
+#define U_UNAN 0u
 
 __device__ __forceinline__ void seg_issue(Rsrc r, uint32_t seg, float (&a)[16])
 {
@@ -226,9 +235,11 @@
 template <bool RZ>
 __device__ __forceinline__ BInfo16 brick_info16(const FsmLaunch &L, const Fsm16Geo &g, int kb, const Smem16 &S,
                                                 const Pos &p, int nstream, int lx, int ly, const BcBoxes &bc,
-                                                unsigned meta, uint32_t col)
+                                                unsigned meta, uint32_t colw)
 {
     BInfo16 b;
+    const unsigned lz = colw & LZ_MASK;
+    const uint32_t col = colw & ~LZ_MASK;
     const int tz = ci_tz(meta);
     const int zb = tz * kb + (RZ ? kb - 1 - p.zbs : p.zbs);
     const bool valid = pos_valid(p, nstream) && (meta & C_BLK) && zb < g.nzb;
@@ -240,8 +251,8 @@
     if (zb == (RZ ? g.nzb - 1 : 0)) fl |= F_FIRST;
     if (zb == (RZ ? 0 : g.nzb - 1)) fl |= F_LAST;
     const bool zd = valid && p.zbs == kb - 1 && !(fl & F_LAST);
-    if (b.zh != OOB) b.zh = zf_boundary<float, RZ>(L, S.ring_b[p.ri], false, lx, ly);
-    if (zd) b.zh = zf_boundary<float, RZ>(L, S.ring_b[p.ri], true, lx, ly);
+    if (b.zh != OOB) b.zh = (lz & LZ_ZB) ? ZF_UNAN : zf_boundary<float, RZ>(L, S.ring_b[p.ri], false, lx, ly);
+    if (zd) b.zh = (lz & LZ_ZA) ? ZF_UNAN : zf_boundary<float, RZ>(L, S.ring_b[p.ri], true, lx, ly);
     if ((meta & C_ZH) && p.zbs == 0) fl |= F_ZH;
     bool slow = (fl & C_PART) || ((fl & C_00) && zb == 0) || (valid && zb * 16 + 16 > L.nz);
     unsigned bcm = 0;
@@ -264,19 +275,26 @@
     }
     if (slow) fl |= F_SLOW;
     const int ccb = ci_ccb(meta) + zb * 4;
-    b.w1 = (uint32_t)fl | ((uint32_t)(valid ? zb : 0) << 12) | ((uint32_t)p.ri << 20) | (zd ? W1_ZD : 0u);
+    b.w1 = (uint32_t)fl | ((uint32_t)(valid ? zb : 0) << 12) | ((uint32_t)p.ri << 20) | (zd ? W1_ZD : 0u) |
+           (valid && (lz & LZ_OWN) ? W1_FW : 0u);
     b.w2 = ((uint32_t)ccb & 0xffffu) | ((uint32_t)p.sp << 16);
     b.w3 = ((uint32_t)S.ring_b[p.ri] & 0xffffu) | (bcm << 16);
     return b;
 }
+__device__ __forceinline__ uint32_t load_seg(const BInfo16 &b)
+{
+    return (b.w1 & W1_FW) ? U_UNAN + (b.seg & 64u) : b.seg;
+}
 template <bool RZ>
 __device__ __forceinline__ uint32_t halo_offset16(const Fsm16Geo &g, int kb, const Pos &pe, int nstream, int half,
-                                                  unsigned meta, uint32_t col, unsigned hbit, uint32_t hdelta)
+                                                  unsigned meta, uint32_t colw, unsigned hbit, uint32_t hdelta,
+                                                  unsigned hlz)
 {
     const int zb = ci_tz(meta) * kb + (RZ ? kb - 1 - pe.zbs : pe.zbs);
     const bool valid = pos_valid(pe, nstream) && (meta & C_BLK) && zb < g.nzb;
-    const uint32_t base = col + ((meta & hbit) ? 0u : hdelta);
-    return valid ? base + zoff16(zb) + (uint32_t)half * 32u : OOB;
+    const uint32_t base = (colw & ~LZ_MASK) + ((meta & hbit) ? 0u : hdelta);
+    const bool unw = (colw & ((meta & hbit) ? LZ_OWN : hlz)) != 0u;
+    return valid ? (unw ? U_UNAN + (zoff16(zb) & 64u) : base + zoff16(zb)) + (uint32_t)half * 32u : OOB;
 }
 
 #define LW_G(p) (9 + 5 * (p))
@@ -305,20 +323,22 @@
 }
 template <bool RZ>
 __device__ __forceinline__ BInfo16 brick_info_lean(const FsmLaunch &L, const Smem16 &S, const Pos &p, int nstream,
-                                                   int lx, int ly, const BcBoxes &bc, unsigned w, uint32_t base)
+                                                   int lx, int ly, const BcBoxes &bc, unsigned w, uint32_t basew)
 {
     BInfo16 b;
     const int ph = p.zbs;
     const unsigned gp = (w >> (ph ? LW_G(1) : LW_G(0))) & 31u;
     const bool pv = pos_valid(p, nstream);
     const bool valid = pv && (gp & 16u);
-    const uint32_t off = base + ((uint32_t)(ph ^ (RZ ? 1 : 0)) << 6);
+    const unsigned lz = basew & LZ_MASK;
+    const uint32_t hoff = (uint32_t)(ph ^ (RZ ? 1 : 0)) << 6;
+    const uint32_t off = (basew & ~LZ_MASK) + hoff;
     b.seg = valid ? off : OOB;
-    b.lseg = pv && (w & ((16u << LW_G(0)) | (16u << LW_G(1)))) ? off : OOB;
-    b.zh = valid && (gp & 8u) ? off + (RZ ? 8192u - 64u : 124u - 8192u) : OOB;
+    b.lseg = pv && (w & ((16u << LW_G(0)) | (16u << LW_G(1)))) ? ((lz & LZ_OWN) ? U_UNAN + hoff : off) : OOB;
     const bool zd = valid && ph == 1 && !(gp & 2u);
-    if (b.zh != OOB) b.zh = zf_boundary<float, RZ>(L, S.ring_b[p.ri], false, lx, ly);
-    if (zd) b.zh = zf_boundary<float, RZ>(L, S.ring_b[p.ri], true, lx, ly);
+    b.zh = OOB;
+    if (valid && (gp & 8u)) b.zh = (lz & LZ_ZB) ? ZF_UNAN : zf_boundary<float, RZ>(L, S.ring_b[p.ri], false, lx, ly);
+    if (zd) b.zh = (lz & LZ_ZA) ? ZF_UNAN : zf_boundary<float, RZ>(L, S.ring_b[p.ri], true, lx, ly);
     int fl = valid ? (int)((w & 0x7fu) | F_VALID | ((gp & 15u) << 8)) : 0;
     unsigned bcm = 0;
     if (__any(fl & C_BC)) {
@@ -338,26 +358,30 @@
         if (bcm) fl |= F_SLOW;
     }
     const int ccb = (int)(w >> LW_CCB) + (RZ ? -4 * ph : 4 * ph);
-    b.w1 = (uint32_t)fl | ((uint32_t)ph << 12) | ((uint32_t)p.ri << 20) | (zd ? W1_ZD : 0u);
+    b.w1 = (uint32_t)fl | ((uint32_t)ph << 12) | ((uint32_t)p.ri << 20) | (zd ? W1_ZD : 0u) |
+           (valid && (lz & LZ_OWN) ? W1_FW : 0u);
     b.w2 = ((uint32_t)ccb & 0xffffu) | ((uint32_t)p.sp << 16);
     b.w3 = ((uint32_t)S.ring_b[p.ri] & 0xffffu) | (bcm << 16);
     return b;
 }
 template <bool RZ>
-__device__ __forceinline__ uint32_t halo_offset_lean(const Pos &pe, int nstream, int half, unsigned me, uint32_t base,
-                                                     unsigned hbit, uint32_t hdelta)
+__device__ __forceinline__ uint32_t halo_offset_lean(const Pos &pe, int nstream, int half, unsigned me, uint32_t basew,
+                                                     unsigned hbit, uint32_t hdelta, unsigned hlz)
 {
     const int ph = pe.zbs;
     const bool valid = pos_valid(pe, nstream) && ((me >> (ph ? LW_G(1) : LW_G(0))) & 16u);
-    const uint32_t o = base + ((me & hbit) ? 0u : hdelta) + ((uint32_t)(ph ^ (RZ ? 1 : 0)) << 6) + (uint32_t)half * 32u;
+    const bool unw = (basew & ((me & hbit) ? LZ_OWN : hlz)) != 0u;
+    const uint32_t o = (unw ? U_UNAN : (basew & ~LZ_MASK) + ((me & hbit) ? 0u : hdelta)) +
+                       ((uint32_t)(ph ^ (RZ ? 1 : 0)) << 6) + (uint32_t)half * 32u;
     return valid ? o : OOB;
 }
 template <bool RZ>
-__device__ __forceinline__ uint32_t halo_line_lean(const Pos &pe, int nstream, unsigned me, uint32_t base,
-                                                   unsigned hbit, uint32_t hdelta)
+__device__ __forceinline__ uint32_t halo_line_lean(const Pos &pe, int nstream, unsigned me, uint32_t basew,
+                                                   unsigned hbit, uint32_t hdelta, unsigned hlz)
 {
     const bool valid = pos_valid(pe, nstream) && (me & ((16u << LW_G(0)) | (16u << LW_G(1))));
-    return valid ? base + ((me & hbit) ? 0u : hdelta) : OOB;
+    const bool unw = (basew & ((me & hbit) ? LZ_OWN : hlz)) != 0u;
+    return valid ? (unw ? U_UNAN : (basew & ~LZ_MASK) + ((me & hbit) ? 0u : hdelta)) : OOB;
 }
 __device__ __forceinline__ unsigned dpp_swap_quad_half(unsigned v)
 {
@@ -373,10 +397,11 @@
 }
 template <bool RZ, bool LEAN>
 __device__ __forceinline__ uint32_t halo_offset_any(const Fsm16Geo &g, int kb, const Pos &pe, int nstream, int half,
-                                                    unsigned meta, uint32_t col, unsigned hbit, uint32_t hdelta)
-{
-    if (LEAN) return halo_offset_lean<RZ>(pe, nstream, half, meta, col, hbit, hdelta);
-    return halo_offset16<RZ>(g, kb, pe, nstream, half, meta, col, hbit, hdelta);
+                                                    unsigned meta, uint32_t col, unsigned hbit, uint32_t hdelta,
+                                                    unsigned hlz)
+{
+    if (LEAN) return halo_offset_lean<RZ>(pe, nstream, half, meta, col, hbit, hdelta, hlz);
+    return halo_offset16<RZ>(g, kb, pe, nstream, half, meta, col, hbit, hdelta, hlz);
 }
 
 __device__ __forceinline__ void build_order16(const FsmLaunch &L, unsigned short *order)
@@ -404,7 +429,7 @@
 template <bool RZ, bool LEAN>
 __device__ __forceinline__ void admit16(const FsmLaunch &L, const Fsm16Geo &g, const Smem16 &S, const BcBoxes &bc,
                                         int entry, int zh, int u0flag, int ri, int C, int lx, int ly, int lxs,
-                                        int lys, int rx, int ry, ColTile &ct)
+                                        int lys, int rx, int ry, ColTile &ct, bool lz)
 {
     unsigned meta = 0;
     int bid = 0, nbv = 0;
@@ -415,7 +440,17 @@
         nbv = min(L.kb, L.nzb - tz * L.kb);
         if ((entry & 0xffffff) != ct.tile) column_tile<float>(L, bc, entry, lx, ly, lxs, lys, rx, ry, ct);
         meta = LEAN ? lean_word<RZ>(L, g, ct, tz, ri, u0flag, zh) : column_word(L, L.kb, ct, tz, ri, u0flag, zh);
-        base = (uint32_t)(ty * L.ntx + tx) * tile_bytes<float>(L) + (LEAN ? (uint32_t)tz << 13 : 0u);
+        base = (uint32_t)(ty * L.ntx + tx) * tile_bytes<float>(L) + (LEAN ? (uint32_t)tz << 13 : 0u) + MCEIK_UNAN_PAD;
+        if (lz) {
+            int lane = threadIdx.x;
+            asm volatile("" : "+v"(lane));
+            const int dx = rx ? 1 : -1, dy = ry ? L.ntx : -L.ntx, dz = RZ ? L.ntiles : -L.ntiles;
+            const int dl = lane == 1 ? dx : lane == 2 ? -dx : lane == 3 ? dy : lane == 4 ? -dy : lane == 5 ? dz
+                         : lane == 6 ? -dz : 0;
+            const int t = min(max(bid + dl, 0), L.nblocks - 1);
+            const unsigned wv = S.wbits[t >> 5];
+            base |= (unsigned)__ballot(!((wv >> (t & 31)) & 1u)) & LZ_MASK;
+        }
     }
     const int nact = L.visit_stats && entry >= 0 ? __builtin_popcountll(__ballot(ct.fl & C_ACT)) : 0;
     asm volatile("" ::: "memory");
@@ -424,6 +459,7 @@
         if (entry >= 0) {
             S.lastproc[bid] = (unsigned short)C;
             S.vbits[bid >> 5] |= 1u << (bid & 31);
+            if (lz) S.wbits[bid >> 5] |= 1u << (bid & 31);
             if (L.visit_stats) {
                 S.scratch[0] += nbv;
                 S.scratch[1] += nbv * nact;
@@ -539,6 +575,7 @@
 
     const int hj = lane >> 1, hh = lane & 1, he = halo_edge_lane(hj), hd = (he & 7) + (he >> 3);
     const unsigned hbit = hj < 16 ? C_XOWN : C_YOWN;
+    const unsigned hlz = 2u << (hj >> 3);
     const uint32_t hdelta = halo_delta(L, tile_bytes<float>(L), hj, he, rx, ry);
     const int hlx = rx ? 7 - (he & 7) : (he & 7), hly = ry ? 7 - (he >> 3) : (he >> 3);
     const uint32_t hcol = (uint32_t)colpos(hlx, hly) * 128u;
@@ -547,6 +584,12 @@
     const unsigned xyface = HOLD_OWN | (lx == 0 ? 2u : 0u) | (lx == 7 ? 4u : 0u) | (ly == 0 ? 8u : 0u) |
                             (ly == 7 ? 16u : 0u);
     hold_norm(L, H);
+    static_assert(MCEIK_MAX_BLOCKS <= 64 * 32, "one wbits word per lane");
+    bool lz_on = false;
+    if (L.lazy_init) {
+        const unsigned w = lane < (L.nblocks + 31) / 32 ? S.wbits[lane] : ~0u;
+        lz_on = __ballot(w != ~0u) != 0ull;
+    }
     if (lane == 0) { S.scratch[4] = 0; S.scratch[5] = -1; }
     clock0 = 64;
     auto decide_any = [&](int pos, int ri, int &zh, int &u0) __attribute__((always_inline)) -> int {
@@ -584,7 +627,7 @@
             nstream = pos;
             break;
         }
-        admit16<RZ, LEAN>(L, g, S, bc, e, zh, u0, dri, clock0 + pos, lx, ly, lxs, lys, rx, ry, ct);
+        admit16<RZ, LEAN>(L, g, S, bc, e, zh, u0, dri, clock0 + pos, lx, ly, lxs, lys, rx, ry, ct, lz_on);
         if (e >= 0) {
             cc_issue<CCR>(L, L.kb, sr, e, ccv, ccsize);
             TRAFU(S, 5, ccsize * 4);
@@ -601,14 +644,14 @@
     const int pbr = pair_row(0, lane), pbn = pair_row(1, lane);
     {
         float t[16];
-        seg_issue(ur, b0.seg, t);
+        seg_issue(ur, load_seg(b0), t);
         raw_write(S.xr, pbn, t);
         load_row16(S.xr, 1, lane, v);
     }
     pos_init(pe, -hd, kb, nr);
     {
         const uint32_t ho = halo_offset_any<RZ, LEAN>(g, kb, pe, nstream, hh, S.meta[pe.ri * 64 + he],
-                                              S.ring_base[pe.ri] + hcol, hbit, hdelta);
+                                              S.ring_base[pe.ri] + hcol, hbit, hdelta, hlz);
         bload4h(ur, ho, *reinterpret_cast<float (*)[4]>(&hq[0]));
         bload4h(ur, ho + 16u, *reinterpret_cast<float (*)[4]>(&hq[4]));
         TRAF(S, 1, ho != OOB, 32);
@@ -621,15 +664,15 @@
                                   S.ring_base[p3.ri] + lanecol);
     {
         float t[16];
-        seg_issue(ur, b1.seg, t);
+        seg_issue(ur, load_seg(b1), t);
         raw_write(S.xr, pbn, t);
     }
     if (FL) {
         Pos pn = p3;
         pos_adv(pn, kb, nr);
         const bool nl = pn.vb >= 0 && pn.zbs == 1;
-        const uint32_t sn = nl ? brick_info_any<RZ, LEAN>(L, g, kb, S, pn, nstream, lx, ly, bc, S.meta[pn.ri * 64 + lane],
-                                                  S.ring_base[pn.ri] + lanecol).seg
+        const uint32_t sn = nl ? load_seg(brick_info_any<RZ, LEAN>(L, g, kb, S, pn, nstream, lx, ly, bc,
+                                                                   S.meta[pn.ri * 64 + lane], S.ring_base[pn.ri] + lanecol))
                                : OOB;
         const bool nlp = dpp_swap_pair((unsigned)nl) != 0u;
         const uint32_t snp = dpp_swap_pair(sn);
@@ -645,7 +688,7 @@
     pos_adv(pe, kb, nr);
     if (HFL) {
         const uint32_t lo = halo_line_lean<RZ>(pe, nstream, S.meta[pe.ri * 64 + he], S.ring_base[pe.ri] + hcol, hbit,
-                                               hdelta);
+                                               hdelta, hlz);
         const uint32_t lp = dpp_swap_quad_half(lo);
         const uint32_t l1 = hcme == (hpi ^ 1) ? lo : lp, l0 = hcme == hpi ? lo : lp;
         const uint32_t qo = 16u * (uint32_t)hr, oa = (RZ ? 64u : 0u) + qo, ob = (RZ ? 0u : 64u) + qo;
@@ -655,7 +698,7 @@
         TRAF(S, 1, l1 != OOB, 32);
     } else {
         const uint32_t ho = halo_offset_any<RZ, LEAN>(g, kb, pe, nstream, hh, S.meta[pe.ri * 64 + he],
-                                              S.ring_base[pe.ri] + hcol, hbit, hdelta);
+                                              S.ring_base[pe.ri] + hcol, hbit, hdelta, hlz);
         bload4h(ur, ho, *reinterpret_cast<float (*)[4]>(&hn[0]));
         bload4h(ur, ho + 16u, *reinterpret_cast<float (*)[4]>(&hn[4]));
         TRAF(S, 1, ho != OOB, 32);
@@ -701,7 +744,7 @@
             if (e == -2) {
                 nstream = pos;
             } else {
-                admit16<RZ, LEAN>(L, g, S, bc, e, zh, u0, dri, clock0 + pos, lx, ly, lxs, lys, rx, ry, ct);
+                admit16<RZ, LEAN>(L, g, S, bc, e, zh, u0, dri, clock0 + pos, lx, ly, lxs, lys, rx, ry, ct, lz_on);
                 if (e >= 0) {
                     cc_issue<CCR>(L, L.kb, sr, e, ccv, ccsize);
                     TRAFU(S, 5, ccsize * 4);
@@ -731,10 +774,10 @@
         if (FL)
             line_issue(ur, b3.lseg, p3.vb >= 0 && p3.zbs == 0, lq, hpnew);
         else
-            seg_issue(ur, b3.seg, qa);
+            seg_issue(ur, load_seg(b3), qa);
         zq = __any(b3.zh != OOB) ? bload1(zr_, b3.zh, 0.0f) : 0.0f;
         if (HFL) {
-            const uint32_t lo = halo_line_lean<RZ>(pe, nstream, me, ce, hbit, hdelta);
+            const uint32_t lo = halo_line_lean<RZ>(pe, nstream, me, ce, hbit, hdelta, hlz);
             const uint32_t lp = dpp_swap_quad_half(lo);
             const uint32_t sl = hcme == (hpi ^ P) ? lo : lp;
             const uint32_t qo = 16u * (uint32_t)hr;
@@ -746,7 +789,7 @@
             TRAF(S, 0, b3.seg != OOB, 64);
             TRAF(S, 2, b3.zh != OOB, 4);
         } else {
-            const uint32_t ho = halo_offset_any<RZ, LEAN>(g, kb, pe, nstream, hh, me, ce, hbit, hdelta);
+            const uint32_t ho = halo_offset_any<RZ, LEAN>(g, kb, pe, nstream, hh, me, ce, hbit, hdelta, hlz);
             bload4h(ur, ho, *reinterpret_cast<float (*)[4]>(&hnew[0]));
             bload4h(ur, ho + 16u, *reinterpret_cast<float (*)[4]>(&hnew[4]));
             TRAF(S, 1, ho != OOB, 32);
@@ -820,19 +863,21 @@
         asm volatile("" ::: "memory");
         store_row16(S.xr, 0, lane, v);
         zprev = v[RZ ? 0 : 15];
-        if (__any(changed)) {
+        const bool fw = (b0.w1 & W1_FW) != 0u, st = changed || fw;
+        if (__any(st)) {
             float t[16];
             raw_read(S.xr, pbr, t);
-            raw_store(ur, b0.seg, changed, t);
-        }
-        TRAF(S, 3, changed, 64);
+            raw_store(ur, b0.seg, st, t);
+        }
+        TRAF(S, 3, st, 64);
         {
             const int zr = LEAN ? (b0.zb() ^ (RZ ? 1 : 0)) : b0.zb() % kb;
             const bool zlo = changed && zr == 0 && c0, zhi = changed && zr == kb - 1 && c15;
             if (changed) atomicOr(&S.fmask[b0.ri()], xyface | (zlo ? HOLD_ZLO : 0u) | (zhi ? HOLD_ZHI : 0u));
-            if (__any(zlo || zhi)) {
-                bstore1(zfr, zlo ? zf_off<float>(b0.bid(), 0, lx, ly) : OOB, v[0]);
-                bstore1(zfr, zhi ? zf_off<float>(b0.bid(), 1, lx, ly) : OOB, v[15]);
+            const bool slo = zlo || (fw && zr == 0), shi = zhi || (fw && zr == kb - 1);
+            if (__any(slo || shi)) {
+                bstore1(zfr, slo ? zf_off<float>(b0.bid(), 0, lx, ly) : OOB, v[0]);
+                bstore1(zfr, shi ? zf_off<float>(b0.bid(), 1, lx, ly) : OOB, v[15]);
             }
         }
         load_row16(S.xr, 1, lane, v);
@@ -887,7 +932,7 @@
             const int zend = min(tz * L.kb + L.kb, L.nzb);
             for (int zb = tz * L.kb; zb < zend; zb++) {
                 const uint32_t seg = (uint32_t)id * tile_bytes<float>(L) + zoff_bytes<float>(zb) +
-                                     (uint32_t)colpos(lx, ly) * 128u;
+                                     (uint32_t)colpos(lx, ly) * 128u + MCEIK_UNAN_PAD;
                 float u[8], v0[8];
                 bload8(ur, seg, u);
                 bload8(u0r, seg, v0);
@@ -1052,8 +1097,9 @@
         if (L.solve_clock && lane == 0) L.solve_clock[2 * (size_t)solve] = __builtin_amdgcn_s_memrealtime();
         const int model = (int)solve / L.nstat, station = (int)solve - model * L.nstat;
         const size_t slot = L.slot_per_solve ? solve : blockIdx.x;
-        float *u = reinterpret_cast<float *>(L.u) + slot * L.field_elems;
-        float *u0 = reinterpret_cast<float *>(L.u0) + (size_t)blockIdx.x * L.field_elems;
+        const size_t fslot = L.field_elems + (size_t)L.upad;
+        float *u = reinterpret_cast<float *>(L.u) + slot * fslot;
+        float *u0 = reinterpret_cast<float *>(L.u0) + (size_t)blockIdx.x * fslot;
         const size_t ncell = (size_t)L.ncx * L.ncy * L.ncz;
         const int phase = L.model_phase ? (MC ? mcmcd::ldv(L.model_phase + model) : L.model_phase[model])
                                         : fsm_plain_phase(L, model);
@@ -1066,9 +1112,10 @@
         }
         const size_t sentry = !L.model_phase ? (size_t)model : (size_t)model * L.nphase + phase;
         const void *slow_model = reinterpret_cast<const float *>(L.slow) + sentry * ncell;
-        const Rsrc ur = make_rsrc(u, fbytes), u0r = make_rsrc(u0, fbytes),
+        const Rsrc ur = make_rsrc(u - MCEIK_UNAN_PAD / 4, fbytes + MCEIK_UNAN_PAD),
+                   u0r = make_rsrc(u0 - MCEIK_UNAN_PAD / 4, fbytes + MCEIK_UNAN_PAD),
                    sr = make_rsrc(slow_model, (uint32_t)(ncell * 4));
-        const size_t zfb = zf_bytes(L, 4);
+        const size_t zfb = zf_slot_bytes(L, 4);
         const Rsrc zfr = make_rsrc(reinterpret_cast<char *>(L.zf) + (size_t)blockIdx.x * zfb, (uint32_t)zfb);
         if (lane == 0) { S.scratch[0] = 0; S.scratch[1] = 0; S.scratch[2] = 0; S.scratch[3] = 0; }
 #ifdef MCEIK_TRAFFIC
@@ -1078,9 +1125,41 @@
         unsigned nchg = 0, nsteps = 0;
         BcBoxes bc;
         bc.box = S.box;
-        const bool ok = init_field<float, 1>(L, u, ur, slow_model, L.src + (size_t)station * L.nsrc * 4, bc);
+        auto block_fill = [&](int b) __attribute__((always_inline)) {
+            const int tz = b / L.ntiles, id = b - tz * L.ntiles;
+            const int lg0 = tz * L.kb / 4, lg1 = mceik_div_up(min(tz * L.kb + L.kb, L.nzb), 4);
+            fill_unan<float>(ur, MCEIK_UNAN_PAD + (uint32_t)id * tile_bytes<float>(L) + (uint32_t)lg0 * 8192u,
+                             (uint32_t)(lg1 - lg0) * 8192u);
+        };
+        const int nbw = (L.nblocks + 31) / 32;
+        for (int w = lane; w < nbw; w += 64)
+            S.wbits[w] = !L.lazy_init ? ~0u : (w == nbw - 1 && (L.nblocks & 31)) ? ~0u << (L.nblocks & 31) : 0u;
+        asm volatile("" ::: "memory");
+        fill_unan<float>(ur, U_UNAN, MCEIK_UNAN_PAD);
+        const double *srcs = L.src + (size_t)station * L.nsrc * 4;
+        bool ok;
+        if (L.lazy_init) {
+            ok = init_sources<float, 1>(L, u, slow_model, srcs, bc, [&](int s) __attribute__((always_inline)) {
+                asm volatile("" ::: "memory");
+                int q[6];
+                for (int i = 0; i < 6; i++) q[i] = __builtin_amdgcn_readfirstlane(bc.box[6 * s + i]);
+                for (int tz = q[4] / (8 * L.kb); tz <= q[5] / (8 * L.kb); tz++)
+                    for (int ty = q[2] >> 3; ty <= q[3] >> 3; ty++)
+                        for (int tx = q[0] >> 3; tx <= q[1] >> 3; tx++) {
+                            const int b = (tz * L.nty + ty) * L.ntx + tx;
+                            const unsigned wv = __builtin_amdgcn_readfirstlane(S.wbits[b >> 5]);
+                            if ((wv >> (b & 31)) & 1u) continue;
+                            block_fill(b);
+                            if (lane == 0) S.wbits[b >> 5] = wv | (1u << (b & 31));
+                            asm volatile("" ::: "memory");
+                        }
+            });
+        } else {
+            fill_unan<float>(ur, MCEIK_UNAN_PAD, fbytes);
+            ok = init_sources<float, 1>(L, u, slow_model, srcs, bc, [](int) {});
+        }
         hold_solve_start(L, hold_lds16(S), bc, g.nr);
-        zf_init<float>(L, zfr, u, bc);
+        zf_init<float>(L, zfr, u, bc, L.lazy_init ? S.wbits : nullptr);
         asm volatile("" ::: "memory");
         int iters = 0, ierr_last = 0;
         if (ok) {
@@ -1128,8 +1207,15 @@
             if (L.niter) L.niter[solve] = iters;
             if (L.ierr) L.ierr[solve] = ierr;
         }
-        TRAFU(S, 7, (unsigned)(L.field_elems * 4) + (L.ttab ? (unsigned)L.nev * (4u + 64u) : 0u));
+        TRAFU(S, 7, (L.lazy_init ? 0u : (unsigned)(L.field_elems * 4)) + (L.ttab ? (unsigned)L.nev * (4u + 64u) : 0u));
         TRAF_FLUSH(L, S);
+        if (L.lazy_init && (L.slot_per_solve || L.ttab)) {
+            asm volatile("" ::: "memory");
+            for (int w = 0; w < nbw; w++) {
+                for (unsigned m = ~__builtin_amdgcn_readfirstlane(S.wbits[w]); m; m &= m - 1)
+                    block_fill(w * 32 + __builtin_ctz(m));
+            }
+        }
         if (L.ttab) {
             for (int e = lane; e < L.nev; e += 64) L.ttab[(size_t)solve * L.nev + e] = event_time<float>(L, u, e);
         }
diff --git a/mceik_amd/csrc/fsm_common.h b/mceik_amd/csrc/fsm_common.h
--- a/mceik_amd/csrc/fsm_common.h
+++ b/mceik_amd/csrc/fsm_common.h
@@ -55,6 +55,7 @@
     unsigned mc_spin_limit;
     int mc_step0, mc_nsteps;
     int mc_nburn, mc_keepk, mc_maxs, mc_nkept0;
+    int lazy_init, upad;
 };
 #define MC_SYNC_WORDS(nchains) (8 + 8 * 32 + 2 * (nchains) + 1)
 
@@ -70,6 +71,8 @@
 
 static inline __host__ __device__ int mceik_div_up(int a, int b) { return (a + b - 1) / b; }
 static inline __host__ __device__ size_t zf_bytes(const FsmLaunch &L, size_t es) { return (size_t)L.nblocks * 128 * es; }
+#define MCEIK_UNAN_PAD 128
+static inline __host__ __device__ size_t zf_slot_bytes(const FsmLaunch &L, size_t es) { return zf_bytes(L, es) + MCEIK_UNAN_PAD; }
 
 #if defined(MCEIK_TRAFFIC)
 #define MCEIK_SCRATCH_BYTES 64
@@ -177,7 +180,7 @@
 }
 static inline __host__ __device__ size_t f16_bitmap_bytes(const FsmLaunch &L)
 {
-    return mceik_align16((size_t)((L.nblocks + 31) / 32) * 4 * 2);
+    return mceik_align16((size_t)((L.nblocks + 31) / 32) * 4 * 3);
 }
 static inline __host__ __device__ size_t fsm16_smem_layout(const FsmLaunch &L, size_t *off)
 {
diff --git a/mceik_amd/csrc/fsm_device.h b/mceik_amd/csrc/fsm_device.h
--- a/mceik_amd/csrc/fsm_device.h
+++ b/mceik_amd/csrc/fsm_device.h
@@ -259,19 +259,23 @@
     return godunov_fast64<FAST>(a, b, c, f);
 }
 
-template <typename R, int SLOWMODE>
-__device__ __forceinline__ bool init_field(const FsmLaunch &L, R *u, Rsrc ur, const void *slow_model, const double *src,
-                           BcBoxes &bc)
-{
-    const int lane = threadIdx.x;
+template <typename R>
+__device__ __forceinline__ void fill_unan(Rsrc r, uint32_t off, uint32_t bytes)
+{
     const R UN = Num<R>::unan();
-    const uint32_t nvec = (uint32_t)(L.field_elems / 8);
     R fill[8];
 #pragma unroll
     for (int i = 0; i < 8; i++) fill[i] = UN;
-    for (uint32_t i = lane; i < nvec; i += 64) bstore8(ur, i * 8u * (uint32_t)sizeof(R), fill);
+    const uint32_t nvec = bytes / (8u * (uint32_t)sizeof(R));
+    for (uint32_t i = threadIdx.x; i < nvec; i += 64) bstore8(r, off + i * 8u * (uint32_t)sizeof(R), fill);
     __builtin_amdgcn_s_waitcnt(0);
     __builtin_amdgcn_fence(__ATOMIC_SEQ_CST, "workgroup");
+}
+template <typename R, int SLOWMODE, typename Pre>
+__device__ __forceinline__ bool init_sources(const FsmLaunch &L, R *u, const void *slow_model, const double *src,
+                                             BcBoxes &bc, Pre pre)
+{
+    const int lane = threadIdx.x;
     bc.n = L.nsrc;
     bool ok = true;
     for (int s = 0; s < L.nsrc; s++) {
@@ -302,6 +306,7 @@
             if (lane == 0) { bc.box[6 * s + 2 * a] = lo; bc.box[6 * s + 2 * a + 1] = hi; }
         }
         if (!ok) { bc.n = s; break; }
+        pre(s);
         if (lane < 27) {
             int i = lane % 3, j = (lane / 3) % 3, k = lane / 9;
             int ix = loc[0][i], iy = loc[1][j], iz = loc[2][k];
@@ -323,6 +328,13 @@
     __builtin_amdgcn_fence(__ATOMIC_SEQ_CST, "workgroup");
     return ok;
 }
+template <typename R, int SLOWMODE>
+__device__ __forceinline__ bool init_field(const FsmLaunch &L, R *u, Rsrc ur, const void *slow_model, const double *src,
+                           BcBoxes &bc)
+{
+    fill_unan<R>(ur, 0u, (uint32_t)(L.field_elems * sizeof(R)));
+    return init_sources<R, SLOWMODE>(L, u, slow_model, src, bc, [](int) {});
+}
 
 __device__ __forceinline__ int next_solve(const FsmLaunch &L, int &pass)
 {
diff --git a/mceik_amd/csrc/fsm_hold.h b/mceik_amd/csrc/fsm_hold.h
--- a/mceik_amd/csrc/fsm_hold.h
+++ b/mceik_amd/csrc/fsm_hold.h
@@ -348,10 +348,11 @@
     asm volatile("" ::: "memory");
 }
 
+#define ZF_UNAN 0u
 template <typename R>
 __device__ __forceinline__ uint32_t zf_off(int b, int side, int lx, int ly)
 {
-    return ((uint32_t)(b * 2 + side) * 64u + (uint32_t)(lx + 8 * ly)) * (uint32_t)sizeof(R);
+    return ((uint32_t)(b * 2 + side) * 64u + (uint32_t)(lx + 8 * ly)) * (uint32_t)sizeof(R) + MCEIK_UNAN_PAD;
 }
 template <typename R, bool RZ>
 __device__ __forceinline__ uint32_t zf_boundary(const FsmLaunch &L, int b, bool zd, int lx, int ly)
@@ -360,16 +361,20 @@
     return zf_off<R>(b + (up ? L.ntiles : -L.ntiles), up ? 0 : 1, lx, ly);
 }
 template <typename R>
-__device__ __forceinline__ void zf_init(const FsmLaunch &L, Rsrc zfr, const R *u, const BcBoxes &bc)
+__device__ __forceinline__ void zf_init(const FsmLaunch &L, Rsrc zfr, const R *u, const BcBoxes &bc,
+                                        const unsigned *wbits = nullptr)
 {
     const int lane = threadIdx.x;
-    const R UN = Num<R>::unan();
-    R fill[8];
-#pragma unroll
-    for (int i = 0; i < 8; i++) fill[i] = UN;
-    const uint32_t nvec = (uint32_t)(zf_bytes(L, sizeof(R)) / (8 * sizeof(R)));
-    for (uint32_t i = lane; i < nvec; i += 64) bstore8(zfr, i * 8u * (uint32_t)sizeof(R), fill);
-    __builtin_amdgcn_s_waitcnt(0);
+    if (!wbits) {
+        fill_unan<R>(zfr, 0u, (uint32_t)zf_slot_bytes(L, sizeof(R)));
+    } else {
+        fill_unan<R>(zfr, 0u, MCEIK_UNAN_PAD);
+        for (int w = 0; w < (L.nblocks + 31) / 32; w++)
+            for (unsigned m = __builtin_amdgcn_readfirstlane(wbits[w]); m; m &= m - 1) {
+                const int b = w * 32 + __builtin_ctz(m);
+                if (b < L.nblocks) fill_unan<R>(zfr, zf_off<R>(b, 0, 0, 0), 128u * (uint32_t)sizeof(R));
+            }
+    }
     const int zbk = 8 * L.kb;
     for (int s = 0; s < bc.n; s++) {
         const int *q = bc.box + 6 * s;
diff --git a/mceik_amd/csrc/fsm_kernel.hip b/mceik_amd/csrc/fsm_kernel.hip
--- a/mceik_amd/csrc/fsm_kernel.hip
+++ b/mceik_amd/csrc/fsm_kernel.hip
@@ -1032,7 +1032,7 @@
         size_t fld = i / nn, e = i - fld * nn;
         int x = (int)(e % L.nx); size_t t = e / L.nx;
         int y = (int)(t % L.ny); int z = (int)(t / L.ny);
-        dst[i] = (RD)src[fld * L.field_elems + brick_index<RS>(L, x, y, z)];
+        dst[i] = (RD)src[fld * (L.field_elems + (size_t)L.upad) + brick_index<RS>(L, x, y, z)];
     }
 }
 
```

New measurement: 640.4 (median of 5 runs). 1.01x the previous value.
